# HPCForge/Bubbleformer

Measured on AMD Instinct MI355X. Metric: train samples/sec, FiLMAViT 16x192x192x4ch, bs=8 per GPU, higher is better.
Workload: dtype bf16; 1 GPU; FiLMAViT-small (E=384, 6 heads, 12 blocks, P=16, 9 fluid params) fwd + relative-L2 loss + bwd + AdamW, 4-field 16x192x192 clips, batch 8 per GPU (BASELINE.json configs[1]); global_batch=8, parallelism=dp1

## Files before the change

bubbleformer_amd/_lib.py:

```python
import ctypes as C
import os
import subprocess

_HERE = os.path.dirname(os.path.abspath(__file__))
LIB_PATH = os.path.join(_HERE, "libbubbleformer_hip.so")
CSRC = os.path.join(_HERE, "csrc")

BF_DTYPE_F32, BF_DTYPE_BF16 = 0, 1
BF_LAY_KC, BF_LAY_XC = 0, 1
BF_PRO_NONE, BF_PRO_AFFINE, BF_PRO_AFFINE_GELU, BF_PRO_GELU = 0, 1, 2, 3
BF_AUX_NONE, BF_AUX_ADD, BF_AUX_DGELU = 0, 1, 2
BF_OUT_STORE, BF_OUT_STORE_F32, BF_OUT_ATOMIC_F32 = 0, 1, 2
BF_MAX_STAGES = 5
BF_LOSS_LIMBS = 5

vp, fp, i32, i64, f32 = C.c_void_p, C.c_void_p, C.c_int32, C.c_int64, C.c_float


class Operand(C.Structure):
    _fields_ = [("p", vp), ("ld", i64), ("layout", i32), ("seglen", i32), ("segstride", i64), ("gw", i32), ("gh", i32),
                ("gc", i32), ("pro", i32), ("sc", fp), ("sh", fp), ("rows_per_frame", i32), ("nch", i32)]


class Epilogue(C.Structure):
# ... 24 lines not shown


class FrameNorm(C.Structure):
    _fields_ = [("w", fp), ("b", fp), ("g", fp), ("gdiv", i32), ("mean", fp), ("rstd", fp), ("sc", fp), ("sh", fp), ("resid", vp), ("out", vp)]


class EmbedParams(C.Structure):
    _fields_ = [("conv_w", fp * BF_MAX_STAGES), ("in_w", fp * BF_MAX_STAGES), ("in_b", fp * BF_MAX_STAGES), ("film_ln_w", fp),
                ("film_ln_b", fp), ("film_w", fp), ("film_b", fp)]


class DebedParams(C.Structure):
    _fields_ = [("conv_w", fp * BF_MAX_STAGES), ("in_w", fp * BF_MAX_STAGES), ("in_b", fp * BF_MAX_STAGES)]


class ConvSrc(C.Structure):
    _fields_ = [("p", vp), ("C", i32), ("nchw", i32), ("f32", i32)]


class ConvGeo(C.Structure):
    _fields_ = [(n, i32) for n in ("F", "Hi", "Wi", "Ho", "Wo", "kh", "kw", "stride", "pad")]


BF_CONV_PRO_NONE, BF_CONV_PRO_AFFINE_GELU, BF_CONV_PRO_GELU = 0, 1, 2

STAGE_DONE_FN = C.CFUNCTYPE(None, C.c_int, C.c_void_p)
P = C.POINTER
SIGNATURES = {
    "bf_last_error": (C.c_char_p, []),
    "bf_abi_version": (C.c_int, []),
    "bf_prof_enable": (None, [C.c_int]),
    "bf_debug_force_generic_attn": (None, [C.c_int]),
    "bf_debug_tokred_fold": (None, [C.c_int]),
    "bf_side_defer": (None, [C.c_int]),
    "bf_prep_stages": (C.c_int, [C.POINTER(Dims), C.c_int, C.POINTER(C.c_int32), C.POINTER(vp), C.POINTER(vp), C.POINTER(vp), vp]),
    "bf_stage_prepared": (None, [C.c_int]),
    "bf_trunk_train_fwd": (C.c_int, [C.POINTER(Dims), C.c_int, C.POINTER(C.c_int32), C.POINTER(vp), C.POINTER(vp), C.POINTER(vp), C.POINTER(vp), vp,
                                     C.POINTER(vp), vp, vp]),
    "bf_trunk_train_bwd": (C.c_int, [C.POINTER(Dims), C.c_int, C.POINTER(C.c_int32), C.POINTER(vp), C.POINTER(vp), C.POINTER(vp), C.POINTER(vp),
                                     C.POINTER(vp), vp, C.POINTER(vp), vp, C.POINTER(vp), vp, vp, vp, vp, vp]),
    "bf_field_stats_ws_doubles": (i64, [C.c_int]),
    "bf_field_stats": (C.c_int, [fp, vp, vp, C.c_int, vp, vp, vp]),
    "bf_stage_chain_next": (C.c_int, [C.POINTER(Dims), C.c_int, vp, vp]),
    "bf_stage_next_scale": (C.c_int, [fp, C.c_int]),
    "bf_gemm_fwd_frames": (C.c_int, [C.c_int, C.c_int, C.c_int, C.c_int, vp, i64, vp, i64, fp, fp, fp, fp, C.c_int, vp, vp, C.c_int,
                                     C.POINTER(FrameNorm), C.POINTER(FrameNorm), vp]),
    "bf_trunk_eval_weights_bytes": (i64, [C.POINTER(Dims), C.c_int, C.POINTER(C.c_int32)]),
    "bf_trunk_eval_prepare": (C.c_int, [C.POINTER(Dims), C.c_int, C.POINTER(C.c_int32), C.POINTER(vp), vp, vp]),
    "bf_trunk_eval_fwd": (C.c_int, [C.POINTER(Dims), C.c_int, C.POINTER(C.c_int32), C.POINTER(vp), vp, vp, vp, vp, vp]),
    "bf_frame_linear": (C.c_int, [C.c_int, C.c_int, C.c_int, C.c_int, C.c_int, vp, i64, vp, i64, fp, fp, fp, fp, fp, vp, i64, C.c_int, fp, fp, fp,
                                  vp, i64, fp, fp, vp, i64, vp]),
    "bf_side_join": (C.c_int, [vp]),
    "bf_prof_report": (C.c_int, [C.c_char_p, C.c_int]),
    "bf_gemm": (C.c_int, [C.c_int, C.c_int, C.c_int, C.c_int, P(Operand), P(Operand), P(Epilogue), C.c_int, vp]),
    "bf_gemm_tokred": (C.c_int, [C.c_int, C.c_int, C.c_int, i64, vp, i64, vp, i64, fp, C.c_int, fp, fp, i64, vp]),
    "bf_gemm_tokred_ws_floats": (i64, [C.c_int, C.c_int, i64]),
    "bf_gemm_inbwd_frames": (C.c_int, [C.c_int, C.c_int, C.c_int, C.c_int, vp, i64, vp, i64, vp, vp, vp, C.c_int, fp, fp, fp, fp, fp, C.c_int, vp]),
    "bf_gemm_inbwd_frames_chain": (C.c_int, [C.c_int, C.c_int, C.c_int, C.c_int, vp, i64, vp, i64, vp, vp, vp, C.c_int, fp, fp, fp, fp, fp, C.c_int,
                                             vp, vp, fp, fp, fp, fp, C.c_int, fp, vp]),
    "bf_in_stats": (C.c_int, [C.c_int, vp, C.c_int, C.c_int, C.c_int, fp, fp, fp, C.c_int, fp, fp, fp, fp, fp, fp, vp]),
    "bf_in_ws_floats": (i64, [C.c_int, C.c_int, C.c_int, C.c_int]),
    "bf_affine_apply": (C.c_int, [C.c_int, vp, vp, fp, fp, vp, i64, C.c_int, C.c_int, vp]),
    "bf_in_bwd": (C.c_int, [C.c_int, vp, vp, vp, vp, C.c_int, C.c_int, C.c_int, fp, fp, fp, fp, fp, C.c_int, C.c_int, fp, fp,
                            fp, fp, fp, vp]),
    "bf_colsum": (C.c_int, [C.c_int, vp, i64, C.c_int, fp, fp, vp]),
    "bf_attn_axial_fwd": (C.c_int, [C.c_int, vp, vp, i64, C.c_int, C.c_int, C.c_int, C.c_int, fp, fp, fp, fp, fp, fp, fp, vp]),
    "bf_attn_axial_norm_fwd": (C.c_int, [C.c_int, vp, vp, vp, i64, C.c_int, C.c_int, C.c_int, C.c_int, fp, fp, fp, fp, fp, fp, fp, fp, fp, fp, fp, fp,
                                         fp, vp]),
    "bf_attn_fwd": (C.c_int, [C.c_int, vp, vp, i64, C.c_int, i64, i64, i64, i64, C.c_int, C.c_int, fp, fp, fp, fp, fp, fp, f32,
                              C.c_int, vp]),
    "bf_attn_bwd": (C.c_int, [C.c_int, vp, vp, vp, i64, C.c_int, i64, i64, i64, i64, C.c_int, C.c_int, fp, fp, fp, fp, fp, fp,
                              fp, fp, fp, fp, fp, fp, f32, C.c_int, fp, i64, vp]),
    "bf_im2col_nchw": (C.c_int, [C.c_int, fp, vp, C.c_int, C.c_int, C.c_int, C.c_int, C.c_int, vp]),
    "bf_col2im_nchw": (C.c_int, [C.c_int, vp, fp, C.c_int, C.c_int, C.c_int, C.c_int, C.c_int, vp]),
    "bf_pm2nchw": (C.c_int, [fp, fp, fp, fp, C.c_int, C.c_int, C.c_int, C.c_int, C.c_int, vp]),
    "bf_debed_last_bwd": (C.c_int, [C.c_int, fp, fp, fp, fp, fp, vp, vp, vp, C.c_int, C.c_int, C.c_int, C.c_int, C.c_int, C.c_int, vp]),
    "bf_debed_last_bwd_norm": (C.c_int, [C.c_int, fp, fp, fp, fp, fp, vp, vp, vp, fp, fp, fp, fp, vp, fp, fp, C.c_int, C.c_int, C.c_int, C.c_int, C.c_int,
                                         C.c_int, fp, C.c_int64, vp]),
    "bf_gather_gemm": (C.c_int, [C.c_int, vp, vp, C.c_int, fp, fp, vp, C.c_int, C.c_int, C.c_int, C.c_int, C.c_int, vp]),
    "bf_scatter_gemm": (C.c_int, [C.c_int, vp, vp, C.c_int, fp, fp, vp, fp, C.c_int, C.c_int, C.c_int, C.c_int, C.c_int, vp]),
    "bf_gather_wgrad_ws_floats": (C.c_int64, [C.c_int, C.c_int, C.c_int]),
    "bf_gather_wgrad": (C.c_int, [C.c_int, vp, vp, fp, fp, fp, fp, fp, C.c_int, C.c_int, C.c_int, C.c_int, C.c_int, C.c_int, fp, C.c_int64, vp]),
    "bf_gather_gemm_rebuilt": (C.c_int, [C.c_int, vp, vp, vp, C.c_int, fp, fp, vp, C.c_int, C.c_int, C.c_int, C.c_int, C.c_int, vp]),
    "bf_gather_wgrad_rebuilt": (C.c_int, [C.c_int, vp, vp, vp, fp, fp, fp, C.c_int, C.c_int, C.c_int, C.c_int, C.c_int, C.c_int, fp, C.c_int64, vp]),
    "bf_stage_chain_head": (C.c_int, [vp, vp, vp]),
    "bf_stage_chain_tail": (C.c_int, [vp, vp, C.c_int]),
    "bf_embed_tail_ws_floats": (C.c_int64, [C.c_int, C.c_int, C.c_int, C.c_int, C.c_int]),
    "bf_embed_tail_bwd": (C.c_int, [C.c_int, vp, vp, vp, vp, vp, fp, fp, fp, fp, fp, fp, fp, fp, C.c_int, C.c_int, C.c_int, C.c_int, C.c_int, C.c_int,
                                    fp, C.c_int64, vp]),
    "bf_embed_first": (C.c_int, [C.c_int, fp, vp, vp, vp, C.c_int, C.c_int, C.c_int, C.c_int, C.c_int, C.c_int, fp, vp]),
    "bf_in_stats_merge_slices": (C.c_int, [C.c_int, C.c_int, C.c_int, C.c_int, C.c_int, fp, fp, fp, C.c_int, fp, fp, fp, fp, fp, fp, vp]),
    "bf_debed_last": (C.c_int, [C.c_int, vp, fp, fp, vp, fp, fp, fp, C.c_int, C.c_int, C.c_int, C.c_int, C.c_int, C.c_int, vp]),
    "bf_lploss_finalize": (C.c_int, [fp, C.c_int, C.c_int, fp, fp, vp]),
    "bf_nchw2pm": (C.c_int, [C.c_int, fp, fp, fp, fp, fp, vp, C.c_int, C.c_int, C.c_int, C.c_int, C.c_int, vp]),
    "bf_wprep": (C.c_int, [C.c_int, C.c_int, fp, vp, C.c_int, C.c_int, C.c_int, vp]),
    "bf_wgrad_unprep": (C.c_int, [C.c_int, fp, fp, C.c_int, C.c_int, C.c_int, C.c_int, vp]),
    "bf_film_net_fwd": (C.c_int, [fp, fp, fp, fp, fp, fp, fp, fp, C.c_int, C.c_int, C.c_int, vp]),
    "bf_film_net_bwd": (C.c_int, [fp, fp, fp, fp, fp, fp, fp, fp, fp, C.c_int, C.c_int, C.c_int, vp]),
    "bf_adamw": (C.c_int, [fp, fp, fp, fp, i64, C.c_int, f32, f32, f32, f32, f32, f32, vp]),
    "bf_adam": (C.c_int, [fp, fp, fp, fp, i64, C.c_int, f32, f32, f32, f32, f32, f32, vp]),
    "bf_lion": (C.c_int, [fp, fp, fp, i64, f32, f32, f32, f32, f32, vp]),
    "bf_grad_norm_ws_doubles": (i64, [i64]),
    "bf_grad_norm": (C.c_int, [fp, i64, f32, f32, fp, vp, i64, vp]),
    "bf_adamw_dev": (C.c_int, [fp, fp, fp, fp, i64, C.c_int, f32, f32, f32, f32, f32, f32, fp, f32, vp]),
    "bf_adam_dev": (C.c_int, [fp, fp, fp, fp, i64, C.c_int, f32, f32, f32, f32, f32, f32, fp, f32, vp]),
# ... 99 lines not shown
```

bubbleformer_amd/csrc/attn.hip:

```cpp
#include "bf_common.h"
#include "param_reduce.h"

namespace {

constexpr int NT = 256;
__device__ __forceinline__ void wave_sync() {
    __builtin_amdgcn_fence(__ATOMIC_ACQ_REL, "wavefront");
    __builtin_amdgcn_wave_barrier();
}
constexpr int LMAX = 32;
constexpr int LONG_LMAX = 128;
constexpr int DMAX = 128;

__device__ __forceinline__ int t5_bucket(int n) {
    const int a = n < 0 ? -n : n;
    int b;
    if (a < 8) b = a;
    else if (a < 10) b = 8;
    else if (a < 12) b = 9;
    else if (a < 14) b = 10;
    else if (a < 16) b = 11;
    else if (a < 20) b = 12;
    else if (a < 23) b = 13;
    else if (a < 27) b = 14;
// ... 307 lines not shown

template <typename K>
int plan_waves(K kernel, size_t floats_per_wave, int* wpb, size_t* shm) {
    int w = 4;
    while (w > 1 && (size_t)w * floats_per_wave * sizeof(float) > 64 * 1024) w >>= 1;
    *wpb = w;
    *shm = (size_t)w * floats_per_wave * sizeof(float);
    if (*shm > 156 * 1024) return bf_fail_msg("attention: L*d too large for the LDS plan", __FILE__, __LINE__);
    if (*shm > 64 * 1024) {
        hipError_t e = hipFuncSetAttribute(reinterpret_cast<const void*>(kernel), hipFuncAttributeMaxDynamicSharedMemorySize, (int)*shm);
        if (e != hipSuccess) return bf_fail(e, __FILE__, __LINE__);
    }
    return 0;
}

bool g_force_generic = false;

int check_geo(const char* who, int dtype, int heads, int d, int L) {
    const int ch = dtype == BF_DTYPE_BF16 ? 8 : 4;
    if (heads < 1 || heads > 16) return bf_fail_msg("attention: heads must be in 1..16", who, 0);
    if (d < ch || d > DMAX || d % ch) return bf_fail_msg("attention: head dim must be a multiple of the 16-byte chunk and <= 128", who, 0);
    if (L < 1 || L > LONG_LMAX) return bf_fail_msg("attention: sequence length must be in 1..128", who, 0);
    return 0;
}

}

int bf_attn_fwd_mfma(const void* qkv, void* out, long nseq, int L, long inner, long outer_stride, long inner_stride, long tok_stride, int heads,
                     int d, const float* qw, const float* qb, const float* kw, const float* kb, const float* emb, const float* hscale,
                     float out_scale, int accumulate, hipStream_t st);
int bf_attn_bwd_mfma(const void* qkv, const void* dout, void* dqkv, long nseq, int L, long inner, long outer_stride, long inner_stride,
                     long tok_stride, int heads, int d, const float* qw, const float* qb, const float* kw, const float* kb, const float* emb,
                     const float* hscale, float* dqw, float* dqb, float* dkw, float* dkb, float* demb, float* dhscale, float out_scale,
                     int accumulate, float* ws, long ws_floats, int* rows_out, hipStream_t st);
int bf_attn_fwd_long(int dtype, const void* qkv, void* out, long nseq, int L, long inner, long outer_stride, long inner_stride, long tok_stride,
                     int heads, int d, const float* qw, const float* qb, const float* kw, const float* kb, const float* emb, const float* hscale,
                     float out_scale, int accumulate, hipStream_t st);
int bf_attn_bwd_long(int dtype, const void* qkv, const void* dout, void* dqkv, long nseq, int L, long inner, long outer_stride, long inner_stride,
                     long tok_stride, int heads, int d, const float* qw, const float* qb, const float* kw, const float* kb, const float* emb,
                     const float* hscale, float* dqw, float* dqb, float* dkw, float* dkb, float* demb, float* dhscale, float out_scale,
                     int accumulate, float* ws, long ws_floats, int* rows_out, hipStream_t st);
int bf_attn_axial_fwd_mfma(const void* qkv, void* out, int frames, int h, int w, int heads, int d, const float* qw, const float* qb, const float* kw,
                           const float* kb, const float* emb, const float* hscale_x, const float* hscale_y, const float* nw, const float* nb,
                           void* out_n, float* mean, float* rstd, float* sc, float* sh, hipStream_t st);
static bool use_mfma(int dtype, int d) { return !g_force_generic && dtype == BF_DTYPE_BF16 && d % 32 == 0 && d <= 128; }
bool bf_attn_raw_modes(int dtype, int d) { return use_mfma(dtype, d); }

extern "C" void bf_debug_force_generic_attn(int on) { g_force_generic = on != 0; }

extern "C" int bf_attn_fwd(int dtype, const void* qkv, void* out, int64_t nseq, int L, int64_t inner, int64_t outer_stride,
                           int64_t inner_stride, int64_t tok_stride, int heads, int d, const float* qw, const float* qb,
                           const float* kw, const float* kb, const float* emb, const float* hscale, float out_scale,
                           int accumulate, bf_stream_t stream) {
    BF_REQUIRE(qkv && out && qw && qb && kw && kb && nseq > 0 && inner > 0, "bf_attn_fwd: bad arguments");
    if (int rc = check_geo("bf_attn_fwd", dtype, heads, d, L)) return rc;
    if (L > LMAX) {
        BfProfScope prof((hipStream_t)stream, "attn_fwd", 4.0 * nseq * heads * L * L * d, (double)nseq * heads * L * d * bf_esize(dtype) * (accumulate ? 5.0 : 4.0));
        return bf_attn_fwd_long(dtype, qkv, out, nseq, L, inner, outer_stride, inner_stride, tok_stride, heads, d, qw, qb, kw, kb, emb, hscale,
                                out_scale, accumulate, (hipStream_t)stream);
    }
    if (use_mfma(dtype, d)) {
        BfProfScope prof((hipStream_t)stream, "attn_fwd", 4.0 * nseq * heads * L * L * d, (double)nseq * heads * L * d * 2.0 * (accumulate ? 5.0 : 4.0));
        return bf_attn_fwd_mfma(qkv, out, nseq, L, inner, outer_stride, inner_stride, tok_stride, heads, d, qw, qb, kw, kb, emb, hscale, out_scale,
                                accumulate, (hipStream_t)stream);
    }
    SeqGeo g{nseq, L, inner, outer_stride, inner_stride, tok_stride};
    AttnParams p{qw, qb, kw, kb, emb, hscale};
// ... 14 lines not shown
extern "C" int bf_attn_axial_fwd(int dtype, const void* qkv, void* out, int64_t frames, int h, int w, int heads, int d, const float* qw,
                                 const float* qb, const float* kw, const float* kb, const float* emb, const float* hscale_x,
                                 const float* hscale_y, bf_stream_t stream) {
    BF_REQUIRE(qkv && out && qw && qb && kw && kb && frames > 0 && h > 0 && w > 0, "bf_attn_axial_fwd: bad arguments");
    if (use_mfma(dtype, d) && frames < (1L << 24)) {
        BfProfScope prof((hipStream_t)stream, "attn_fwd", 4.0 * frames * heads * h * w * (h + w) * d, (double)frames * h * w * heads * d * 2.0 * 4.0);
        const int rc = bf_attn_axial_fwd_mfma(qkv, out, (int)frames, h, w, heads, d, qw, qb, kw, kb, emb, hscale_x, hscale_y, nullptr, nullptr, nullptr,
                                              nullptr, nullptr, nullptr, nullptr, (hipStream_t)stream);
        if (rc <= 0) return rc;
    }
    const long S = (long)h * w;
    int rc = bf_attn_fwd(dtype, qkv, out, frames * h, w, 1, w, 0, 1, heads, d, qw, qb, kw, kb, emb, hscale_x, 0.5f, 0, stream);
    if (rc) return rc;
    return bf_attn_fwd(dtype, qkv, out, frames * w, h, w, S, 1, w, heads, d, qw, qb, kw, kb, emb, hscale_y, 0.5f, 1, stream);
}

extern "C" int bf_attn_axial_norm_fwd(int dtype, const void* qkv, void* out, void* out_n, int64_t frames, int h, int w, int heads, int d,
                                      const float* qw, const float* qb, const float* kw, const float* kb, const float* emb,
                                      const float* hscale_x, const float* hscale_y, const float* norm_w, const float* norm_b, float* mean,
                                      float* rstd, float* sc, float* sh, bf_stream_t stream) {
    BF_REQUIRE(qkv && out && out_n && qw && qb && kw && kb && norm_w && norm_b && mean && rstd && sc && sh && frames > 0 && h > 0 && w > 0,
               "bf_attn_axial_norm_fwd: bad arguments");
    static const bool off = bf_knob("BF_ATTN_AXIAL_NORM", 1) == 0;
    if (off || !use_mfma(dtype, d) || frames >= (1L << 24)) return 1;
    BfProfScope prof((hipStream_t)stream, "attn_fwd", 4.0 * frames * heads * h * w * (h + w) * d, (double)frames * h * w * heads * d * 2.0 * 5.0);
    return bf_attn_axial_fwd_mfma(qkv, out, (int)frames, h, w, heads, d, qw, qb, kw, kb, emb, hscale_x, hscale_y, norm_w, norm_b, out_n, mean, rstd, sc,
                                  sh, (hipStream_t)stream);
}

static int attn_bwd_impl(int dtype, const void* qkv, const void* dout, void* dqkv, int64_t nseq, int L, int64_t inner,
                         int64_t outer_stride, int64_t inner_stride, int64_t tok_stride, int heads, int d, const float* qw,
                         const float* qb, const float* kw, const float* kb, const float* emb, const float* hscale,
                         float* dqw, float* dqb, float* dkw, float* dkb, float* demb, float* dhscale, float out_scale,
                         int accumulate, float* ws, int64_t ws_floats, int* rows_out, bf_stream_t stream) {
    if (rows_out) *rows_out = 0;
    BF_REQUIRE(qkv && dout && dqkv && qw && qb && kw && kb && nseq > 0 && inner > 0, "bf_attn_bwd: bad arguments");
    if (int rc = check_geo("bf_attn_bwd", dtype, heads, d, L)) return rc;
    BF_REQUIRE(accumulate == 0 || accumulate == 1 || ((accumulate == 2 || accumulate == 5) && use_mfma(dtype, d)),
               "bf_attn_bwd: accumulate must be 0 / 1 (or 2 / 5, the raw-gradient pair of passes, on the bf16 MFMA path)");
    if (L > LMAX) {
        BfProfScope prof((hipStream_t)stream, "attn_bwd", 10.0 * nseq * heads * L * L * d, (double)nseq * heads * L * d * bf_esize(dtype) * (accumulate ? 10.0 : 7.0));
        return bf_attn_bwd_long(dtype, qkv, dout, dqkv, nseq, L, inner, outer_stride, inner_stride, tok_stride, heads, d, qw, qb, kw, kb, emb, hscale,
                                dqw, dqb, dkw, dkb, demb, dhscale, out_scale, accumulate, ws, (long)ws_floats, rows_out, (hipStream_t)stream);
    }
    if (use_mfma(dtype, d)) {
        BfProfScope prof((hipStream_t)stream, "attn_bwd", 10.0 * nseq * heads * L * L * d, (double)nseq * heads * L * d * 2.0 * (accumulate ? 10.0 : 7.0));
        return bf_attn_bwd_mfma(qkv, dout, dqkv, nseq, L, inner, outer_stride, inner_stride, tok_stride, heads, d, qw, qb, kw, kb, emb, hscale, dqw,
                                dqb, dkw, dkb, demb, dhscale, out_scale, accumulate, ws, (long)ws_floats, rows_out, (hipStream_t)stream);
    }
    SeqGeo g{nseq, L, inner, outer_stride, inner_stride, tok_stride};
    AttnParams p{qw, qb, kw, kb, emb, hscale};
    AttnGrads gr{dqw, dqb, dkw, dkb, demb, dhscale};
    const size_t fpw = 6 * L * (d + 1) + 2 * L * (L + 1) + 2 * L;
    int WPB; size_t shm;
    if (int rc = dtype == BF_DTYPE_BF16 ? plan_waves(attn_bwd_kernel<bf16>, fpw, &WPB, &shm) : plan_waves(attn_bwd_kernel<float>, fpw, &WPB, &shm)) return rc;
    const long nprob = nseq * heads;
    BfProfScope prof((hipStream_t)stream, "attn_bwd", 10.0 * nprob * L * L * d, (double)nprob * L * d * bf_esize(dtype) * (accumulate ? 10.0 : 7.0));
    const int full = (int)std::min<long>((nprob + WPB - 1) / WPB, 256 * 4), nvals = 4 * d + 32 * heads + heads;
    int grid = full;
    if (ws && ws_floats < (int64_t)full * nvals) { grid = (int)(ws_floats / nvals); if (grid < 1) { ws = nullptr; grid = full; } }
    if (dtype == BF_DTYPE_BF16)
        hipLaunchKernelGGL(attn_bwd_kernel<bf16>, dim3(grid), dim3(WPB * 64), shm, (hipStream_t)stream, (const bf16*)qkv, (const bf16*)dout, (bf16*)dqkv, g, heads, d, p, gr, out_scale, accumulate, ws);
    else
        hipLaunchKernelGGL(attn_bwd_kernel<float>, dim3(grid), dim3(WPB * 64), shm, (hipStream_t)stream, (const float*)qkv, (const float*)dout, (float*)dqkv, g, heads, d, p, gr, out_scale, accumulate, ws);
    BF_CHECK_LAUNCH();
    if (rows_out) { *rows_out = ws ? grid : 0; return 0; }
    if (ws) {
        const AttnReduceJob j{ws, grid, d, heads, dqw, dqb, dkw, dkb, demb, dhscale};
        hipLaunchKernelGGL(attn_rows_reduce_kernel, dim3(bf_cdiv(nvals, 64)), dim3(64 * BF_RED_FL), 0, (hipStream_t)stream, j);
        BF_CHECK_LAUNCH();
    }
    return 0;
}

extern "C" int bf_attn_bwd(int dtype, const void* qkv, const void* dout, void* dqkv, int64_t nseq, int L, int64_t inner,
                           int64_t outer_stride, int64_t inner_stride, int64_t tok_stride, int heads, int d, const float* qw,
                           const float* qb, const float* kw, const float* kb, const float* emb, const float* hscale,
                           float* dqw, float* dqb, float* dkw, float* dkb, float* demb, float* dhscale, float out_scale,
                           int accumulate, float* ws, int64_t ws_floats, bf_stream_t stream) {
    return attn_bwd_impl(dtype, qkv, dout, dqkv, nseq, L, inner, outer_stride, inner_stride, tok_stride, heads, d, qw, qb, kw, kb, emb, hscale, dqw,
                         dqb, dkw, dkb, demb, dhscale, out_scale, accumulate, ws, ws_floats, nullptr, stream);
}
int bf_attn_bwd_partials(int dtype, const void* qkv, const void* dout, void* dqkv, int64_t nseq, int L, int64_t inner, int64_t outer_stride,
                         int64_t inner_stride, int64_t tok_stride, int heads, int d, const float* qw, const float* qb, const float* kw,
                         const float* kb, const float* emb, const float* hscale, float* dqw, float* dqb, float* dkw, float* dkb, float* demb,
                         float* dhscale, float out_scale, int accumulate, float* ws, int64_t ws_floats, int* rows, hipStream_t stream) {
    return attn_bwd_impl(dtype, qkv, dout, dqkv, nseq, L, inner, outer_stride, inner_stride, tok_stride, heads, d, qw, qb, kw, kb, emb, hscale, dqw,
                         dqb, dkw, dkb, demb, dhscale, out_scale, accumulate, ws, ws_floats, rows, (bf_stream_t)stream);
}
```

bubbleformer_amd/csrc/attn_mfma.hip:

```cpp
#include "bf_common.h"
#include "param_reduce.h"
#include <stdlib.h>

namespace {

typedef __attribute__((ext_vector_type(8))) short s16x8;
typedef __attribute__((address_space(3))) s16x4* lds_s16x4;

__device__ __forceinline__ void drain_vm() { __builtin_amdgcn_s_waitcnt(0x0F70); }
__device__ __forceinline__ void wsync() {
    __builtin_amdgcn_fence(__ATOMIC_ACQ_REL, "wavefront");
    __builtin_amdgcn_wave_barrier();
}
__device__ __forceinline__ int t5b(int n) {
    const int a = n < 0 ? -n : n;
    int b;
    if (a < 8) b = a; else if (a < 10) b = 8; else if (a < 12) b = 9; else if (a < 14) b = 10; else if (a < 16) b = 11;
    else if (a < 20) b = 12; else if (a < 23) b = 13; else if (a < 27) b = 14; else b = 15;
    return b + (n < 0 ? 16 : 0);
}
typedef unsigned u32x2 __attribute__((ext_vector_type(2)));
__device__ __forceinline__ float quad_sum(float v) {
    u32x2 r = __builtin_amdgcn_permlane16_swap(__float_as_uint(v), __float_as_uint(v), false, false);
    v = __uint_as_float(r[0]) + __uint_as_float(r[1]);
    r = __builtin_amdgcn_permlane32_swap(__float_as_uint(v), __float_as_uint(v), false, false);
    return __uint_as_float(r[0]) + __uint_as_float(r[1]);
}
__device__ __forceinline__ float row16_sum(float v) {
    v += __builtin_bit_cast(float, __builtin_amdgcn_update_dpp(0, __builtin_bit_cast(int, v), 0xB1, 0xF, 0xF, true));
    v += __builtin_bit_cast(float, __builtin_amdgcn_update_dpp(0, __builtin_bit_cast(int, v), 0x4E, 0xF, 0xF, true));
    v += __builtin_bit_cast(float, __builtin_amdgcn_update_dpp(0, __builtin_bit_cast(int, v), 0x141, 0xF, 0xF, true));
    v += __builtin_bit_cast(float, __builtin_amdgcn_update_dpp(0, __builtin_bit_cast(int, v), 0x140, 0xF, 0xF, true));
    return v;
}
__device__ __forceinline__ float quad_max(float v) {
    u32x2 r = __builtin_amdgcn_permlane16_swap(__float_as_uint(v), __float_as_uint(v), false, false);
    v = fmaxf(__uint_as_float(r[0]), __uint_as_float(r[1]));
    r = __builtin_amdgcn_permlane32_swap(__float_as_uint(v), __float_as_uint(v), false, false);
    return fmaxf(__uint_as_float(r[0]), __uint_as_float(r[1]));
}

struct Geo { long nseq; int L; long inner, outer_stride, inner_stride, tok_stride; };
struct Prob { long tok0; int head; };
__device__ __forceinline__ Prob locate(const Geo& g, int heads, long pr) {
    const unsigned p = (unsigned)pr, hd = (unsigned)heads, inner = (unsigned)g.inner;
    const unsigned s = p / hd, head = p - s * hd;
    const unsigned q = s / inner, r = s - q * inner;
    return Prob{(long)q * g.outer_stride + (long)r * g.inner_stride, (int)head};
}
template <int CTRL>
__device__ __forceinline__ float dpp_add(float keep, float send) {
    return keep + __builtin_bit_cast(float, __builtin_amdgcn_update_dpp(0, __builtin_bit_cast(int, send), CTRL, 0xF, 0xF, true));
}
__device__ __forceinline__ float row16_scatter_sum(const float (&p)[16], int i16) {
    float a0, a1, a2, a3, a4, a5, a6, a7, b[4];
#define BF_M1(a, lo, hi) "v_add_f32_dpp " a ", " lo ", " lo " row_mirror row_mask:0xf bank_mask:0x3\n\t" \
                         "v_add_f32_dpp " a ", " hi ", " hi " row_mirror row_mask:0xf bank_mask:0xc\n\t"
#define BF_M2(b, lo, hi) "v_add_f32_dpp " b ", " lo ", " lo " row_half_mirror row_mask:0xf bank_mask:0x5\n\t" \
                         "v_add_f32_dpp " b ", " hi ", " hi " row_half_mirror row_mask:0xf bank_mask:0xa\n\t"
    asm("s_nop 4\n\t"
        BF_M1("%4", "%12", "%20") BF_M1("%5", "%13", "%21") BF_M1("%6", "%14", "%22") BF_M1("%7", "%15", "%23")
        BF_M1("%8", "%16", "%24") BF_M1("%9", "%17", "%25") BF_M1("%10", "%18", "%26") BF_M1("%11", "%19", "%27")
        BF_M2("%0", "%4", "%8") BF_M2("%1", "%5", "%9") BF_M2("%2", "%6", "%10") BF_M2("%3", "%7", "%11")
        : "=&v"(b[0]), "=&v"(b[1]), "=&v"(b[2]), "=&v"(b[3]), "=&v"(a0), "=&v"(a1), "=&v"(a2), "=&v"(a3), "=&v"(a4), "=&v"(a5), "=&v"(a6), "=&v"(a7)
        : "v"(p[0]), "v"(p[1]), "v"(p[2]), "v"(p[3]), "v"(p[4]), "v"(p[5]), "v"(p[6]), "v"(p[7]),
          "v"(p[8]), "v"(p[9]), "v"(p[10]), "v"(p[11]), "v"(p[12]), "v"(p[13]), "v"(p[14]), "v"(p[15]));
#undef BF_M1
#undef BF_M2
    const bool b1 = i16 & 2, b0 = i16 & 1;
    float c[2];
#pragma unroll
    for (int j = 0; j < 2; ++j) c[j] = dpp_add<0x4E>(b1 ? b[2 + j] : b[j], b1 ? b[j] : b[2 + j]);
    return dpp_add<0xB1>(b0 ? c[1] : c[0], b0 ? c[0] : c[1]);
}
struct Par { const float *qw, *qb, *kw, *kb, *emb, *hscale; };
struct Grd { float *dqw, *dqb, *dkw, *dkb, *demb, *dhscale; };

__device__ __forceinline__ s16x4 tr4(const bf16* tile, int ld, int r0, int c0, int lane) {
    const int i16 = lane & 15, q = i16 >> 2, p = i16 & 3;
// ... 442 lines not shown
            __syncthreads();
        }
    }
}

template <int NB, int KS> struct RawRows { bf16x8 q[NB][KS], k[NB][KS], v[NB][KS], d[NB][KS]; };
template <int NB, int KS> struct OldRows { bf16x8 q[NB][KS], k[NB][KS], v[NB][KS]; };

template <int NB, int KS>
__device__ __forceinline__ void load_raw(RawRows<NB, KS>& r, const bf16* __restrict__ qkv, const bf16* __restrict__ dout, const Geo& g, int heads, const Prob& at,
                                         int lane) {
    constexpr int D = 32 * KS;
    const int E = heads * D;
    const int head = at.head;
    const long tok0 = at.tok0;
    const int gq = lane >> 4, i16 = lane & 15;
#pragma unroll
    for (int b = 0; b < NB; ++b) {
        const int i = b * 16 + i16, ic = i < g.L ? i : g.L - 1;
        const bf16* rp = qkv + (tok0 + ic * g.tok_stride) * 3L * E + head * 3 * D + 8 * gq;
        const bf16* dp = dout + (tok0 + ic * g.tok_stride) * (long)E + head * D + 8 * gq;
#pragma unroll
        for (int ks = 0; ks < KS; ++ks) {
            r.q[b][ks] = *reinterpret_cast<const bf16x8*>(rp + 32 * ks);
            r.k[b][ks] = *reinterpret_cast<const bf16x8*>(rp + D + 32 * ks);
            r.v[b][ks] = *reinterpret_cast<const bf16x8*>(rp + 2 * D + 32 * ks);
            r.d[b][ks] = *reinterpret_cast<const bf16x8*>(dp + 32 * ks);
        }
    }
}

template <int NB, int KS, int ACC>
__global__ void __launch_bounds__(256, ((NB == 1 && KS <= 2) ? 2 : 1)) attn_bwd_mfma(const bf16* __restrict__ qkv, const bf16* __restrict__ dout, bf16* __restrict__ dqkv, Geo g,
                                                     int heads, Par p, Grd gr, float out_scale, int accumulate_rt, float* __restrict__ ws) {
    constexpr int D = 32 * KS, LD = D + 16, NT16 = D / 16, R = 16 * NB, LDP = 32 + 8;
    constexpr bool PREFETCH = NB * KS <= 4;
    extern __shared__ __attribute__((aligned(16))) bf16 smem_bwd[];
    __shared__ float s_demb[32 * 16];
    __shared__ float s_dhs[16];
    __shared__ __attribute__((aligned(16))) float s_par[4 * 32 * KS];
    __shared__ float s_emb[32 * 16];
    __shared__ float s_hsc[16];
    const int lane = threadIdx.x & 63, wave = __builtin_amdgcn_readfirstlane(threadIdx.x >> 6), wpb = blockDim.x >> 6;
    constexpr int PER_WAVE = 3 * R * LD + 2 * R * LDP;
    static_assert(3 * R * LD * 2 >= 4 * D * 4, "the parameter-gradient flush must fit in the operand tiles");
    bf16* qn_t = smem_bwd + wave * PER_WAVE;
    bf16* kn_t = qn_t + R * LD;
    bf16* do_t = kn_t + R * LD;
    bf16* at_t = do_t + R * LD;
    bf16* ds_t = at_t + R * LDP;
    float* relay = reinterpret_cast<float*>(qn_t);
    for (int i = threadIdx.x; i < 32 * 16; i += blockDim.x) {
        s_demb[i] = 0.f;
        const int t = i >> 4, h = i & 15;
        s_emb[i] = (p.emb && h < heads) ? p.emb[t * heads + h] : 0.f;
    }
    if (threadIdx.x < 16) { s_dhs[threadIdx.x] = 0.f; s_hsc[threadIdx.x] = (p.hscale && (int)threadIdx.x < heads) ? p.hscale[threadIdx.x] : 1.f; }
    for (int i = threadIdx.x; i < 4 * D; i += blockDim.x) {
        const int q = i / D, e = i % D;
        s_par[i] = (q == 0 ? p.qw : q == 1 ? p.qb : q == 2 ? p.kw : p.kb)[e];
    }
    __syncthreads();
    const int E = heads * D, L = g.L;
    const float scale = rsqrtf((float)D);
    const long nprob = g.nseq * heads;
    const int gq = lane >> 4, i16 = lane & 15;
    const int mode = ACC >= 0 ? ACC : accumulate_rt;
    const bool raw_out = mode & 2, raw_in = mode & 4, accumulate = mode & 1;

    constexpr int NACC = 2 * KS;
    float a_ln[NACC];
#pragma unroll
    for (int k = 0; k < NACC; ++k) a_ln[k] = 0.f;
    const long pstep = (long)gridDim.x * wpb;
    const bool one_head = pstep % heads == 0;
    float a_emb[NB][NB][4], a_dhs = 0.f;
#pragma unroll
    for (int jb = 0; jb < NB; ++jb)
#pragma unroll
        for (int ib = 0; ib < NB; ++ib)
#pragma unroll
            for (int r = 0; r < 4; ++r) a_emb[jb][ib][r] = 0.f;
    long pr = (long)blockIdx.x * wpb + wave;
    RawRows<NB, KS> cur, nxt;
    Prob at = locate(g, heads, pr < nprob ? pr : 0), at_next = at;
    if (pr < nprob) load_raw<NB, KS>(cur, qkv, dout, g, heads, at, lane);
    if (PREFETCH) drain_vm();
    float mk[NB][NB][4], mneg[NB][NB][4];
    int eidx[NB][NB][4];
    lane_masks<NB>(L, lane, mk, mneg, eidx);
    if (NB == 1) {
        for (int c = lane; c < 16 * 16; c += 64) { at_t[(c >> 4) * LDP + 16 + (c & 15)] = (bf16)0.f; ds_t[(c >> 4) * LDP + 16 + (c & 15)] = (bf16)0.f; }
    }
    for (; pr < nprob; pr += pstep) {
        const int head = at.head;
        const long tok0 = at.tok0;
        const bool more = pr + pstep < nprob;
        if (more) at_next = locate(g, heads, pr + pstep);
        if (PREFETCH && more) load_raw<NB, KS>(nxt, qkv, dout, g, heads, at_next, lane);
        OldRows<NB, KS> old;
        if (accumulate) {
#pragma unroll
            for (int b = 0; b < NB; ++b) {
                const int row = b * 16 + i16, rc = row < L ? row : L - 1;
                const bf16* ob = dqkv + (tok0 + rc * g.tok_stride) * 3L * E + head * 3 * D;
#pragma unroll
                for (int ks = 0; ks < KS; ++ks) {
                    old.q[b][ks] = *reinterpret_cast<const bf16x8*>(ob + 32 * ks + 8 * gq);
                    old.k[b][ks] = *reinterpret_cast<const bf16x8*>(ob + D + 32 * ks + 8 * gq);
                    old.v[b][ks] = *reinterpret_cast<const bf16x8*>(ob + 2 * D + 32 * ks + 8 * gq);
                }
                if (raw_in && row >= L) {
                    const bf16x8 z8 = {};
#pragma unroll
                    for (int ks = 0; ks < KS; ++ks) { old.q[b][ks] = z8; old.k[b][ks] = z8; }
                }
            }
        }
        float xq[NB][KS][8], xk[NB][KS][8], rq[NB], rk[NB];
        bf16x8 qf[NB][KS], kf[NB][KS], vf[NB][KS], df[NB][KS];
#pragma unroll
        for (int b = 0; b < NB; ++b) {
#pragma unroll
            for (int ks = 0; ks < KS; ++ks)
#pragma unroll
                for (int j = 0; j < 8; ++j) { xq[b][ks][j] = (float)cur.q[b][ks][j]; xk[b][ks][j] = (float)cur.k[b][ks][j]; }
            rq[b] = ln_quad<KS>(xq[b], D);
            affine_frag<KS>(xq[b], s_par, s_par + D, scale, lane, qf[b]);
            rk[b] = ln_quad<KS>(xk[b], D);
            affine_frag<KS>(xk[b], s_par + 2 * D, s_par + 3 * D, 1.f, lane, kf[b]);
            const int row = b * 16 + i16;
// ... 149 lines not shown
#pragma unroll
                    for (int ks = 0; ks < KS; ++ks) {
                        bf16x8 o;
#pragma unroll
                        for (int j = 0; j < 8; ++j) {
                            const float xh = part == 0 ? xq[b][ks][j] : xk[b][ks][j];
                            float v = rs * (dn[ks][j] - m1 - xh * m2);
                            if (accumulate && !raw_in) v += (float)(part == 0 ? old.q[b][ks][j] : old.k[b][ks][j]);
                            o[j] = (bf16)v;
                        }
                        *reinterpret_cast<bf16x8*>(dst + 32 * ks) = o;
                    }
                }
            }
            {
                float flat[16 * KS];
#pragma unroll
                for (int ks = 0; ks < KS; ++ks)
#pragma unroll
                    for (int j = 0; j < 8; ++j) { flat[8 * ks + j] = pw[ks][j]; flat[8 * KS + 8 * ks + j] = pb[ks][j]; }
#pragma unroll
                for (int gi = 0; gi < KS; ++gi) {
                    float grp[16];
#pragma unroll
                    for (int q = 0; q < 16; ++q) grp[q] = flat[16 * gi + q];
                    a_ln[part * KS + gi] += row16_scatter_sum(grp, i16);
                }
            }
        }
        wsync();
        if (PREFETCH) cur = nxt;
        else if (more) load_raw<NB, KS>(cur, qkv, dout, g, heads, at_next, lane);
        at = at_next;
    }
    if (one_head && pr - pstep >= 0) {
        const int head = (int)(((long)blockIdx.x * wpb + wave) % heads);
#pragma unroll
        for (int jb = 0; jb < NB; ++jb)
#pragma unroll
            for (int ib = 0; ib < NB; ++ib)
#pragma unroll
                for (int r = 0; r < 4; ++r) {
                    const int i = 16 * ib + i16, j = 16 * jb + 4 * gq + r;
                    if (gr.demb && i < L && j < L) atomicAdd(&s_demb[t5b(i - j) * 16 + head], a_emb[jb][ib][r]);
                }
        if (p.hscale && gr.dhscale) {
            a_dhs = wave_sum(a_dhs);
            if (lane == 0) atomicAdd(&s_dhs[head], a_dhs);
        }
    }
#pragma unroll
    for (int k = 0; k < NACC; ++k) {
        const int v = 16 * k + i16, q = v / (8 * KS), ks = (v >> 3) % KS, j = v & 7;
        relay[q * D + 32 * ks + 8 * gq + j] = a_ln[k];
    }
    __syncthreads();
    const int nvals = 4 * D + 32 * heads + heads;
    for (int i = threadIdx.x; i < nvals; i += blockDim.x) {
        float val;
        float* dst;
        if (i < 4 * D) {
            val = 0.f;
            for (int w = 0; w < wpb; ++w) val += reinterpret_cast<const float*>(smem_bwd + w * PER_WAVE)[i];
            const int q = i / D, e = i % D; dst = (q == 0 ? gr.dqw : q == 1 ? gr.dqb : q == 2 ? gr.dkw : gr.dkb); if (dst) dst += e; }
        else if (i < 4 * D + 32 * heads) { const int t = i - 4 * D; val = s_demb[(t / heads) * 16 + (t % heads)]; dst = gr.demb ? gr.demb + t : nullptr; }
        else { const int t = i - 4 * D - 32 * heads; val = s_dhs[t]; dst = gr.dhscale ? gr.dhscale + t : nullptr; }
// ... 1 lines not shown
        else if (dst && val != 0.f) atomicAdd(dst, val);
    }
}

__global__ void __launch_bounds__(64 * BF_RED_FL) attn_ws_reduce(AttnReduceJob j) {
    __shared__ float red[1][BF_RED_FL][64];
    attn_reduce_block(j, blockIdx.x, blockIdx.y, gridDim.y, red);
}

template <typename K>
int set_lds(K kernel, size_t shm) {
    if (shm > 64 * 1024) {
        hipError_t e = hipFuncSetAttribute(reinterpret_cast<const void*>(kernel), hipFuncAttributeMaxDynamicSharedMemorySize, (int)shm);
        if (e != hipSuccess) return bf_fail(e, __FILE__, __LINE__);
    }
    return 0;
}

template <int NB, int KS>
int go_fwd(const bf16* qkv, bf16* out, Geo g, int heads, Par p, float out_scale, int accumulate, hipStream_t st) {
    constexpr int D = 32 * KS;
    const int wpb = 4;
    const size_t shm = (size_t)wpb * 16 * NB * (D + 16) * sizeof(bf16);
    const long nprob = g.nseq * heads;
    BF_REQUIRE(nprob < (1L << 31) && g.inner < (1L << 31), "attention: problem count must fit 31 bits");
    static const int bpc = bf_knob("BF_ATTN_FWD_BPC", 2);
    const int grid = (int)std::min<long>((nprob + wpb - 1) / wpb, 256L * bpc);
    hipLaunchKernelGGL((attn_fwd_mfma<NB, KS>), dim3(grid), dim3(wpb * 64), shm, st, qkv, out, g, heads, p, out_scale, accumulate);
    BF_CHECK_LAUNCH();
    return 0;
}
template <int NB, int KS, int ACC>
int go_bwd_mode(const bf16* qkv, const bf16* dout, bf16* dqkv, Geo g, int heads, Par p, Grd gr, float out_scale, int accumulate, float* ws,
                long ws_floats, int* rows_out, hipStream_t st) {
    constexpr int D = 32 * KS, R = 16 * NB;
    const int wpb = NB == 1 ? 4 : 2;
    const size_t shm = (size_t)wpb * (3 * R * (D + 16) + 2 * R * 40) * sizeof(bf16);
    if (int rc = set_lds(attn_bwd_mfma<NB, KS, ACC>, shm)) return rc;
    const long nprob = g.nseq * heads;
    BF_REQUIRE(nprob < (1L << 31) && g.inner < (1L << 31), "attention: problem count must fit 31 bits");
    const int nvals = 4 * D + 32 * heads + heads;
    static int resident = 0;
    if (!resident) {
        int dev = 0, cus = 256, per_cu = 1;
        (void)hipGetDevice(&dev);
        (void)hipDeviceGetAttribute(&cus, hipDeviceAttributeMultiprocessorCount, dev);
        if (hipOccupancyMaxActiveBlocksPerMultiprocessor(&per_cu, attn_bwd_mfma<NB, KS, ACC>, wpb * 64, shm) != hipSuccess || per_cu < 1) per_cu = 1;
        static const int bpc = bf_knob("BF_ATTN_BWD_BPC", 0);
        if (bpc > 0) per_cu = bpc;
        resident = cus * per_cu;
    }
    long grid = std::min<long>((nprob + wpb - 1) / wpb, (long)resident);
    {
        long a = wpb, b = heads;
        while (b) { const long t = a % b; a = b; b = t; }
        const long m = heads / a;
        if (grid >= 8 * m) grid -= grid % m;
    }
    if (ws && ws_floats < grid * nvals) { grid = ws_floats / nvals; if (grid < 1) ws = nullptr; }
    hipLaunchKernelGGL((attn_bwd_mfma<NB, KS, ACC>), dim3((int)grid), dim3(wpb * 64), shm, st, qkv, dout, dqkv, g, heads, p, gr, out_scale, accumulate, ws);
    BF_CHECK_LAUNCH();
    if (rows_out) { *rows_out = ws ? (int)grid : 0; return 0; }
    if (ws) {
        const AttnReduceJob j{ws, (int)grid, D, heads, gr.dqw, gr.dqb, gr.dkw, gr.dkb, gr.demb, gr.dhscale};
        hipLaunchKernelGGL(attn_ws_reduce, dim3(bf_cdiv(nvals, 64), 1), dim3(64 * BF_RED_FL), 0, st, j);
        BF_CHECK_LAUNCH();
    }
    return 0;
}
template <int NB, int KS>
int go_bwd(const bf16* qkv, const bf16* dout, bf16* dqkv, Geo g, int heads, Par p, Grd gr, float out_scale, int accumulate, float* ws,
           long ws_floats, int* rows_out, hipStream_t st) {
#define BF_MODE(A) return go_bwd_mode<NB, KS, A>(qkv, dout, dqkv, g, heads, p, gr, out_scale, accumulate, ws, ws_floats, rows_out, st)
    if constexpr (NB == 1 && KS == 2) {
        switch (accumulate) { case 0: BF_MODE(0); case 1: BF_MODE(1); case 2: BF_MODE(2); case 5: BF_MODE(5); default: break; }
    }
    BF_MODE(-1);
#undef BF_MODE
}

}

int bf_attn_fwd_mfma(const void* qkv, void* out, long nseq, int L, long inner, long outer_stride, long inner_stride, long tok_stride, int heads,
                     int d, const float* qw, const float* qb, const float* kw, const float* kb, const float* emb, const float* hscale,
                     float out_scale, int accumulate, hipStream_t st) {
    Geo g{nseq, L, inner, outer_stride, inner_stride, tok_stride};
    Par p{qw, qb, kw, kb, emb, hscale};
    const int nb = L <= 16 ? 1 : 2, ks = d / 32;
#define GO(NB, KS) if (nb == NB && ks == KS) return go_fwd<NB, KS>((const bf16*)qkv, (bf16*)out, g, heads, p, out_scale, accumulate, st)
    GO(1, 1); GO(1, 2); GO(1, 3); GO(1, 4); GO(2, 1); GO(2, 2); GO(2, 3); GO(2, 4);
#undef GO
    return bf_fail_msg("bf_attn_fwd_mfma: unsupported shape", __FILE__, __LINE__);
}
int bf_attn_axial_fwd_mfma(const void* qkv, void* out, int frames, int h, int w, int heads, int d, const float* qw, const float* qb, const float* kw,
                           const float* kb, const float* emb, const float* hscale_x, const float* hscale_y, const float* nw, const float* nb,
                           void* out_n, float* mean, float* rstd, float* sc, float* sh, hipStream_t st) {
    static const bool off = bf_knob("BF_ATTN_AXIAL_FUSED", 1) == 0;
    if (off || h > 16 || w > 16 || h < 1 || w < 1 || d % 32 || d > 128 || heads > 16) return 1;
    Par p{qw, qb, kw, kb, emb, hscale_x};
    const long ntile = (long)frames * heads;
    static const int wpb_env = bf_knob("BF_ATTN_AXIAL_WPB", 0);
    const int ks = d / 32, wpb = (wpb_env == 4 || wpb_env == 12) ? wpb_env : (ntile <= 256 ? 12 : 4);
    const bool norm = nw != nullptr;
    const size_t tile = ((size_t)h * w * (d + 8) + 7) & ~(size_t)7;
    const size_t shm = ((size_t)wpb * 16 * (d + 16) + tile) * sizeof(bf16) + (norm ? ((size_t)(256 / (d / 8)) + 2) * d * sizeof(float) : 0);
    const int grid = (int)std::min<long>(ntile, 256L * 3);
    const AxNorm nrm{nw, nb, (bf16*)out_n, mean, rstd, sc, sh};
#define GO2(KS, NRM, W) { if (int rc = set_lds(attn_fwd_axial_mfma<KS, NRM, W>, shm)) return rc; \
        hipLaunchKernelGGL((attn_fwd_axial_mfma<KS, NRM, W>), dim3(grid), dim3(W * 64), shm, st, (const bf16*)qkv, (bf16*)out, frames, h, w, heads, p, hscale_y, nrm); }
#define GO(KS) if (ks == KS) { \
        if (norm) { if (wpb == 12) GO2(KS, true, 12) else GO2(KS, true, 4) } \
        else { if (wpb == 12) GO2(KS, false, 12) else GO2(KS, false, 4) } }
    GO(1) GO(2) GO(3) GO(4)
#undef GO
#undef GO2
    BF_CHECK_LAUNCH();
    return 0;
}
int bf_attn_bwd_mfma(const void* qkv, const void* dout, void* dqkv, long nseq, int L, long inner, long outer_stride, long inner_stride,
                     long tok_stride, int heads, int d, const float* qw, const float* qb, const float* kw, const float* kb, const float* emb,
                     const float* hscale, float* dqw, float* dqb, float* dkw, float* dkb, float* demb, float* dhscale, float out_scale,
                     int accumulate, float* ws, long ws_floats, int* rows_out, hipStream_t st) {
    Geo g{nseq, L, inner, outer_stride, inner_stride, tok_stride};
    Par p{qw, qb, kw, kb, emb, hscale};
    Grd gr{dqw, dqb, dkw, dkb, demb, dhscale};
    const int nb = L <= 16 ? 1 : 2, ks = d / 32;
#define GO(NB, KS) if (nb == NB && ks == KS) return go_bwd<NB, KS>((const bf16*)qkv, (const bf16*)dout, (bf16*)dqkv, g, heads, p, gr, out_scale, accumulate, ws, ws_floats, rows_out, st)
    GO(1, 1); GO(1, 2); GO(1, 3); GO(1, 4); GO(2, 1); GO(2, 2); GO(2, 3); GO(2, 4);
#undef GO
    return bf_fail_msg("bf_attn_bwd_mfma: unsupported shape", __FILE__, __LINE__);
}
```

bubbleformer_amd/csrc/bf_common.h:

```cpp
#pragma once
#include <hip/hip_runtime.h>
#include <stdint.h>
#include <math.h>

#include "../../include/bubbleformer_hip.h"

typedef __bf16 bf16;
typedef __attribute__((ext_vector_type(8))) __bf16 bf16x8;
typedef __attribute__((ext_vector_type(4))) __bf16 bf16x4;
typedef __attribute__((ext_vector_type(4))) short s16x4;
typedef __attribute__((ext_vector_type(4))) float f32x4;

#define BF_WAVE 64
#define BF_IN_EPS 1e-5f

#define BF_CHECK_LAUNCH()                                   \
    do {                                                    \
        hipError_t e__ = hipGetLastError();                 \
        if (e__ != hipSuccess) return bf_fail(e__, __FILE__, __LINE__); \
    } while (0)
#define BF_REQUIRE(cond, msg)                                \
    do {                                                     \
        if (!(cond)) return bf_fail_msg(msg, __FILE__, __LINE__); \
    } while (0)

int bf_prof_begin(hipStream_t st);
bool bf_prof_is_on();
void bf_prof_end(int idx, hipStream_t st, const char* name, double flops, double bytes);
struct BfProfScope {
    int idx; hipStream_t st; const char* name; double flops, bytes;
    BfProfScope(hipStream_t s, const char* n, double f, double b) : idx(bf_prof_begin(s)), st(s), name(n), flops(f), bytes(b) {}
    ~BfProfScope() { if (idx >= 0) bf_prof_end(idx, st, name, flops, bytes); }
};

int bf_in_bwd_partials(int dtype, const void* dy, const void* x, const void* add, void* dx, int frames, int S, int C, const float* mean,
                       const float* rstd, const float* w, const float* b, const float* g, int gdiv, int gelu, float* ws, hipStream_t stream);
int bf_attn_bwd_partials(int dtype, const void* qkv, const void* dout, void* dqkv, int64_t nseq, int L, int64_t inner, int64_t outer_stride,
                         int64_t inner_stride, int64_t tok_stride, int heads, int d, const float* qw, const float* qb, const float* kw,
                         const float* kb, const float* emb, const float* hscale, float* dqw, float* dqb, float* dkw, float* dkb, float* demb,
                         float* dhscale, float out_scale, int accumulate, float* ws, int64_t ws_floats, int* rows, hipStream_t stream);
int bf_in_stats_apply(int dtype, const void* x, int frames, int S, int C, const float* w, const float* b, const float* g, int gdiv, const float* gb,
                      float* mean, float* rstd, float* sc, float* sh, float* ws, const void* resid, void* out, hipStream_t stream);
int bf_in_stats_apply_chain(int dtype, const void* x, int frames, int S, int C, const float* w, const float* b, const float* g, int gdiv, const float* gb,
                            float* mean, float* rstd, float* sc, float* sh, float* ws, const void* resid, void* out, const float* nw, const float* nb,
                            float* nmean, float* nrstd, float* nsc, float* nsh, void* nxn, bool* chained, hipStream_t stream);
int bf_wprep_multi(int dtype, int n, const int* mode, const float* const* src, void* const* dst, const int* R, const int* K, const int* Kp, hipStream_t st);
int bf_frame_scale(int dtype, const void* z, const float* m, int fdiv, void* out, long nrows, int S, int C, hipStream_t st);

int bf_gemm_slabs(int dtype, int M, int N, int K, const bf_operand* A, const bf_operand* B, float* out, long ldc, int accumulate, int splitk,
                  float* ws, long ws_floats, hipStream_t st);
int bf_tokred_narrow(int dtype, int C, int64_t P, const void* wide, const void* narrow, float* out, int ldo, int accumulate, int transposed,
                     const float* sc, const float* sh, int64_t rows_per_frame, float* ws, int64_t ws_floats, hipStream_t st);
int bf_gemm_pair_scaled(int M, int N, int K, const bf_operand* A, const bf_operand* B, const bf_epilogue* E, void* out2, const float* rowfac,
                        int rows_per_group, hipStream_t st);

#ifdef BF_EXPERIMENTS
#include <stdlib.h>
inline int bf_knob(const char* name, int dflt) { const char* v = getenv(name); return v ? atoi(v) : dflt; }
#else
constexpr int bf_knob(const char*, int dflt) { return dflt; }
#endif

struct BfPerDeviceOnce {
    bool done[64] = {};
    bool& flag() { int dev = 0; (void)hipGetDevice(&dev); return done[(dev >= 0 && dev < 64) ? dev : 0]; }
};
template <class T> struct BfPerDevice {
    T tab[64] = {};
    T& get() { int dev = 0; (void)hipGetDevice(&dev); return tab[(dev >= 0 && dev < 64) ? dev : 0]; }
};
int bf_fail(hipError_t e, const char* file, int line);
int bf_fail_msg(const char* msg, const char* file, int line);
int bf_decline(const char* msg);
// ... 77 lines not shown
```

bubbleformer_amd/csrc/gemm_tokred.hip:

```cpp
#include "gemm_common.h"
#include <stdio.h>
#include <stdlib.h>
#include <algorithm>

namespace {
using namespace bfgemm;

constexpr int PTN = 192;
constexpr int HR = 32;
constexpr int NSB = PTN / 64;
constexpr int SUBB = HR * 64 * 2;
constexpr int NBUF = 4;
template <int NI> struct PPGeom {
    static constexpr int TM = 64 * NI, HALFB = (NI + NSB) * SUBB, TILES = NI * 6, TILE_FLOATS = TM * PTN;
};

template <int OFF>
__device__ __forceinline__ void glds16_off(const void* gsrc, unsigned lds_dst) {
    unsigned keep;
    asm volatile("s_mov_b32 %0, m0\n\ts_mov_b32 m0, %2\n\ts_nop 0\n\tglobal_load_lds_dwordx4 %1, off offset:%3\n\ts_mov_b32 m0, %0"
                 : "=&s"(keep) : "v"(gsrc), "s"(lds_dst - (unsigned)OFF), "n"(OFF) : "memory");
}

typedef __attribute__((address_space(3))) s16x4* lds_s16x4_ptr;
__device__ __forceinline__ bf16x8 tr_frag(unsigned addr) {
    const s16x4 lo = __builtin_amdgcn_ds_read_tr16_b64_v4i16((lds_s16x4_ptr)(uintptr_t)addr);
    const s16x4 hi = __builtin_amdgcn_ds_read_tr16_b64_v4i16((lds_s16x4_ptr)(uintptr_t)(addr + 512u));
    typedef __attribute__((ext_vector_type(8))) short s16x8;
    const s16x8 r = {lo[0], lo[1], lo[2], lo[3], hi[0], hi[1], hi[2], hi[3]};
    return __builtin_bit_cast(bf16x8, r);
}

template <int NI, int GRP>
__device__ __forceinline__ void tokred_pp_body(const bf16* __restrict__ A, long lda, const bf16* __restrict__ B, long ldb,
                                               float* __restrict__ slab_tile, float* __restrict__ cslab_row, int nh, bool do_cs,
                                               unsigned ring_lds, int lane, int w4) {
    using Gm = PPGeom<NI>;
    constexpr int HALFB = Gm::HALFB;
    constexpr int PG = NI == 6 ? (GRP == 0 ? 5 : 4) : 3;
    constexpr int NCS = 3;
    const int wm = w4, wn = GRP;
    const int dr = 8 * w4 + (lane >> 3);
    const int dkey = ((dr >> 1) & 1) | (((dr >> 3) & 1) << 1);
    const int dch = (lane & 7) ^ (dkey << 1);
    const bf16* pA = A + (long)dr * lda + 8 * dch;
    const bf16* pB = B + (long)dr * ldb + 8 * dch;
    const long stepA = (long)HR * lda, stepB = (long)HR * ldb;
    auto issue = [&](int buf) {
        const unsigned base = __builtin_amdgcn_readfirstlane(ring_lds + (unsigned)buf * (unsigned)HALFB + (unsigned)w4 * 1024u);
        if constexpr (NI == 6 && GRP == 0) {
            glds16_off<0>(pA, base + 0 * SUBB); glds16_off<128>(pA, base + 1 * SUBB); glds16_off<256>(pA, base + 2 * SUBB);
            glds16_off<384>(pA, base + 3 * SUBB); glds16_off<512>(pA, base + 4 * SUBB);
            pA += stepA;
        } else if constexpr (NI == 6) {
            glds16_off<640>(pA, base + 5 * SUBB);
            glds16_off<0>(pB, base + 6 * SUBB); glds16_off<128>(pB, base + 7 * SUBB); glds16_off<256>(pB, base + 8 * SUBB);
            pA += stepA; pB += stepB;
        } else if constexpr (GRP == 0) {
            glds16_off<0>(pA, base + 0 * SUBB); glds16_off<128>(pA, base + 1 * SUBB); glds16_off<256>(pA, base + 2 * SUBB);
            pA += stepA;
        } else {
            glds16_off<0>(pB, base + 3 * SUBB); glds16_off<128>(pB, base + 4 * SUBB); glds16_off<256>(pB, base + 5 * SUBB);
            pB += stepB;
        }
    };
    const int g = lane >> 4, q = (lane >> 2) & 3, p = lane & 3;
    const int fkey = ((q >> 1) & 1) | ((g & 1) << 1);
    const unsigned rowb = (unsigned)(8 * g + q) * 128u + (unsigned)(p & 1) * 8u;
    const unsigned offA = rowb + (unsigned)(((2 * wm + (p >> 1)) ^ (fkey << 1)) * 16);
    const unsigned offB0 = rowb + (unsigned)(((2 * wn + (p >> 1)) ^ (fkey << 1)) * 16) + (unsigned)(NI * SUBB);
    const unsigned offB1 = rowb + (unsigned)(((2 * wn + 4 + (p >> 1)) ^ (fkey << 1)) * 16) + (unsigned)(NI * SUBB);

    f32x4 acc[NI][6];
#pragma unroll
    for (int i = 0; i < NI; ++i)
#pragma unroll
        for (int j = 0; j < 6; ++j) acc[i][j] = f32x4{0.f, 0.f, 0.f, 0.f};
    f32x4 cs[NCS];
#pragma unroll
    for (int c = 0; c < NCS; ++c) cs[c] = f32x4{0.f, 0.f, 0.f, 0.f};
    bf16x8 ones;
#pragma unroll
    for (int c = 0; c < 8; ++c) ones[c] = (bf16)1.0f;

    issue(0);
    if (nh > 1) issue(1);
    if (nh > 2) issue(2);
    if (nh > 2) wait_vm<2 * PG>(); else if (nh > 1) wait_vm<PG>(); else wait_vm<0>();
    __builtin_amdgcn_s_barrier();
    if constexpr (GRP == 1) __builtin_amdgcn_s_barrier();

    int buf = 0;
    for (int h = 0; h < nh; ++h) {
        const unsigned hb = ring_lds + (unsigned)buf * (unsigned)HALFB;
        bf16x8 fa[NI], fb[6];
#pragma unroll
        for (int i = 0; i < NI; ++i) fa[i] = tr_frag(hb + offA + (unsigned)(i * SUBB));
#pragma unroll
        for (int j = 0; j < 6; ++j) fb[j] = tr_frag(hb + ((j & 1) ? offB1 : offB0) + (unsigned)((j >> 1) * SUBB));
        if (h + 3 < nh) issue((buf + 3) & 3);
        const int younger = min(h + 3, nh - 1) - (h + 1);
        if (younger >= 2) wait_vm<2 * PG>(); else if (younger == 1) wait_vm<PG>(); else wait_vm<0>();
        asm volatile("s_waitcnt lgkmcnt(0)" ::: "memory");
        __builtin_amdgcn_sched_barrier(0);
        __builtin_amdgcn_s_barrier();
#pragma unroll
        for (int i = 0; i < NI; ++i)
#pragma unroll
            for (int j = 0; j < 6; ++j) acc[i][j] = __builtin_amdgcn_mfma_f32_16x16x32_bf16(fb[j], fa[i], acc[i][j], 0, 0, 0);
        if (do_cs) {
#pragma unroll
            for (int c = 0; c < NCS; ++c) {
                if constexpr (NI == 6) cs[c] = __builtin_amdgcn_mfma_f32_16x16x32_bf16(ones, fa[NCS * GRP + c], cs[c], 0, 0, 0);
                else if constexpr (GRP == 0) cs[c] = __builtin_amdgcn_mfma_f32_16x16x32_bf16(ones, fa[c], cs[c], 0, 0, 0);
            }
        }
        __builtin_amdgcn_sched_barrier(0);
        __builtin_amdgcn_s_barrier();
        buf = (buf + 1) & 3;
    }
    if constexpr (GRP == 0) __builtin_amdgcn_s_barrier();

    const int wave = GRP * 4 + w4;
    float* so = slab_tile + ((size_t)wave * Gm::TILES * 64 + lane) * 4;
#pragma unroll
    for (int i = 0; i < NI; ++i)
#pragma unroll
        for (int j = 0; j < 6; ++j)
            *reinterpret_cast<float4*>(so + (size_t)(i * 6 + j) * 256) = make_float4(acc[i][j][0], acc[i][j][1], acc[i][j][2], acc[i][j][3]);
    if (do_cs && lane < 16) {
        if constexpr (NI == 6) {
#pragma unroll
            for (int c = 0; c < NCS; ++c) cslab_row[16 * (wm + 4 * (NCS * GRP + c)) + lane] = cs[c][0];
        } else if constexpr (GRP == 0) {
#pragma unroll
            for (int c = 0; c < NCS; ++c) cslab_row[16 * (wm + 4 * c) + lane] = cs[c][0];
        }
    }
// ... 3 lines not shown
template <int NI>
__device__ __forceinline__ void fold_reduce(const FoldRed& r, int b) {
    using Gm = PPGeom<NI>;
    constexpr int T4 = Gm::TILE_FLOATS / 4;
    const long total = (long)r.ntiles * T4;
    const size_t sstride = (size_t)r.ntiles * Gm::TILE_FLOATS;
    for (long e = (long)b * 512 + threadIdx.x; e < total; e += (long)r.nwg * 512) {
        const int tile = (int)(e / T4), q = (int)(e - (long)tile * T4);
        const int lane = q & 63, t = q >> 6, wave = t / Gm::TILES, ij = t - wave * Gm::TILES, i = ij / 6, j = ij - i * 6;
        const int wm = wave & 3, wn = wave >> 2;
        const int nout = (tile / r.tiles_k) * Gm::TM + 16 * (wm + 4 * i) + (lane & 15);
        const int kin = (tile % r.tiles_k) * PTN + 16 * (wn + 2 * j) + 4 * (lane >> 4);
        const float* src = r.slab + (size_t)tile * Gm::TILE_FLOATS + (size_t)q * 4;
        float4* dst = reinterpret_cast<float4*>(r.out + (size_t)nout * r.Kin + kin);
        float4 a = r.accumulate ? *dst : make_float4(0.f, 0.f, 0.f, 0.f);
        for (int s0 = 0; s0 < r.nslice; s0 += 8) {
            float4 v[8];
#pragma unroll
            for (int u = 0; u < 8; ++u) v[u] = s0 + u < r.nslice ? *reinterpret_cast<const float4*>(src + (size_t)(s0 + u) * sstride) : make_float4(0.f, 0.f, 0.f, 0.f);
#pragma unroll
            for (int u = 0; u < 8; ++u)
                if (s0 + u < r.nslice) { a.x += v[u].x; a.y += v[u].y; a.z += v[u].z; a.w += v[u].w; }
        }
        *dst = a;
    }
    if (r.colsum)
        for (long m = (long)b * 512 + threadIdx.x; m < r.Nout; m += (long)r.nwg * 512) {
            float a = r.accumulate ? r.colsum[m] : 0.f;
            for (int s2 = 0; s2 < r.nslice; ++s2) a += r.cslab[(size_t)s2 * r.Nout + m];
            r.colsum[m] = a;
        }
}

template <int NI>
__global__ void __launch_bounds__(512) tokred_pp_kernel(const bf16* __restrict__ A, long lda, const bf16* __restrict__ B, long ldb,
                                                      float* __restrict__ slab, float* __restrict__ cslab, int Nout, int halves_total,
                                                      int halves_per, int tiles_k, int ntiles, int main_wgs, FoldRed red) {
    using Gm = PPGeom<NI>;
    extern __shared__ __attribute__((aligned(16))) char smem[];
    if ((int)blockIdx.x >= main_wgs) { fold_reduce<NI>(red, (int)blockIdx.x - main_wgs); return; }
    const int tid = threadIdx.x, lane = tid & 63, wave = __builtin_amdgcn_readfirstlane(tid >> 6);
    const int seq = xcd_remap(blockIdx.x, main_wgs);
    const int slice = seq / ntiles, tile = seq - slice * ntiles;
    const int n0 = (tile / tiles_k) * Gm::TM, c0 = (tile % tiles_k) * PTN;
    const int h_beg = slice * halves_per;
    const int nh = min(halves_per, halves_total - h_beg);
    const bf16* a0 = A + (long)h_beg * HR * lda + n0;
    const bf16* b0 = B + (long)h_beg * HR * ldb + c0;
    float* slab_tile = slab + ((size_t)slice * ntiles + tile) * Gm::TILE_FLOATS;
    const bool do_cs = cslab != nullptr && c0 == 0;
    float* cslab_row = do_cs ? cslab + (size_t)slice * Nout + n0 : nullptr;
    const unsigned ring_lds = lds_addr(smem);
    if (wave < 4) tokred_pp_body<NI, 0>(a0, lda, b0, ldb, slab_tile, cslab_row, nh, do_cs, ring_lds, lane, wave);
    else tokred_pp_body<NI, 1>(a0, lda, b0, ldb, slab_tile, cslab_row, nh, do_cs, ring_lds, lane, wave - 4);
}

template <int NI, int MAXS>
__global__ void __launch_bounds__(256) tokred_pp_reduce_kernel(const float* __restrict__ slab, const float* __restrict__ cslab, int nslice,
                                                               int ntiles, int tiles_k, int Nout, int Kin, float* __restrict__ out,
                                                               float* __restrict__ colsum, int accumulate) {
    using Gm = PPGeom<NI>;
    constexpr int T4 = Gm::TILE_FLOATS / 4;
    const long e = (long)blockIdx.x * 256 + threadIdx.x;
    if (e < (long)ntiles * T4) {
        const int tile = (int)(e / T4), r = (int)(e - (long)tile * T4);
        const int lane = r & 63, t = r >> 6, wave = t / Gm::TILES, ij = t - wave * Gm::TILES, i = ij / 6, j = ij - i * 6;
        const int wm = wave & 3, wn = wave >> 2;
        const int nout = (tile / tiles_k) * Gm::TM + 16 * (wm + 4 * i) + (lane & 15);
        const int kin = (tile % tiles_k) * PTN + 16 * (wn + 2 * j) + 4 * (lane >> 4);
        const size_t sstride = (size_t)ntiles * Gm::TILE_FLOATS;
        const float* src = slab + (size_t)tile * Gm::TILE_FLOATS + (size_t)r * 4;
        float4 v[MAXS];
#pragma unroll
        for (int s = 0; s < MAXS; ++s) v[s] = s < nslice ? *reinterpret_cast<const float4*>(src + s * sstride) : make_float4(0.f, 0.f, 0.f, 0.f);
        float4* dst = reinterpret_cast<float4*>(out + (size_t)nout * Kin + kin);
        float4 a = accumulate ? *dst : make_float4(0.f, 0.f, 0.f, 0.f);
#pragma unroll
        for (int s = 0; s < MAXS; ++s)
            if (s < nslice) { a.x += v[s].x; a.y += v[s].y; a.z += v[s].z; a.w += v[s].w; }
        *dst = a;
    }
    if (colsum && e < Nout) {
        float v[MAXS];
#pragma unroll
        for (int s = 0; s < MAXS; ++s) v[s] = s < nslice ? cslab[(size_t)s * Nout + e] : 0.f;
        float a = accumulate ? colsum[e] : 0.f;
#pragma unroll
// ... 211 lines not shown
            float4 v[8];
#pragma unroll
            for (int q = 0; q < 8; ++q) v[q] = s0 + q < nslice ? reinterpret_cast<const float4*>(slab + (size_t)(s0 + q) * n)[i] : make_float4(0.f, 0.f, 0.f, 0.f);
#pragma unroll
            for (int q = 0; q < 8; ++q)
                if (s0 + q < nslice) { a.x += v[q].x; a.y += v[q].y; a.z += v[q].z; a.w += v[q].w; }
        }
        reinterpret_cast<float4*>(out)[i] = a;
    }
    if (colsum) {
        for (long m = (long)blockIdx.x * 256 + threadIdx.x; m < Nout; m += (long)gridDim.x * 256) {
            float a = accumulate ? colsum[m] : 0.f;
            for (int s = 0; s < nslice; ++s) a += cslab[(size_t)s * Nout + m];
            colsum[m] = a;
        }
    }
}

constexpr int MAX_SLICES = 16;

}

extern "C" int64_t bf_gemm_tokred_ws_floats(int Nout, int Kin, int64_t M) {
    if (Nout <= 0 || Kin <= 0 || M <= 0) return 0;
    return (int64_t)MAX_SLICES * ((int64_t)Nout * Kin + Nout);
}

namespace {
struct PendingRed { bool on = false; FoldRed r{}; int NI = 0; hipStream_t st = nullptr; bool half = false; hipEvent_t handoff = nullptr; };
PendingRed g_pending[64];
PendingRed& pending_slot() { int dev = 0; (void)hipGetDevice(&dev); return g_pending[(dev >= 0 && dev < 64) ? dev : 0]; }
constexpr int FOLD_WGS = 40;
}
static int tokred_impl(int dtype, int Nout, int Kin, int64_t M, const void* dy, int64_t ldy, const void* x, int64_t ldx, float* out,
                       int accumulate, float* colsum, float* ws, int64_t ws_floats, bool defer, bf_stream_t stream);
static int flush_pending(PendingRed& p, hipStream_t caller) {
    if (!p.on) return 0;
    p.on = false;
    hipStream_t st = p.st;
    const FoldRed& r = p.r;
    const long n = (long)r.Nout * r.Kin;
    const unsigned rblocks = (unsigned)bf_cdiv(std::max<long>(n / 4, r.Nout), 256);
    BfProfScope prof(st, "tokred_reduce_kernel", 0.0, (double)(r.nslice + 1 + (r.accumulate ? 1 : 0)) * n * 4.0);
    if (p.NI == 6) {
        if (r.nslice <= 8) hipLaunchKernelGGL((tokred_pp_reduce_kernel<6, 8>), dim3(rblocks), dim3(256), 0, st, r.slab, r.cslab, r.nslice, r.ntiles, r.tiles_k, r.Nout, r.Kin, r.out, r.colsum, r.accumulate);
        else hipLaunchKernelGGL((tokred_pp_reduce_kernel<6, MAX_SLICES>), dim3(rblocks), dim3(256), 0, st, r.slab, r.cslab, r.nslice, r.ntiles, r.tiles_k, r.Nout, r.Kin, r.out, r.colsum, r.accumulate);
    } else {
        if (r.nslice <= 8) hipLaunchKernelGGL((tokred_pp_reduce_kernel<3, 8>), dim3(rblocks), dim3(256), 0, st, r.slab, r.cslab, r.nslice, r.ntiles, r.tiles_k, r.Nout, r.Kin, r.out, r.colsum, r.accumulate);
        else hipLaunchKernelGGL((tokred_pp_reduce_kernel<3, MAX_SLICES>), dim3(rblocks), dim3(256), 0, st, r.slab, r.cslab, r.nslice, r.ntiles, r.tiles_k, r.Nout, r.Kin, r.out, r.colsum, r.accumulate);
    }
    BF_CHECK_LAUNCH();
    if (caller == st) return 0;
    hipError_t e = p.handoff ? hipSuccess : hipEventCreateWithFlags(&p.handoff, hipEventDisableTiming);
    if (e == hipSuccess) e = hipEventRecord(p.handoff, st);
    if (e == hipSuccess) e = hipStreamWaitEvent(caller, p.handoff, 0);
    return e == hipSuccess ? 0 : bf_fail(e, __FILE__, __LINE__);
}
int bf_gemm_tokred_flush(hipStream_t st) { return flush_pending(pending_slot(), st); }
namespace { bool g_fold_off = false; }
extern "C" void bf_debug_tokred_fold(int on) { g_fold_off = on == 0; }
bool bf_gemm_tokred_pending() { return pending_slot().on; }
const float* bf_gemm_tokred_pending_out() { const PendingRed& p = pending_slot(); return p.on ? p.r.out : nullptr; }
int bf_gemm_tokred_deferred(int dtype, int Nout, int Kin, int64_t M, const void* dy, int64_t ldy, const void* x, int64_t ldx, float* out,
                            int accumulate, float* colsum, float* ws, int64_t ws_floats, hipStream_t stream) {
    return tokred_impl(dtype, Nout, Kin, M, dy, ldy, x, ldx, out, accumulate, colsum, ws, ws_floats, true, (bf_stream_t)stream);
}
extern "C" int bf_gemm_tokred(int dtype, int Nout, int Kin, int64_t M, const void* dy, int64_t ldy, const void* x, int64_t ldx, float* out,
                              int accumulate, float* colsum, float* ws, int64_t ws_floats, bf_stream_t stream) {
    return tokred_impl(dtype, Nout, Kin, M, dy, ldy, x, ldx, out, accumulate, colsum, ws, ws_floats, false, stream);
}
static int tokred_impl(int dtype, int Nout, int Kin, int64_t M, const void* dy, int64_t ldy, const void* x, int64_t ldx, float* out,
                       int accumulate, float* colsum, float* ws, int64_t ws_floats, bool defer, bf_stream_t stream) {
    if (dtype != BF_DTYPE_BF16) return 1;
    static const int skip_env = bf_knob("BF_TOKRED_SKIP", 0);
    if (skip_env) return 0;
    const bool pp = Nout % 192 == 0 && Kin % PTN == 0 && M % HR == 0 && M >= 4 * HR;
    if (!pp && (Nout % TB || Kin % TB || M % BK || M < BK)) return 1;
    if (ldy % 8 || ldx % 8) return 1;
    BF_REQUIRE(dy && x && out && ws, "bf_gemm_tokred: null pointer");
    BF_REQUIRE(((uintptr_t)dy & 15) == 0 && ((uintptr_t)x & 15) == 0 && ((uintptr_t)out & 15) == 0 && ((uintptr_t)ws & 15) == 0,
               "bf_gemm_tokred: operands must be 16-byte aligned");
    BF_REQUIRE(ldy >= Nout && ldx >= Kin, "bf_gemm_tokred: leading dimensions smaller than the row length");
    hipStream_t st = (hipStream_t)stream;
    const long n = (long)Nout * Kin;
    static const int slices_env = bf_knob("BF_TOKRED_SLICES", 0);
    static const int tile_env = bf_knob("BF_TOKRED_TILE", 0);
    static const int wgs_env = bf_knob("BF_TOKRED_WGS", 128);
    if (pp) {
        const long halves = M / HR;
        const int tiles_k0 = Kin / PTN;
        const bool big = Nout % 384 == 0 && tile_env == 384;
        const int tm = big ? 384 : 192;
        int nslice = slices_env > 0 ? slices_env : std::max(1, wgs_env / ((Nout / tm) * tiles_k0));
        nslice = (int)std::max<long>(1, std::min<long>({(long)nslice, (long)MAX_SLICES, halves / 4}));
        const int halves_per = bf_cdiv(halves, nslice);
        const int ns = bf_cdiv(halves, halves_per);
        BF_REQUIRE(ws_floats >= (int64_t)ns * (n + Nout), "bf_gemm_tokred: workspace too small (bf_gemm_tokred_ws_floats)");
        const int tiles_k = Kin / PTN, ntiles = (Nout / tm) * tiles_k;
        static const bool fold_on = bf_knob("BF_TOKRED_FOLD", 1) != 0;
        const int64_t half_floats = (ws_floats / 2) & ~(int64_t)3;
        const bool fold = defer && fold_on && !g_fold_off && (int64_t)ns * (n + Nout) <= half_floats;
        PendingRed& pend = pending_slot();
        if (pend.on && (!fold || pend.NI != (big ? 6 : 3) || pend.st != st)) { const int frc = flush_pending(pend, st); if (frc) return frc; }
        float* region = ws;
        if (fold) { region = ws + (pend.half ? half_floats : 0); pend.half = !pend.half; }
        float* slab = region;
        float* cslab = colsum ? region + (size_t)ns * n : nullptr;
        const unsigned rblocks = (unsigned)bf_cdiv(std::max<long>(n / 4, Nout), 256);
        FoldRed red{};
        static const int fold_wgs = bf_knob("BF_TOKRED_FOLD_WGS", FOLD_WGS);
        if (fold && pend.on) { red = pend.r; red.nwg = fold_wgs; }
        const unsigned extra = red.nwg > 0 ? (unsigned)red.nwg : 0u;
#define BF_PP_GO(NIV)                                                                                                                     \
        do {                                                                                                                              \
            {                                                                                                                             \
                BfProfScope prof(st, NIV == 6 ? "tokred_pp_kernel<384x192,h32,ring4>" : "tokred_pp_kernel<192x192,h32,ring4>",           \
                                 2.0 * Nout * Kin * (double)M, (double)M * (Nout + Kin) * 2.0 + (double)n * 4.0);                         \
                static BfPerDeviceOnce attr_once; bool& attr_done = attr_once.flag();                                                                                            \
                constexpr int lds_bytes = NBUF * PPGeom<NIV>::HALFB;                                                                      \
                if (!attr_done) {                                                                                                         \
                    hipError_t e_ = hipFuncSetAttribute((const void*)tokred_pp_kernel<NIV>, hipFuncAttributeMaxDynamicSharedMemorySize, lds_bytes); \
                    if (e_ != hipSuccess) return bf_fail(e_, __FILE__, __LINE__);                                                         \
                    attr_done = true;                                                                                                     \
                }                                                                                                                         \
                hipLaunchKernelGGL(tokred_pp_kernel<NIV>, dim3((unsigned)(ns * ntiles) + extra), dim3(512), lds_bytes, st, (const bf16*)dy, (long)ldy, \
                                   (const bf16*)x, (long)ldx, slab, cslab, Nout, (int)halves, halves_per, tiles_k, ntiles, ns * ntiles, red); \
                BF_CHECK_LAUNCH();                                                                                                        \
            }                                                                                                                             \
            if (fold) {                                                                                                                   \
                pend.on = true; pend.NI = NIV; pend.st = st;                                                                              \
                pend.r = FoldRed{slab, cslab, ns, ntiles, tiles_k, Nout, Kin, out, colsum, accumulate, 0};                                \
                break;                                                                                                                    \
            }                                                                                                                             \
            BfProfScope prof(st, "tokred_reduce_kernel", 0.0, (double)(ns + 1 + (accumulate ? 1 : 0)) * n * 4.0);                         \
            if (ns <= 8) hipLaunchKernelGGL((tokred_pp_reduce_kernel<NIV, 8>), dim3(rblocks), dim3(256), 0, st, slab, cslab, ns, ntiles, tiles_k, Nout, Kin, out, colsum, accumulate); \
            else hipLaunchKernelGGL((tokred_pp_reduce_kernel<NIV, MAX_SLICES>), dim3(rblocks), dim3(256), 0, st, slab, cslab, ns, ntiles, tiles_k, Nout, Kin, out, colsum, accumulate); \
            BF_CHECK_LAUNCH();                                                                                                            \
        } while (0)
        if (big) BF_PP_GO(6); else BF_PP_GO(3);
#undef BF_PP_GO
        return 0;
    }
    { const int frc = flush_pending(pending_slot(), st); if (frc) return frc; }
    const long steps = M / BK;
    int nslice = slices_env > 0 ? slices_env : 8;
    nslice = (int)std::max<long>(1, std::min<long>({(long)nslice, (long)MAX_SLICES, steps}));
    BF_REQUIRE(ws_floats >= (int64_t)nslice * (n + Nout), "bf_gemm_tokred: workspace too small (bf_gemm_tokred_ws_floats)");
    const int steps_per = bf_cdiv(steps, nslice);
    const int ns = bf_cdiv(steps, steps_per);
    const int tiles_k = Kin / TB, ntiles = (Nout / TB) * tiles_k;
    float* slab = ws;
    float* cslab = colsum ? ws + (size_t)ns * n : nullptr;
    {
        BfProfScope prof(st, "tokred_kernel<128x128,bk64,slots3>", 2.0 * Nout * Kin * (double)M, (double)M * (Nout + Kin) * 2.0 + (double)n * 4.0);
        static BfPerDeviceOnce attr_once; bool& attr_done = attr_once.flag();
        constexpr int lds_bytes = NSLOT * 2 * BK * TB * 2;
        if (!attr_done) {
            hipError_t e_ = hipFuncSetAttribute((const void*)tokred_kernel, hipFuncAttributeMaxDynamicSharedMemorySize, lds_bytes);
            if (e_ != hipSuccess) return bf_fail(e_, __FILE__, __LINE__);
            attr_done = true;
        }
        hipLaunchKernelGGL(tokred_kernel, dim3((unsigned)(ns * ntiles)), dim3(512), lds_bytes, st, (const bf16*)dy, (long)ldy, (const bf16*)x,
                           (long)ldx, slab, cslab, Nout, Kin, (int)steps, steps_per, tiles_k, ntiles);
        BF_CHECK_LAUNCH();
    }
    {
        BfProfScope prof(st, "tokred_reduce_kernel", 0.0, (double)(ns + 1 + (accumulate ? 1 : 0)) * n * 4.0);
        const int blocks = (int)std::min<long>(512, (n / 4 + 255) / 256);
        hipLaunchKernelGGL(tokred_reduce_kernel, dim3(blocks), dim3(256), 0, st, slab, cslab, ns, n, Nout, out, colsum, accumulate);
        BF_CHECK_LAUNCH();
    }
    return 0;
// ... 28 lines not shown
```

bubbleformer_amd/csrc/model.hip:

```cpp
#include <functional>
#include <vector>
#include "bf_common.h"
#include "param_reduce.h"
#include <stdlib.h>
#include <string.h>

bool bf_attn_raw_modes(int dtype, int d);
int bf_gemm_tokred_deferred(int dtype, int Nout, int Kin, int64_t M, const void* dy, int64_t ldy, const void* x, int64_t ldx, float* out,
                            int accumulate, float* colsum, float* ws, int64_t ws_floats, hipStream_t stream);
int bf_gemm_tokred_flush(hipStream_t st);
bool bf_gemm_tokred_pending();
const float* bf_gemm_tokred_pending_out();
int bf_gemm_inbwd_frames_scaled(int dtype, int M, int N, int K, const void* A, int64_t lda, const void* B, int64_t ldb, const void* x,
                                const void* add, void* out, int S, const float* mean, const float* rstd, const float* w, float* ws,
                                const float* fscale, int fdiv, void* out_s, const float* f_s, int fdiv_s, hipStream_t stream);

namespace {

struct D {
    int dtype, B, T, h, w, E, heads, attn_scale, feat_scale, patch, cin, cout, nfluid;
    long N, F, S;
    int d, nst;
    size_t es;
};
int get_dims(const bf_dims* s, D* o) {
    if (!s) return bf_fail_msg("dims: null", __FILE__, __LINE__);
    o->dtype = s->dtype; o->B = s->B; o->T = s->T; o->h = s->h; o->w = s->w; o->E = s->E; o->heads = s->heads;
    o->attn_scale = s->attn_scale; o->feat_scale = s->feat_scale; o->patch = s->patch; o->cin = s->cin; o->cout = s->cout;
    o->nfluid = s->nfluid;
    if (o->B < 1 || o->T < 1 || o->h < 1 || o->w < 1 || o->E < 8 || o->E > 1024 || o->heads < 1 || o->E % o->heads)
        return bf_fail_msg("dims: bad sizes", __FILE__, __LINE__);
    if (o->dtype != BF_DTYPE_F32 && o->dtype != BF_DTYPE_BF16) return bf_fail_msg("dims: bad dtype", __FILE__, __LINE__);
    o->F = (long)o->B * o->T; o->S = (long)o->h * o->w; o->N = o->F * o->S; o->d = o->E / o->heads;
    o->es = bf_esize(o->dtype);
    const int ch = o->dtype == BF_DTYPE_BF16 ? 8 : 4;
    if (o->E % ch || o->d % ch) return bf_fail_msg("dims: E and head dim must be multiples of the 16-byte chunk", __FILE__, __LINE__);
    if (o->T > 128 || o->h > 128 || o->w > 128) return bf_fail_msg("dims: attention axes are limited to 128 tokens", __FILE__, __LINE__);
    o->nst = 0;
    if (o->patch > 0) {
        int p = o->patch;
        while (p > 1) { if (p & 1) return bf_fail_msg("dims: patch must be a power of two", __FILE__, __LINE__); p >>= 1; o->nst++; }
        if (o->nst < 1 || o->nst > BF_MAX_STAGES) return bf_fail_msg("dims: patch size out of range", __FILE__, __LINE__);
// ... 508 lines not shown
    __shared__ float red[5][BF_RED_FL][64];
    const int z = blockIdx.z;
    if (z < J.n_in) {
        const InReduceJob& j = J.in[z];
        if ((int)blockIdx.x < (j.C + 63) / 64 && (int)blockIdx.y < (j.frames + j.rdiv() - 1) / j.rdiv()) in_reduce_block(j, blockIdx.x, blockIdx.y, red);
    } else {
        int a = z - J.n_in;
        if (J.at_follows[a]) return;
        for (;; ++a) {
            const AttnReduceJob& j = J.at[a];
            const int nvals = 4 * j.D + 32 * j.heads + j.heads;
            if ((int)blockIdx.x < (nvals + 63) / 64 && blockIdx.y == 0) attn_reduce_block(j, blockIdx.x, 0, 1, red);
            if (a + 1 >= J.n_attn || !J.at_follows[a + 1]) break;
            __syncthreads();
        }
    }
}
int launch_reduce_jobs(ReduceJobs& J, hipStream_t st) {
    int k = 0;
    for (int i = 0; i < J.n_attn; ++i) if (J.at[i].rows > 0) J.at[k++] = J.at[i];
    J.n_attn = k;
    for (int i = 0; i < J.n_attn; ++i)
        J.at_follows[i] = i > 0 && J.at[i].D == J.at[i - 1].D && J.at[i].heads == J.at[i - 1].heads &&
                          ((J.at[i].dqw && J.at[i].dqw == J.at[i - 1].dqw) || (J.at[i].demb && J.at[i].demb == J.at[i - 1].demb));
    if (J.n_in + J.n_attn == 0) return 0;
    int gx = 1, gy = 1;
    for (int i = 0; i < J.n_in; ++i) { gx = std::max(gx, bf_cdiv(J.in[i].C, 64)); gy = std::max(gy, bf_cdiv(J.in[i].frames, J.in[i].rdiv())); }
    for (int i = 0; i < J.n_attn; ++i) { gx = std::max(gx, bf_cdiv(4 * J.at[i].D + 33 * J.at[i].heads, 64)); }
    hipLaunchKernelGGL(stage_param_reduce_kernel, dim3(gx, gy, J.n_in + J.n_attn), dim3(64 * BF_RED_FL), 0, st, J);
    BF_CHECK_LAUNCH();
    return 0;
}

int qkv_gemm(const D& d, const void* xn, const void* w_c, const float* bias, void* qkv, hipStream_t st) {
    bf_operand A = op_plain(xn, d.E, BF_LAY_KC);
    bf_operand Bo = op_plain(w_c, d.E, BF_LAY_KC);
    bf_epilogue e = epi_store(qkv, 3L * d.E);
    e.bias = bias;
    return bf_gemm(d.dtype, (int)d.N, 3 * d.E, d.E, &A, &Bo, &e, 1, st);
}
int outproj_gemm(const D& d, const void* on, const void* w_c, const float* alpha, const float* beta,
                 const void* resid, void* out, const float* drop, long rows_per_group, hipStream_t st) {
    bf_operand A = op_plain(on, d.E, BF_LAY_KC);
    bf_operand Bo = op_plain(w_c, d.E, BF_LAY_KC);
    bf_epilogue e = epi_store(out, d.E);
    e.colscale = alpha; e.colshift = beta; e.aux_mode = BF_AUX_ADD; e.aux = resid; e.ld_aux = d.E;
    e.rowscale = drop; e.rows_per_group = (int)rows_per_group;
    return bf_gemm(d.dtype, (int)d.N, d.E, d.E, &A, &Bo, &e, 1, st);
}
void* bwd_scratch(TrunkLinks& L, const D& d, void* scratch) {
    if (!g_side_defer || !L.side_stream()) return scratch;
    L.scratch_parity ^= 1;
    return (char*)scratch + (size_t)L.scratch_parity * Scratch(d, nullptr).bytes;
}
struct TailNorm { const void* z; void* dz; const float *mean, *rstd, *w, *g; int gdiv; float* ws; bool* done; };
struct InFuse { const void* x; const void* add; void* dx; const float* mean; const float* rstd; const float* w; const float* b; float* ws;
                const float* fscale = nullptr; int fdiv = 1;
                const TailNorm* tail = nullptr;
                void* scaled_out = nullptr; const float* scaled_f = nullptr; int scaled_fdiv = 1; bool* scaled_done = nullptr; };
int dgrad_inbwd(const D& d, const void* dy, int Kdim, const void* w_xc, int Nout, void* tmp, const InFuse& f, hipStream_t st) {
    if (f.tail) {
        const TailNorm& t = *f.tail;
        const int crc = bf_gemm_inbwd_frames_chain(d.dtype, (int)d.N, Nout, Kdim, dy, Kdim, w_xc, Nout, f.x, f.add, f.dx, (int)d.S, f.mean, f.rstd, f.w, f.ws,
                                                   f.fscale, f.fdiv, t.z, t.dz, t.mean, t.rstd, t.w, t.g, t.gdiv, t.ws, st);
        if (crc < 0) return crc;
        if (crc == 0) { *t.done = true; return 0; }
    }
    if (f.scaled_out) {
        const int src = bf_gemm_inbwd_frames_scaled(d.dtype, (int)d.N, Nout, Kdim, dy, Kdim, w_xc, Nout, f.x, f.add, f.dx, (int)d.S, f.mean, f.rstd, f.w, f.ws,
                                                    f.fscale, f.fdiv, f.scaled_out, f.scaled_f, f.scaled_fdiv, st);
        if (src < 0) return src;
        if (src == 0) { *f.scaled_done = true; return 0; }
    }
    const int rc = bf_gemm_inbwd_frames(d.dtype, (int)d.N, Nout, Kdim, dy, Kdim, w_xc, Nout, f.x, f.add, f.dx, (int)d.S, f.mean, f.rstd, f.w, f.ws,
                                        f.fscale, f.fdiv, st);
    if (rc <= 0) return rc;
    bf_operand A = op_plain(dy, Kdim, BF_LAY_KC);
    bf_operand Bo = op_plain(w_xc, Nout, BF_LAY_XC);
    bf_epilogue e = epi_store(tmp, Nout);
    if (f.fscale) { e.rowscale = f.fscale; e.rows_per_group = (int)(d.S * f.fdiv); }
    TRY(bf_gemm(d.dtype, (int)d.N, Nout, Kdim, &A, &Bo, &e, 1, st));
    return bf_in_bwd_partials(d.dtype, tmp, f.x, f.add, f.dx, (int)d.F, (int)d.S, Nout, f.mean, f.rstd, f.w, f.b, nullptr, 1, 0, f.ws, st);
}
int outproj_bwd(const D& d, const Scratch& sc, const void* dout, const void* on, const void* w_s,
                const float* W, const float* bias, const float* nb, const float* gamma, const float* lo, const float* hi,
                const float* alpha, const float* mc, float* dW, float* dbias, float* dnb, float* dgamma, float* dlo, float* dhi,
                void* don, hipStream_t st, Fork& fk, const InFuse* fu = nullptr) {
    TRY(fk.run([=](hipStream_t ss) -> int {
        const void* dsrc = dout;
        const int trc = bf_gemm_tokred_deferred(d.dtype, d.E, d.E, d.N, dsrc, d.E, on, d.E, sc.G, 0, sc.csum, sc.tokred_ws, sc.tokred_floats, ss);
        if (trc < 0) return trc;
        if (trc == 1) {
            ZERO_ON(ss, sc.G, (size_t)((char*)sc.csum - (char*)sc.G) + (size_t)d.E * 4);
            bf_operand A = op_plain(dsrc, d.E, BF_LAY_XC);
            bf_operand Bo = op_plain(on, d.E, BF_LAY_XC);
            bf_epilogue e = epi_atomic(sc.G, d.E);
            e.colsum = sc.csum;
            TRY(bf_gemm(d.dtype, d.E, d.E, (int)d.N, &A, &Bo, &e, splitk_for(d.E, d.E, d.N), ss));
        }
        return 0;
    }));
    fk.run_late([=](hipStream_t ss) -> int {
        if (bf_gemm_tokred_pending_out() == sc.G) TRY(bf_gemm_tokred_flush(ss));
        hipLaunchKernelGGL(outproj_finalize_kernel, dim3(d.E + (lo ? bf_cdiv(d.E, 16) : 0)), dim3(256), 0, ss, sc.G, sc.csum, W, bias, nb, gamma, lo, hi, mc,
                           dW, dbias, dnb, dgamma, dlo, dhi, d.E);
        BF_CHECK_LAUNCH();
        return 0;
    });
    if (fu) return dgrad_inbwd(d, dout, d.E, w_s, d.E, don, *fu, st);
    {
        bf_operand A = op_plain(dout, d.E, BF_LAY_KC);
        bf_operand Bo = op_plain(w_s, d.E, BF_LAY_XC);
        bf_epilogue e = epi_store(don, d.E);
        TRY(bf_gemm(d.dtype, (int)d.N, d.E, d.E, &A, &Bo, &e, 1, st));
    }
    return 0;
}
int linear_bwd(const D& d, const Scratch& sc, const void* dy, int Nout, const void* x, int Kin, int xpro, const float* xsc, const float* xsh,
               const void* w_c, float* dW, float* db, void* dxn, const bf_epilogue* dx_epi, hipStream_t st, Fork& fk, const InFuse* fu = nullptr,
               bool last = false, const void* w_t = nullptr, void* scaled_out = nullptr, const float* rowfac = nullptr, int rpg = 1,
               bool* scaled_done = nullptr) {
    TRY(fk.run([=](hipStream_t ss) -> int {
        const void* xo = x;
        int pro = xpro;
        bf_operand A = op_plain(dy, Nout, BF_LAY_XC);
        if (pro == BF_PRO_AFFINE) {
            TRY(bf_affine_apply(d.dtype, x, nullptr, xsc, xsh, sc.s1, d.N, (int)d.S, Kin, ss));
            xo = sc.s1;
            pro = BF_PRO_NONE;
        }
        bf_operand Bo = op_plain(xo, Kin, BF_LAY_XC);
        if (pro == BF_PRO_NONE) {
            const int trc = bf_gemm_tokred_deferred(d.dtype, Nout, Kin, d.N, dy, Nout, xo, Kin, dW, 1, db, sc.tokred_ws, sc.tokred_floats, ss);
            if (trc <= 0) return trc;
        }
        if (pro != BF_PRO_NONE) op_affine(Bo, pro, xsc, xsh, d.S, Kin);
        bf_epilogue e = epi_atomic(dW, Kin);
        e.colsum = db;
        return bf_gemm(d.dtype, Nout, Kin, (int)d.N, &A, &Bo, &e, splitk_for(Nout, Kin, d.N), ss);
    }));
    if (last) TRY(fk.flush());
    if (fu) return dgrad_inbwd(d, dy, Nout, w_c, Kin, dxn, *fu, st);
    {
        bf_operand A = op_plain(dy, Nout, BF_LAY_KC);
        bf_operand Bo = w_t ? op_plain(w_t, Nout, BF_LAY_KC) : op_plain(w_c, Kin, BF_LAY_XC);
        bf_epilogue e = dx_epi ? *dx_epi : epi_store(dxn, Kin);
        e.c = dxn; e.ldc = Kin;
        if (scaled_out && rowfac && d.dtype == BF_DTYPE_BF16) {
            const int rc = bf_gemm_pair_scaled((int)d.N, Kin, Nout, &A, &Bo, &e, scaled_out, rowfac, rpg, st);
            if (rc < 0) return rc;
            if (rc == 0) { if (scaled_done) *scaled_done = true; return 0; }
        }
        TRY(bf_gemm(d.dtype, (int)d.N, Kin, Nout, &A, &Bo, &e, 1, st));
    }
    return 0;
}

}

extern "C" int64_t bf_temporal_saved_bytes(const bf_dims* s) { D d; if (get_dims(s, &d)) return -1; return (int64_t)TemporalSaved(d, nullptr).bytes; }
extern "C" int64_t bf_spatial_saved_bytes(const bf_dims* s) { D d; if (get_dims(s, &d)) return -1; return (int64_t)SpatialSaved(d, nullptr).bytes; }
size_t dbr_bytes(const D& d) { return (((size_t)d.N * d.E * d.es) + 255) & ~(size_t)255; }
extern "C" int64_t bf_scratch_bytes(const bf_dims* s) { D d; if (get_dims(s, &d)) return -1; return 2 * (int64_t)Scratch(d, nullptr).bytes + 2 * (int64_t)dbr_bytes(d); }

extern "C" void bf_side_defer(int on) { g_side_defer = on != 0; }
extern "C" int bf_side_join(bf_stream_t s) { return side_join_pending(g_links.get(), (hipStream_t)s); }

extern "C" void bf_stage_prepared(int on) { g_links.get().hints.prepared = on != 0; }
extern "C" int bf_stage_chain_tail(const bf_spatial_params* prev_p, const void* prev_saved, int has_drop_mlp) {
    g_links.get().hints.tail = NextTail{prev_p && prev_saved, prev_p, prev_saved, has_drop_mlp != 0};
    return 0;
}
extern "C" int bf_stage_next_scale(const float* factors, int fdiv) { g_links.get().hints.scale = NextScale{factors, fdiv > 0 ? fdiv : 1}; return 0; }
static NextHead next_head(const D& d, int kind, const void* params, void* saved) {
    auto of = [&](auto* np, const auto& sv) { return NextHead{true, np->norm1_w, np->norm1_b, sv.mean1, sv.rstd1, sv.sc1, sv.sh1, sv.xn, saved}; };
    return kind == 0 ? of((const bf_temporal_params*)params, TemporalSaved(d, saved)) : of((const bf_spatial_params*)params, SpatialSaved(d, saved));
}
extern "C" int bf_stage_chain_next(const bf_dims* dims, int next_kind, const void* next_params, void* next_saved) {
    NextHead& h = g_links.get().hints.head;
    h = NextHead{};
    if (!dims || !next_params || !next_saved) return 0;
    BF_REQUIRE(next_kind == 0 || next_kind == 1, "bf_stage_chain_next: kind must be 0 (temporal) or 1 (spatial)");
    D d; TRY(get_dims(dims, &d));
    h = next_head(d, next_kind, next_params, next_saved);
    return 0;
}
extern "C" int bf_stage_chain_head(const bf_dims* dims, const bf_temporal_params* next_p, void* next_saved) {
    return bf_stage_chain_next(dims, 0, next_p, next_saved);
}

static int temporal_fwd(TrunkLinks& L, const StageHints& H, const bf_dims* dims, const bf_temporal_params* p, const void* x, void* out, void* saved,
                        void* scratch, const float* drop, bf_stream_t s) {
    D d; TRY(get_dims(dims, &d));
    BF_REQUIRE(p && x && out && saved && scratch, "bf_temporal_fwd: null pointer");
    hipStream_t st = (hipStream_t)s;
    const bool head_done = L.take_head_done(saved, st);
    TRY(side_join_pending(L, st));
    TemporalSaved sv(d, saved);
// ... 26 lines not shown
        const int rc = bf_gemm_fwd_frames(d.dtype, (int)d.N, d.E, d.E, sv.on, d.E, sv.wout_t, d.E, nullptr, sv.alpha, sv.beta, drop, d.T, x, out, (int)d.S,
                                          nullptr, &n2, s);
        if (rc < 0) return rc;
        if (rc == 0) { L.head_done = {h.saved, st}; return 0; }
    }
    TRY(outproj_gemm(d, sv.on, wout_c, sv.alpha, sv.beta, x, out, drop, (long)d.T * d.S, st));
    return 0;
}

static int temporal_bwd(TrunkLinks& L, const StageHints& H, const bf_dims* dims, const bf_temporal_params* p, const bf_temporal_params* g, const void* x,
                        const void* dout, void* dx, void* saved, void* scratch, const float* drop, bf_stream_t s) {
    D d; TRY(get_dims(dims, &d));
    BF_REQUIRE(p && g && x && dout && dx && saved && scratch, "bf_temporal_bwd: null pointer");
    hipStream_t st = (hipStream_t)s;
    TemporalSaved sv(d, saved);
    Scratch sc(d, bwd_scratch(L, d, scratch));
    const void* win_c = d.dtype == BF_DTYPE_F32 ? (const void*)p->input_head_w : sv.win_c;
    Fork fk(L, st, true, L.scratch_parity);
    if (fk.deferred) TRY(side_join_pending(L, st, fk.set));
    void* don = sc.t1;
    void* dO = sc.t1b;
    void* dqkv = sc.t3;
    const void* dbr = dout;
    if (drop) {
        const TrunkLinks::DbrReady& r = L.dbr_ready;
        if (r.dx == dout && r.f == drop && r.buf && r.st == st) dbr = r.buf;
        else {
            TRY(bf_frame_scale(d.dtype, dout, drop, d.T, sc.t4, d.N, (int)d.S, d.E, st));
            dbr = sc.t4;
        }
    }
    L.dbr_ready = TrunkLinks::DbrReady{};
    const InFuse fu2{sv.o, nullptr, dO, sv.mean2, sv.rstd2, p->norm2_w, p->norm2_b, sc.in_ws2};
    TRY(outproj_bwd(d, sc, dbr, sv.on, sv.wout_s, p->output_head_w, p->output_head_b, p->norm2_b, p->gamma, nullptr, nullptr,
                    sv.alpha, sv.mc, g->output_head_w, g->output_head_b, nullptr, g->gamma, nullptr, nullptr, don, st, fk, &fu2));
    ReduceJobs jobs;
    TRY(jobs.push(InReduceJob{sc.in_ws2, (int)d.F, d.E, p->norm2_w, p->norm2_b, nullptr, 1, g->norm2_w, g->norm2_b, nullptr, nullptr, nullptr, nullptr}));
    {
        int rows = 0;
        TRY(bf_attn_bwd_partials(d.dtype, sv.qkv, dO, dqkv, (long)d.B * d.S, d.T, d.S, (long)d.T * d.S, 1, d.S, d.heads, d.d, p->qnorm_w, p->qnorm_b,
                                 p->knorm_w, p->knorm_b, p->rel_pos_emb, d.attn_scale ? p->attn_scale_factor : nullptr, g->qnorm_w, g->qnorm_b,
                                 g->knorm_w, g->knorm_b, g->rel_pos_emb, d.attn_scale ? g->attn_scale_factor : nullptr, 1.f, 0, sc.attn_ws,
                                 Scratch::ATTN_WS_FLOATS, &rows, st));
        TRY(jobs.push(AttnReduceJob{sc.attn_ws, rows, d.d, d.heads, g->qnorm_w, g->qnorm_b, g->knorm_w, g->knorm_b, g->rel_pos_emb,
                                    d.attn_scale ? g->attn_scale_factor : nullptr}));
    }
    void* dxn = sc.t1;
    InFuse fu1{x, dout, dx, sv.mean1, sv.rstd1, p->norm1_w, p->norm1_b, sc.in_ws};
    TailNorm tn;
    bool tail_done = false;
    static const bool chain_on = bf_knob("BF_BWD_CHAIN", 1) != 0;
    if (H.tail.armed && chain_on && fk.deferred && d.dtype == BF_DTYPE_BF16 && d.S == 144 && d.F % 2 == 0) {
        const NextTail& h = H.tail;
        const int oset = L.scratch_parity ^ 1;
        TRY(side_join_pending(L, st, oset));
        Scratch so(d, (char*)scratch + (size_t)oset * Scratch(d, nullptr).bytes);
        SpatialSaved ps(d, const_cast<void*>(h.saved));
        tn = TailNorm{ps.z, so.t1, ps.mean3, ps.rstd3, h.p->mlp_norm_w, h.drop ? ps.gtab : h.p->gamma_mlp, h.drop ? 1 : (int)d.F, L.tail_ws_flip ? so.in_ws5 : so.in_ws4, &tail_done};
        L.tail_ws_flip = !L.tail_ws_flip;
        fu1.tail = &tn;
    }
    if (H.tail.armed) L.tail_done = TrunkLinks::TailDone{};
    TRY(linear_bwd(d, sc, dqkv, 3 * d.E, sv.xn, d.E, BF_PRO_NONE, nullptr, nullptr, win_c, g->input_head_w, g->input_head_b, dxn, nullptr, st, fk, &fu1, true));
    if (tail_done) L.tail_done = {H.tail.saved, dx, tn.ws, st};
    TRY(jobs.push(InReduceJob{sc.in_ws, (int)d.F, d.E, p->norm1_w, p->norm1_b, nullptr, 1, g->norm1_w, g->norm1_b, nullptr, nullptr, nullptr, nullptr}));
    TRY(launch_with_pending(L, jobs, st));
    return fk.join();
}
extern "C" int bf_temporal_fwd(const bf_dims* dims, const bf_temporal_params* p, const void* x, void* out, void* saved, void* scratch,
                               const float* drop, bf_stream_t s) {
    TrunkLinks& L = g_links.get();
    return temporal_fwd(L, L.take_hints(), dims, p, x, out, saved, scratch, drop, s);
}
extern "C" int bf_temporal_bwd(const bf_dims* dims, const bf_temporal_params* p, const bf_temporal_params* g, const void* x, const void* dout,
                               void* dx, void* saved, void* scratch, const float* drop, bf_stream_t s) {
    TrunkLinks& L = g_links.get();
    return temporal_bwd(L, L.take_hints(), dims, p, g, x, dout, dx, saved, scratch, drop, s);
}

static int prep_stages(TrunkLinks& L, const bf_dims* dims, int n, const int32_t* kinds, const void* const* params, void* const* saved,
                       const float* const* drop_mlp, bf_stream_t s) {
    D d; TRY(get_dims(dims, &d));
    BF_REQUIRE(n >= 1 && kinds && params && saved, "bf_prep_stages: bad arguments");
    if (d.dtype != BF_DTYPE_BF16) return 1;
    hipStream_t st = (hipStream_t)s;
    TRY(side_join_pending(L, st));
    for (int i0 = 0; i0 < n; i0 += PREP_BATCH) {
        PrepBatch b;
        memset(&b, 0, sizeof(b));
        const int m = std::min(PREP_BATCH, n - i0);
        for (int i = 0; i < m; ++i) {
            BF_REQUIRE(params[i0 + i] && saved[i0 + i] && (kinds[i0 + i] == 0 || kinds[i0 + i] == 1), "bf_prep_stages: bad stage entry");
            Cast4& j = b.j[i];
            if (kinds[i0 + i] == 0) {
                const bf_temporal_params* p = (const bf_temporal_params*)params[i0 + i];
                TemporalSaved sv(d, saved[i0 + i]);
// ... 118 lines not shown
    }
    TRY(bf_in_stats_apply(d.dtype, sv.z, (int)d.F, (int)d.S, d.E, p->mlp_norm_w, p->mlp_norm_b, g3, g3div, nullptr, sv.mean3, sv.rstd3,
                          sv.sc3, sv.sh3, sc.in_ws, sv.x1, out, st));
    return 0;
}

static int spatial_bwd(TrunkLinks& L, const StageHints& H, const bf_dims* dims, const bf_spatial_params* p, const bf_spatial_params* g, const void* x,
                       const void* dout, void* dx, void* saved, void* scratch, const float* drop_att, const float* drop_mlp, bf_stream_t s) {
    D d; TRY(get_dims(dims, &d));
    BF_REQUIRE(p && g && x && dout && dx && saved && scratch, "bf_spatial_bwd: null pointer");
    hipStream_t st = (hipStream_t)s;
    SpatialSaved sv(d, saved);
    Scratch sc(d, bwd_scratch(L, d, scratch));
    const bool f32 = d.dtype == BF_DTYPE_F32;
    const void* win_c = f32 ? (const void*)p->input_head_w : sv.win_c;
    const void* w1_c = f32 ? (const void*)p->fc1_w : sv.w1_c;
    const void* w2_c = f32 ? (const void*)p->fc2_w : sv.w2_c;
    TRY(flush_pending_reduce(L, st));
    Fork fk(L, st, true, L.scratch_parity);
    if (fk.deferred) TRY(side_join_pending(L, st, fk.set));
    void* dz = sc.t1;
    ReduceJobs jobs;
    const TrunkLinks::TailDone td = L.tail_done;
    L.tail_done = TrunkLinks::TailDone{};
    const bool tail_done = td.saved == saved && td.dx == dout && td.st == st;
    {
        const float* gsc = drop_mlp ? sv.gtab : p->gamma_mlp;
        const int gdiv = drop_mlp ? 1 : (int)d.F;
        if (!tail_done)
            TRY(bf_in_bwd_partials(d.dtype, dout, sv.z, nullptr, dz, (int)d.F, (int)d.S, d.E, sv.mean3, sv.rstd3, p->mlp_norm_w, p->mlp_norm_b, gsc, gdiv, 0, sc.in_ws3, st));
        TRY(jobs.push(InReduceJob{tail_done ? td.ws : sc.in_ws3, (int)d.F, d.E, p->mlp_norm_w, p->mlp_norm_b, gsc, gdiv, g->mlp_norm_w, g->mlp_norm_b,
                                  drop_mlp ? nullptr : g->gamma_mlp, nullptr, drop_mlp, drop_mlp ? g->gamma_mlp : nullptr}));
    }
    void* dpre = sc.t4;
    {
        bf_epilogue e; memset(&e, 0, sizeof(e));
        e.aux_mode = BF_AUX_DGELU; e.aux = sv.pre; e.ld_aux = 4L * d.E; e.out_mode = BF_OUT_STORE;
        static const bool use_t = bf_knob("BF_FC2_DGRAD_T", 1) != 0;
        TRY(linear_bwd(d, sc, dz, d.E, sv.hid, 4 * d.E, BF_PRO_NONE, nullptr, nullptr, w2_c, g->fc2_w, g->fc2_b, dpre, &e, st, fk, nullptr, false,
                       (!f32 && use_t) ? sv.w2t_c : nullptr));
    }
    void* dx1 = sc.t1b;
    bool dbr_done = false;
    {
        bf_epilogue e; memset(&e, 0, sizeof(e));
        e.aux_mode = BF_AUX_ADD; e.aux = dout; e.ld_aux = d.E; e.out_mode = BF_OUT_STORE;
        TRY(linear_bwd(d, sc, dpre, 4 * d.E, sv.x1, d.E, BF_PRO_NONE, nullptr, nullptr, w1_c, g->fc1_w, g->fc1_b, dx1, &e, st, fk, nullptr, false, nullptr,
                       drop_att ? sc.e5 : nullptr, drop_att, (int)d.S, &dbr_done));
    }
    void* don = sc.e6;
    const void* dbr = dx1;
    if (dbr_done) dbr = sc.e5;
    else if (drop_att) {
        TRY(bf_frame_scale(d.dtype, dx1, drop_att, 1, sc.e5, d.N, (int)d.S, d.E, st));
        dbr = sc.e5;
    }
    void* dO = sc.e7;
    const InFuse fu2{sv.o, nullptr, dO, sv.mean2, sv.rstd2, p->norm2_w, p->norm2_b, sc.in_ws2};
    TRY(outproj_bwd(d, sc, dbr, sv.on, sv.wout_s, p->output_head_w, p->output_head_b, p->norm2_b, p->gamma_att,
                    d.feat_scale ? p->low_freq_scalar : nullptr, d.feat_scale ? p->high_freq_scalar : nullptr, sv.alpha, sv.mc,
                    g->output_head_w, g->output_head_b, g->norm2_b, g->gamma_att, d.feat_scale ? g->low_freq_scalar : nullptr,
                    d.feat_scale ? g->high_freq_scalar : nullptr, don, st, fk, &fu2));
    TRY(jobs.push(InReduceJob{sc.in_ws2, (int)d.F, d.E, p->norm2_w, p->norm2_b, nullptr, 1, g->norm2_w, g->norm2_b, nullptr, nullptr, nullptr, nullptr}));
    void* dqkv = sc.t3;
    {
        int rows = 0;
        static const bool raw_on = bf_knob("BF_ATTN_RAW", 1) != 0;
        const bool rawm = raw_on && bf_attn_raw_modes(d.dtype, d.d);
        TRY(bf_attn_bwd_partials(d.dtype, sv.qkv, dO, dqkv, d.F * d.h, d.w, 1, d.w, 0, 1, d.heads, d.d, p->qnorm_w, p->qnorm_b, p->knorm_w, p->knorm_b,
                                 p->rel_pos_emb, d.attn_scale ? p->attn_scale_factor_x : nullptr, g->qnorm_w, g->qnorm_b, g->knorm_w, g->knorm_b,
                                 g->rel_pos_emb, d.attn_scale ? g->attn_scale_factor_x : nullptr, 0.5f, rawm ? 2 : 0, sc.attn_ws, Scratch::ATTN_WS_FLOATS, &rows, st));
        TRY(jobs.push(AttnReduceJob{sc.attn_ws, rows, d.d, d.heads, g->qnorm_w, g->qnorm_b, g->knorm_w, g->knorm_b, g->rel_pos_emb,
                                    d.attn_scale ? g->attn_scale_factor_x : nullptr}));
        TRY(bf_attn_bwd_partials(d.dtype, sv.qkv, dO, dqkv, d.F * d.w, d.h, d.w, d.S, 1, d.w, d.heads, d.d, p->qnorm_w, p->qnorm_b, p->knorm_w, p->knorm_b,
                                 p->rel_pos_emb, d.attn_scale ? p->attn_scale_factor_y : nullptr, g->qnorm_w, g->qnorm_b, g->knorm_w, g->knorm_b,
                                 g->rel_pos_emb, d.attn_scale ? g->attn_scale_factor_y : nullptr, 0.5f, rawm ? 5 : 1, sc.attn_ws2, Scratch::ATTN_WS_FLOATS, &rows, st));
        TRY(jobs.push(AttnReduceJob{sc.attn_ws2, rows, d.d, d.heads, g->qnorm_w, g->qnorm_b, g->knorm_w, g->knorm_b, g->rel_pos_emb,
                                    d.attn_scale ? g->attn_scale_factor_y : nullptr}));
    }
    void* dxn = sc.e6;
    InFuse fu1{x, dx1, dx, sv.mean1, sv.rstd1, p->norm1_w, p->norm1_b, sc.in_ws};
    bool scaled_done = false;
    const NextScale& ns = H.scale;
    L.dbr_ready = TrunkLinks::DbrReady{};
    static const bool scaled_on = bf_knob("BF_BWD_SCALED_COPY", 1) != 0;
    if (ns.f && scaled_on && fk.deferred && d.dtype == BF_DTYPE_BF16) {
        fu1.scaled_out = (char*)scratch + 2 * Scratch(d, nullptr).bytes + (L.dbr_flip ? dbr_bytes(d) : 0);
        fu1.scaled_f = ns.f; fu1.scaled_fdiv = ns.fdiv; fu1.scaled_done = &scaled_done;
    }
    TRY(linear_bwd(d, sc, dqkv, 3 * d.E, sv.xn, d.E, BF_PRO_NONE, nullptr, nullptr, win_c, g->input_head_w, g->input_head_b, dxn, nullptr, st, fk, &fu1, true));
    if (scaled_done) { L.dbr_ready = {dx, ns.f, fu1.scaled_out, st}; L.dbr_flip = !L.dbr_flip; }
    TRY(jobs.push(InReduceJob{sc.in_ws, (int)d.F, d.E, p->norm1_w, p->norm1_b, nullptr, 1, g->norm1_w, g->norm1_b, nullptr, nullptr, nullptr, nullptr}));
    static const bool merge_on = bf_knob("BF_REDUCE_MERGE", 1) != 0;
    if (fk.deferred && merge_on) { L.reduce.jobs = jobs; L.reduce.on = true; L.reduce.st = st; }
    else TRY(launch_reduce_jobs(jobs, st));
    return fk.join();
}
extern "C" int bf_spatial_fwd(const bf_dims* dims, const bf_spatial_params* p, const void* x, void* out, void* saved, void* scratch,
                              const float* drop_att, const float* drop_mlp, bf_stream_t s) {
    TrunkLinks& L = g_links.get();
    return spatial_fwd(L, L.take_hints(), dims, p, x, out, saved, scratch, drop_att, drop_mlp, s);
}
extern "C" int bf_spatial_bwd(const bf_dims* dims, const bf_spatial_params* p, const bf_spatial_params* g, const void* x, const void* dout,
                              void* dx, void* saved, void* scratch, const float* drop_att, const float* drop_mlp, bf_stream_t s) {
    TrunkLinks& L = g_links.get();
    return spatial_bwd(L, L.take_hints(), dims, p, g, x, dout, dx, saved, scratch, drop_att, drop_mlp, s);
}

extern "C" int bf_trunk_train_fwd(const bf_dims* dims, int n, const int32_t* kinds, const void* const* params, void* const* saved,
                                  const float* const* drop_a, const float* const* drop_b, const void* x, void* const* acts, void* scratch,
                                  bf_stream_t s) {
    D d; TRY(get_dims(dims, &d));
    BF_REQUIRE(n >= 1 && kinds && params && saved && x && acts && scratch, "bf_trunk_train_fwd: bad arguments");
    for (int i = 0; i < n; ++i)
        BF_REQUIRE(params[i] && saved[i] && acts[i] && (kinds[i] == 0 || kinds[i] == 1), "bf_trunk_train_fwd: bad stage entry");
    TrunkLinks& L = g_links.get();
    (void)L.take_hints();
    const bool b16 = d.dtype == BF_DTYPE_BF16;
    if (b16) {
        const int rc = prep_stages(L, dims, n, kinds, params, saved, drop_b, s);
        if (rc < 0) return rc;
    }
    for (int i = 0; i < n; ++i) {
// ... 620 lines not shown
```

bubbleformer_amd/ops.py:

```python
import collections
import ctypes as C
import os
from typing import List, Optional, Sequence

import torch

from . import _lib as L

_SCRATCH = {}


def _require_gpu(t: torch.Tensor) -> None:
    if not t.is_cuda:
        raise L.BubbleformerHipError(
            "bubbleformer_amd runs only on a ROCm GPU (gfx950): got a tensor on %s; there is no CPU fallback" % t.device)


def _dt(t: torch.dtype) -> int:
    if t == torch.float32:
        return L.BF_DTYPE_F32
    if t == torch.bfloat16:
        return L.BF_DTYPE_BF16
    raise L.BubbleformerHipError(f"unsupported compute dtype {t}")

# ... 369 lines not shown
        ctx.mask = [p is not None for p in params]
        return out

    @staticmethod
    def backward(ctx, dout):
        x, saved, *ps = ctx.saved_tensors
        it = iter(ps)
        params = [next(it) if m else None for m in ctx.mask]
        heads, attn_scale, feat_scale = ctx.cfg
        B, T, h, w, E = x.shape
        d = make_dims(x.dtype, B, T, h, w, E, heads, attn_scale, feat_scale)
        lib = L.lib()
        dout = dout.contiguous()
        gviews, ret, direct = _stage_grads(params)
        if ctx.kind == "temporal":
            st, gs, bwd = L.TemporalParams(*[_p(p) for p in params]), L.TemporalParams(*[_p(g) for g in gviews]), lib.bf_temporal_bwd
        else:
            st, gs, bwd = L.SpatialParams(*[_p(p) for p in params]), L.SpatialParams(*[_p(g) for g in gviews]), lib.bf_spatial_bwd
        dx = torch.empty_like(x)
        drop_a, drop_b = ctx.drops
        if ctx.kind == "temporal":
            ps = getattr(ctx, "prev_spatial", None)
            if ps is not None and direct:
                L.check(lib.bf_stage_chain_tail(C.byref(ps[0]), _p(ps[1]), 1 if ps[2] else 0), "bf_stage_chain_tail")
            rc = bwd(C.byref(d), C.byref(st), C.byref(gs), _p(x), _p(dout), _p(dx), _p(saved), _p(scratch_for(d, x.device)), _p(drop_a), _stream())
        else:
            ns = getattr(ctx, "next_scale", None)
            if ns is not None and direct:
                lib.bf_stage_next_scale(_p(ns[0]), ns[1])
            rc = bwd(C.byref(d), C.byref(st), C.byref(gs), _p(x), _p(dout), _p(dx), _p(saved), _p(scratch_for(d, x.device)), _p(drop_a),
                     _p(drop_b), _stream())
        L.check(rc, f"bf_{ctx.kind}_bwd")
        if _DEFER["on"]:
            _DEFER["keep"].append((saved, dout, x))
        _stage_done(params, direct)
        return (dx, None, None, None, None, None, None, *ret)


class _TrunkFn(torch.autograd.Function):

    @staticmethod
    def forward(ctx, x, cfg, kinds, masks, drops, *flat):
        _require_gpu(x)
        heads, attn_scale, feat_scale = cfg
        x = x.contiguous()
        B, T, h, w, E = x.shape
        d = make_dims(x.dtype, B, T, h, w, E, heads, attn_scale, feat_scale)
        lib = L.lib()
        n = len(kinds)
        it = iter(flat)
        plist = [[_f32c(next(it)) if m else None for m in mask] for mask in masks]
        for kind, ps in zip(kinds, plist):
            _check_stage_params(kind, ps, E, heads, x.device)
        structs = [(L.TemporalParams if kind == "temporal" else L.SpatialParams)(*[_p(p) for p in ps]) for kind, ps in zip(kinds, plist)]
        kinds_c = (C.c_int32 * n)(*[0 if k == "temporal" else 1 for k in kinds])
        pp = (C.c_void_p * n)(*[C.addressof(s) for s in structs])
        nb = {"temporal": lib.bf_temporal_saved_bytes(C.byref(d)), "spatial": lib.bf_spatial_saved_bytes(C.byref(d))}
        if min(nb.values()) < 0:
            L.check(-1, "bf_*_saved_bytes")
        offs, total = [], 0
        for k in kinds:
            offs.append(total)
            total += (nb[k] + 255) // 256 * 256
        arena = torch.empty(total, dtype=torch.uint8, device=x.device)
        sp = (C.c_void_p * n)(*[arena.data_ptr() + o for o in offs])
        acts = torch.empty((max(n - 1, 1),) + tuple(x.shape), dtype=x.dtype, device=x.device)
        out = torch.empty_like(x)
# ... 28 lines not shown
            rets.append(ret)
            directs.append(direct)
        kinds_c = (C.c_int32 * n)(*[0 if k == "temporal" else 1 for k in kinds])
        pp = (C.c_void_p * n)(*[C.addressof(s) for s in pstructs])
        gp = (C.c_void_p * n)(*[C.addressof(s) for s in gstructs])
        sp = (C.c_void_p * n)(*[arena.data_ptr() + o for o in ctx.offs])
        ap = (C.c_void_p * n)(*([acts[i].data_ptr() for i in range(n - 1)] + [None]))
        da, db = ctx.drops
        dap = (C.c_void_p * n)(*[_p(t) for t in da])
        dbp = (C.c_void_p * n)(*[_p(t) for t in db])
        dout = dout.contiguous()
        gbuf = torch.empty((3,) + tuple(x.shape), dtype=x.dtype, device=x.device)
        g3 = (C.c_void_p * 3)(*[gbuf[i].data_ptr() for i in range(3)])
        dx = torch.empty_like(x)
        on_ready = _DIRECT["on_ready"]
        errs = []

        def done(i, _user):
            try:
                if directs[i] and on_ready is not None:
                    on_ready([p.data_ptr() for p in plist[i] if p is not None])
            except BaseException as e:
                errs.append(e)

        cb = L.STAGE_DONE_FN(done)
        rc = lib.bf_trunk_train_bwd(C.byref(d), n, kinds_c, pp, gp, sp, dap, dbp, _p(x), ap, _p(dout), g3, _p(dx), _p(scratch_for(d, x.device)),
                                    C.cast(cb, C.c_void_p), None, _stream())
        L.check(rc, "bf_trunk_train_bwd")
        if errs:
            raise errs[0]
        if not all(directs):
            L.check(lib.bf_side_join(_stream()), "bf_side_join")
        if _DEFER["on"]:
            _DEFER["keep"].append((arena, acts, dout, x, gbuf))
        flat_ret = [g for ret, mask in zip(rets, masks) for g, m in zip(ret, mask) if m]
        return (dx, None, None, None, None, *flat_ret)


def trunk_train(tok: torch.Tensor, heads: int, attn_scale: bool, feat_scale: bool, stages) -> Optional[torch.Tensor]:
    if not tok.is_cuda or not stages or os.environ.get("BF_TRUNK_NATIVE", "1") == "0" or os.environ.get("BF_STAGE_CHAIN", "1") == "0":
        return None
    if tok.dim() != 5:
        raise L.BubbleformerHipError("trunk_train: tokens must be (B, T, h, w, E)")
    kinds = tuple(k for k, _, _ in stages)
    masks = tuple(tuple(p is not None for p in ps) for _, ps, _ in stages)
    flat = [p for _, ps, _ in stages for p in ps if p is not None]
    drops = [dr for _, _, dr in stages]
    return _TrunkFn.apply(tok, (heads, bool(attn_scale), bool(feat_scale)), kinds, masks, drops, *flat)


def temporal_block(x: torch.Tensor, heads: int, attn_scale: bool, params: List[Optional[torch.Tensor]], drop=None) -> torch.Tensor:
    return _BlockFn.apply(x, "temporal", heads, attn_scale, True, drop, None, *params)


def spatial_block(x: torch.Tensor, heads: int, attn_scale: bool, feat_scale: bool, params: List[Optional[torch.Tensor]], drop_att=None,
                  drop_mlp=None) -> torch.Tensor:
    return _BlockFn.apply(x, "spatial", heads, attn_scale, feat_scale, drop_att, drop_mlp, *params)


def drop_path_factors(n: int, drop_prob: float, device) -> torch.Tensor:
    keep = 1.0 - drop_prob
    return torch.empty(n, dtype=torch.float32, device=device).bernoulli_(keep).div_(keep)


def _stage_arrays(conv, inw, inb):
    n = L.BF_MAX_STAGES
    arr = lambda xs: (L.fp * n)(*([_p(t) for t in xs] + [None] * (n - len(xs))))
# ... 1076 lines not shown
```

include/bubbleformer_hip.h:

```cpp
#ifndef BUBBLEFORMER_HIP_H
#define BUBBLEFORMER_HIP_H

#include <stdint.h>

#ifdef __cplusplus
extern "C" {
#endif

typedef void* bf_stream_t;

enum { BF_DTYPE_F32 = 0, BF_DTYPE_BF16 = 1 };

enum { BF_LAY_KC = 0,
       BF_LAY_XC = 1   };
enum { BF_PRO_NONE = 0, BF_PRO_AFFINE = 1, BF_PRO_AFFINE_GELU = 2, BF_PRO_GELU = 3 };
enum { BF_AUX_NONE = 0, BF_AUX_ADD = 1 , BF_AUX_DGELU = 2  };
enum { BF_OUT_STORE = 0 , BF_OUT_ATOMIC_F32 = 2 ,
       BF_OUT_STORE_F32 = 1  };

typedef struct bf_operand {
    const void* p;
    int64_t ld;
    int32_t layout;
    int32_t seglen;
// ... 21 lines not shown
    int32_t gw, gh, gc;
    void* gelu_out;
    float* colsum;
    const float* rowscale;
    int32_t rows_per_group;
} bf_epilogue;

int bf_gemm(int dtype, int M, int N, int K, const bf_operand* A, const bf_operand* B, const bf_epilogue* E,
            int splitk, bf_stream_t stream);

int bf_gemm_inbwd_frames(int dtype, int M, int N, int K, const void* A, int64_t lda, const void* B, int64_t ldb, const void* x,
                         const void* add, void* out, int S, const float* mean, const float* rstd, const float* w, float* ws,
                         const float* fscale , int fdiv,
                         bf_stream_t stream);
int bf_gemm_inbwd_frames_chain(int dtype, int M, int N, int K, const void* A, int64_t lda, const void* B, int64_t ldb, const void* x,
                               const void* add, void* out, int S, const float* mean, const float* rstd, const float* w, float* ws,
                               const float* fscale, int fdiv, const void* cz, void* cdz, const float* cmean, const float* crstd,
                               const float* cw, const float* cg, int cgdiv, float* cws, bf_stream_t stream);

typedef struct bf_frame_norm {
    const float *w, *b;
    const float* g; int32_t gdiv;
    float *mean, *rstd, *sc, *sh;
    const void* resid;
    void* out;
} bf_frame_norm;
int bf_gemm_fwd_frames(int dtype, int M, int N, int K, const void* A, int64_t lda, const void* Bt, int64_t ldb, const float* bias,
                       const float* colscale, const float* colshift, const float* fscale, int fdiv, const void* add, void* out, int S,
                       const bf_frame_norm* n1, const bf_frame_norm* n2, bf_stream_t stream);

int bf_gemm_tokred(int dtype, int Nout, int Kin, int64_t M, const void* dy, int64_t ldy, const void* x, int64_t ldx, float* out,
                   int accumulate, float* colsum, float* ws, int64_t ws_floats, bf_stream_t stream);
int64_t bf_gemm_tokred_ws_floats(int Nout, int Kin, int64_t M);

int bf_frame_linear(int dtype, int frames, int S, int K, int N, const void* A, int64_t lda, const void* W, int64_t ldw,
                    const float* norm_w, const float* norm_b, const float* bias, const float* colscale, const float* colshift,
                    const void* resid, int64_t ldr, int gelu, const float* en_w, const float* en_b, const float* en_g,
                    void* out, int64_t ldo,
                    const float* next_w, const float* next_b, void* out_n, int64_t ldn,
                    bf_stream_t stream);


int bf_in_stats(int dtype, const void* x, int frames, int S, int C, const float* w, const float* b, const float* g, int gdiv,
                const float* gb, float* mean, float* rstd, float* sc, float* sh,
                float* ws ,
                bf_stream_t stream);
int64_t bf_in_ws_floats(int dtype, int frames, int S, int C);
int bf_affine_apply(int dtype, const void* z, const void* resid, const float* sc, const float* sh, void* out, int64_t nrows,
                    int S, int C, bf_stream_t stream);
int bf_in_bwd(int dtype, const void* dy, const void* x, const void* add, void* dx, int frames, int S, int C, const float* mean,
              const float* rstd, const float* w, const float* b, const float* g, int gdiv, int gelu, float* dw, float* db,
              float* dg, float* dgb, float* ws ,
              bf_stream_t stream);
int bf_colsum(int dtype, const void* x, int64_t nrows, int C, const float* scale, float* out, bf_stream_t stream);

int bf_attn_fwd(int dtype, const void* qkv, void* out, int64_t nseq, int L, int64_t inner, int64_t outer_stride,
                int64_t inner_stride, int64_t tok_stride, int heads, int d, const float* qw, const float* qb, const float* kw,
                const float* kb, const float* emb, const float* hscale, float out_scale, int accumulate, bf_stream_t stream);
int bf_attn_axial_fwd(int dtype, const void* qkv, void* out, int64_t frames, int h, int w, int heads, int d, const float* qw,
                      const float* qb, const float* kw, const float* kb, const float* emb, const float* hscale_x,
                      const float* hscale_y, bf_stream_t stream);
int bf_attn_axial_norm_fwd(int dtype, const void* qkv, void* out, void* out_n, int64_t frames, int h, int w, int heads, int d,
                           const float* qw, const float* qb, const float* kw, const float* kb, const float* emb, const float* hscale_x,
                           const float* hscale_y, const float* norm_w, const float* norm_b, float* mean, float* rstd, float* sc,
                           float* sh, bf_stream_t stream);
int bf_attn_bwd(int dtype, const void* qkv, const void* dout, void* dqkv, int64_t nseq, int L, int64_t inner,
                int64_t outer_stride, int64_t inner_stride, int64_t tok_stride, int heads, int d, const float* qw,
                const float* qb, const float* kw, const float* kb, const float* emb, const float* hscale, float* dqw,
                float* dqb, float* dkw, float* dkb, float* demb, float* dhscale, float out_scale, int accumulate,
                float* ws, int64_t ws_floats,
                bf_stream_t stream);

void bf_side_defer(int on);
int bf_side_join(bf_stream_t stream);
void bf_debug_force_generic_attn(int on);
void bf_debug_tokred_fold(int on);

int bf_im2col_nchw(int dtype, const float* x, void* out, int frames, int C, int H, int W, int Kp, bf_stream_t stream);
int bf_col2im_nchw(int dtype, const void* g, float* dx, int frames, int C, int H, int W, int Kp, bf_stream_t stream);
#define BF_LOSS_LIMBS 5
int bf_pm2nchw(const float* pm, float* pred, const float* y, float* lossbuf, int frames, int Co, int h, int w, int Np,
               bf_stream_t stream);
int bf_debed_last(int dtype, const void* act, const float* sc, const float* sh, const void* wc, float* pred, const float* y,
                  float* lossbuf, int frames, int Ci, int Co, int h, int w, int Np, bf_stream_t stream);
int bf_debed_last_bwd(int dtype, const float* dpred, const float* pred, const float* y, const float* coef, const float* gscale,
                      const void* wc, void* dpm, void* dact, int frames, int Ci, int Co, int h, int w, int Np, bf_stream_t stream);
int bf_debed_last_bwd_norm(int dtype, const float* dpred, const float* pred, const float* y, const float* coef, const float* gscale,
                           const void* wc, void* dpm, const void* ymap, const float* mean, const float* rstd, const float* in_w,
                           const float* in_b, void* dx, float* d_in_w, float* d_in_b, int frames, int Ci, int Co, int h, int w, int Np,
                           float* ws, int64_t ws_floats, bf_stream_t stream);
int bf_embed_first(int dtype, const float* x, const void* wc, void* patches, void* y0, int frames, int C0, int cin, int h2, int w2,
                   int Kp, float* stat_part, bf_stream_t stream);
int bf_in_stats_merge_slices(int dtype, int frames, int S, int C, int rows, const float* w, const float* b, const float* g, int gdiv,
                             const float* gb, float* mean, float* rstd, float* sc, float* sh, float* ws, bf_stream_t stream);
int bf_gather_gemm(int dtype, const void* map, const void* w, int w_kn, const float* sc, const float* sh, void* out, int frames, int gh,
                   int gw, int C0, int N, bf_stream_t stream);
int bf_scatter_gemm(int dtype, const void* a, const void* w, int w_kn, const float* sc, const float* sh, void* map, float* stat_part, int frames,
                    int gh, int gw, int K, int C0, bf_stream_t stream);
int64_t bf_gather_wgrad_ws_floats(int frames, int gh, int gw);
int bf_gather_wgrad(int dtype, const void* fine, const void* coarse, const float* fsc, const float* fsh, const float* csc, const float* csh,
                    float* out, int transposed, int frames, int gh, int gw, int C0, int Kc, float* ws, int64_t ws_floats, bf_stream_t stream);
int bf_gather_gemm_rebuilt(int dtype, const void* patches, const void* w0c, const void* w, int w_kn, const float* sc, const float* sh, void* out,
                           int frames, int gh, int gw, int C0, int N, bf_stream_t stream);
int bf_gather_wgrad_rebuilt(int dtype, const void* patches, const void* w0c, const void* coarse, const float* fsc, const float* fsh, float* out,
                            int transposed, int frames, int gh, int gw, int C0, int Kc, float* ws, int64_t ws_floats, bf_stream_t stream);
int64_t bf_embed_tail_ws_floats(int frames, int gh1, int gw1, int C0, int Kp);
int bf_embed_tail_bwd(int dtype, const void* dy1, const void* w1c, const void* y0, const void* patches, const void* w0c, const float* sc,
                      const float* sh, const float* mean, const float* rstd, const float* in_w, float* dwprep, float* d_in_w, float* d_in_b,
                      int frames, int gh1, int gw1, int C1, int C0, int Kp, float* ws, int64_t ws_floats, bf_stream_t stream);
// ... 186 lines not shown
```

Baseline: 821.8 samples/s.

## Skip backward work for drop-path-dropped sample groups in attention and weight-grad

Adds a per-group liveness table, taken from the stochastic-depth drop masks, to the attention backward kernel and the token-reduction weight-gradient GEMMs. The kernel compacts live groups into an order table in shared memory, runs attention backward only over live sequences, and zero-fills the dqkv rows of dropped groups. Samples whose branch was dropped contribute zero gradient, so their backward FLOPs are wasted. The cost is extra indirection, extra kernel variants and plumbing of the masks through the backward path, and the drop tensors are now kept alive in deferred mode.

```diff
diff --git a/bubbleformer_amd/_lib.py b/bubbleformer_amd/_lib.py
--- a/bubbleformer_amd/_lib.py
+++ b/bubbleformer_amd/_lib.py
@@ -80,6 +80,7 @@
     "bf_prof_enable": (None, [C.c_int]),
     "bf_debug_force_generic_attn": (None, [C.c_int]),
     "bf_debug_tokred_fold": (None, [C.c_int]),
+    "bf_debug_drop_skip": (None, [C.c_int]),
     "bf_side_defer": (None, [C.c_int]),
     "bf_prep_stages": (C.c_int, [C.POINTER(Dims), C.c_int, C.POINTER(C.c_int32), C.POINTER(vp), C.POINTER(vp), C.POINTER(vp), vp]),
     "bf_stage_prepared": (None, [C.c_int]),
@@ -103,6 +104,9 @@
     "bf_gemm": (C.c_int, [C.c_int, C.c_int, C.c_int, C.c_int, P(Operand), P(Operand), P(Epilogue), C.c_int, vp]),
     "bf_gemm_tokred": (C.c_int, [C.c_int, C.c_int, C.c_int, i64, vp, i64, vp, i64, fp, C.c_int, fp, fp, i64, vp]),
     "bf_gemm_tokred_ws_floats": (i64, [C.c_int, C.c_int, i64]),
+    "bf_gemm_tokred_live": (C.c_int, [C.c_int, C.c_int, C.c_int, i64, vp, i64, vp, i64, fp, C.c_int, fp, fp, i64, fp, C.c_int, C.c_int, vp]),
+    "bf_gemm_tokred_deferred_live": (C.c_int, [C.c_int, C.c_int, C.c_int, i64, vp, i64, vp, i64, fp, C.c_int, fp, fp, i64, fp, C.c_int, C.c_int, vp]),
+    "bf_gemm_tokred_flush_on": (C.c_int, [vp]),
     "bf_gemm_inbwd_frames": (C.c_int, [C.c_int, C.c_int, C.c_int, C.c_int, vp, i64, vp, i64, vp, vp, vp, C.c_int, fp, fp, fp, fp, fp, C.c_int, vp]),
     "bf_gemm_inbwd_frames_chain": (C.c_int, [C.c_int, C.c_int, C.c_int, C.c_int, vp, i64, vp, i64, vp, vp, vp, C.c_int, fp, fp, fp, fp, fp, C.c_int,
                                              vp, vp, fp, fp, fp, fp, C.c_int, fp, vp]),
@@ -119,6 +123,8 @@
                               C.c_int, vp]),
     "bf_attn_bwd": (C.c_int, [C.c_int, vp, vp, vp, i64, C.c_int, i64, i64, i64, i64, C.c_int, C.c_int, fp, fp, fp, fp, fp, fp,
                               fp, fp, fp, fp, fp, fp, f32, C.c_int, fp, i64, vp]),
+    "bf_attn_bwd_live": (C.c_int, [C.c_int, vp, vp, vp, i64, C.c_int, i64, i64, i64, i64, C.c_int, C.c_int, fp, fp, fp, fp, fp, fp,
+                                   fp, fp, fp, fp, fp, fp, f32, C.c_int, fp, i64, fp, C.c_int, vp]),
     "bf_im2col_nchw": (C.c_int, [C.c_int, fp, vp, C.c_int, C.c_int, C.c_int, C.c_int, C.c_int, vp]),
     "bf_col2im_nchw": (C.c_int, [C.c_int, vp, fp, C.c_int, C.c_int, C.c_int, C.c_int, C.c_int, vp]),
     "bf_pm2nchw": (C.c_int, [fp, fp, fp, fp, C.c_int, C.c_int, C.c_int, C.c_int, C.c_int, vp]),
diff --git a/bubbleformer_amd/csrc/attn.hip b/bubbleformer_amd/csrc/attn.hip
--- a/bubbleformer_amd/csrc/attn.hip
+++ b/bubbleformer_amd/csrc/attn.hip
@@ -363,7 +363,7 @@
 int bf_attn_bwd_mfma(const void* qkv, const void* dout, void* dqkv, long nseq, int L, long inner, long outer_stride, long inner_stride,
                      long tok_stride, int heads, int d, const float* qw, const float* qb, const float* kw, const float* kb, const float* emb,
                      const float* hscale, float* dqw, float* dqb, float* dkw, float* dkb, float* demb, float* dhscale, float out_scale,
-                     int accumulate, float* ws, long ws_floats, int* rows_out, hipStream_t st);
+                     int accumulate, float* ws, long ws_floats, int* rows_out, hipStream_t st, BfLive live);
 int bf_attn_fwd_long(int dtype, const void* qkv, void* out, long nseq, int L, long inner, long outer_stride, long inner_stride, long tok_stride,
                      int heads, int d, const float* qw, const float* qb, const float* kw, const float* kb, const float* emb, const float* hscale,
                      float out_scale, int accumulate, hipStream_t st);
@@ -444,8 +444,10 @@
                          int64_t outer_stride, int64_t inner_stride, int64_t tok_stride, int heads, int d, const float* qw,
                          const float* qb, const float* kw, const float* kb, const float* emb, const float* hscale,
                          float* dqw, float* dqb, float* dkw, float* dkb, float* demb, float* dhscale, float out_scale,
-                         int accumulate, float* ws, int64_t ws_floats, int* rows_out, bf_stream_t stream) {
+                         int accumulate, float* ws, int64_t ws_floats, int* rows_out, bf_stream_t stream, BfLive live = BfLive{}) {
     if (rows_out) *rows_out = 0;
+    if (live.tab) BF_REQUIRE(live.group > 0 && nseq % live.group == 0, "bf_attn_bwd: nseq must be whole groups of seqs_per_group sequences");
+    if (live.tab && nseq / live.group > BF_LIVE_MAX_GROUPS) live = BfLive{};
     BF_REQUIRE(qkv && dout && dqkv && qw && qb && kw && kb && nseq > 0 && inner > 0, "bf_attn_bwd: bad arguments");
     if (int rc = check_geo("bf_attn_bwd", dtype, heads, d, L)) return rc;
     BF_REQUIRE(accumulate == 0 || accumulate == 1 || ((accumulate == 2 || accumulate == 5) && use_mfma(dtype, d)),
@@ -458,7 +460,7 @@
     if (use_mfma(dtype, d)) {
         BfProfScope prof((hipStream_t)stream, "attn_bwd", 10.0 * nseq * heads * L * L * d, (double)nseq * heads * L * d * 2.0 * (accumulate ? 10.0 : 7.0));
         return bf_attn_bwd_mfma(qkv, dout, dqkv, nseq, L, inner, outer_stride, inner_stride, tok_stride, heads, d, qw, qb, kw, kb, emb, hscale, dqw,
-                                dqb, dkw, dkb, demb, dhscale, out_scale, accumulate, ws, (long)ws_floats, rows_out, (hipStream_t)stream);
+                                dqb, dkw, dkb, demb, dhscale, out_scale, accumulate, ws, (long)ws_floats, rows_out, (hipStream_t)stream, live);
     }
     SeqGeo g{nseq, L, inner, outer_stride, inner_stride, tok_stride};
     AttnParams p{qw, qb, kw, kb, emb, hscale};
@@ -493,10 +495,18 @@
     return attn_bwd_impl(dtype, qkv, dout, dqkv, nseq, L, inner, outer_stride, inner_stride, tok_stride, heads, d, qw, qb, kw, kb, emb, hscale, dqw,
                          dqb, dkw, dkb, demb, dhscale, out_scale, accumulate, ws, ws_floats, nullptr, stream);
 }
+extern "C" int bf_attn_bwd_live(int dtype, const void* qkv, const void* dout, void* dqkv, int64_t nseq, int L, int64_t inner,
+                                int64_t outer_stride, int64_t inner_stride, int64_t tok_stride, int heads, int d, const float* qw,
+                                const float* qb, const float* kw, const float* kb, const float* emb, const float* hscale,
+                                float* dqw, float* dqb, float* dkw, float* dkb, float* demb, float* dhscale, float out_scale,
+                                int accumulate, float* ws, int64_t ws_floats, const float* live, int seqs_per_group, bf_stream_t stream) {
+    return attn_bwd_impl(dtype, qkv, dout, dqkv, nseq, L, inner, outer_stride, inner_stride, tok_stride, heads, d, qw, qb, kw, kb, emb, hscale, dqw,
+                         dqb, dkw, dkb, demb, dhscale, out_scale, accumulate, ws, ws_floats, nullptr, stream, BfLive{live, seqs_per_group});
+}
 int bf_attn_bwd_partials(int dtype, const void* qkv, const void* dout, void* dqkv, int64_t nseq, int L, int64_t inner, int64_t outer_stride,
                          int64_t inner_stride, int64_t tok_stride, int heads, int d, const float* qw, const float* qb, const float* kw,
                          const float* kb, const float* emb, const float* hscale, float* dqw, float* dqb, float* dkw, float* dkb, float* demb,
-                         float* dhscale, float out_scale, int accumulate, float* ws, int64_t ws_floats, int* rows, hipStream_t stream) {
+                         float* dhscale, float out_scale, int accumulate, float* ws, int64_t ws_floats, int* rows, hipStream_t stream, BfLive live) {
     return attn_bwd_impl(dtype, qkv, dout, dqkv, nseq, L, inner, outer_stride, inner_stride, tok_stride, heads, d, qw, qb, kw, kb, emb, hscale, dqw,
-                         dqb, dkw, dkb, demb, dhscale, out_scale, accumulate, ws, ws_floats, rows, (bf_stream_t)stream);
-}
+                         dqb, dkw, dkb, demb, dhscale, out_scale, accumulate, ws, ws_floats, rows, (bf_stream_t)stream, live);
+}
diff --git a/bubbleformer_amd/csrc/attn_mfma.hip b/bubbleformer_amd/csrc/attn_mfma.hip
--- a/bubbleformer_amd/csrc/attn_mfma.hip
+++ b/bubbleformer_amd/csrc/attn_mfma.hip
@@ -42,9 +42,14 @@
 
 struct Geo { long nseq; int L; long inner, outer_stride, inner_stride, tok_stride; };
 struct Prob { long tok0; int head; };
-__device__ __forceinline__ Prob locate(const Geo& g, int heads, long pr) {
+__device__ __forceinline__ Prob locate(const Geo& g, int heads, long pr, const unsigned char* order = nullptr, int spg = 1) {
     const unsigned p = (unsigned)pr, hd = (unsigned)heads, inner = (unsigned)g.inner;
-    const unsigned s = p / hd, head = p - s * hd;
+    unsigned s = p / hd;
+    const unsigned head = p - s * hd;
+    if (order) {
+        const unsigned gi = s / (unsigned)spg;
+        s = (unsigned)__builtin_amdgcn_readfirstlane((int)order[gi]) * (unsigned)spg + (s - gi * (unsigned)spg);
+    }
     const unsigned q = s / inner, r = s - q * inner;
     return Prob{(long)q * g.outer_stride + (long)r * g.inner_stride, (int)head};
 }
@@ -553,7 +558,7 @@
 
 template <int NB, int KS, int ACC>
 __global__ void __launch_bounds__(256, ((NB == 1 && KS <= 2) ? 2 : 1)) attn_bwd_mfma(const bf16* __restrict__ qkv, const bf16* __restrict__ dout, bf16* __restrict__ dqkv, Geo g,
-                                                     int heads, Par p, Grd gr, float out_scale, int accumulate_rt, float* __restrict__ ws) {
+                                                     int heads, Par p, Grd gr, float out_scale, int accumulate_rt, float* __restrict__ ws, BfLive live) {
     constexpr int D = 32 * KS, LD = D + 16, NT16 = D / 16, R = 16 * NB, LDP = 32 + 8;
     constexpr bool PREFETCH = NB * KS <= 4;
     extern __shared__ __attribute__((aligned(16))) bf16 smem_bwd[];
@@ -562,7 +567,16 @@
     __shared__ __attribute__((aligned(16))) float s_par[4 * 32 * KS];
     __shared__ float s_emb[32 * 16];
     __shared__ float s_hsc[16];
+    __shared__ unsigned char s_order[BF_LIVE_MAX_GROUPS];
     const int lane = threadIdx.x & 63, wave = __builtin_amdgcn_readfirstlane(threadIdx.x >> 6), wpb = blockDim.x >> 6;
+    int ngroups = 0, nlive = 0;
+    float tab_lo = 0.f, tab_hi = 0.f;
+    if (live.tab) {
+        ngroups = (int)(g.nseq / live.group);
+        if (lane < ngroups) tab_lo = live.tab[lane];
+        if (lane + 64 < ngroups) tab_hi = live.tab[lane + 64];
+    }
+    const unsigned char* order = live.tab ? s_order : nullptr;
     constexpr int PER_WAVE = 3 * R * LD + 2 * R * LDP;
     static_assert(3 * R * LD * 2 >= 4 * D * 4, "the parameter-gradient flush must fit in the operand tiles");
     bf16* qn_t = smem_bwd + wave * PER_WAVE;
@@ -581,10 +595,21 @@
         const int q = i / D, e = i % D;
         s_par[i] = (q == 0 ? p.qw : q == 1 ? p.qb : q == 2 ? p.kw : p.kb)[e];
     }
+    if (live.tab) {
+        const unsigned long long lo = __ballot(tab_lo != 0.f), hi = __ballot(tab_hi != 0.f);
+        nlive = __popcll(lo) + __popcll(hi);
+        const int t = threadIdx.x;
+        if (t < ngroups) {
+            const unsigned long long below = t < 64 ? (1ull << t) - 1ull : ~0ull, below_hi = t < 64 ? 0ull : (1ull << (t - 64)) - 1ull;
+            const int rank = __popcll(lo & below) + __popcll(hi & below_hi);
+            const bool on = ((t < 64 ? lo >> t : hi >> (t - 64)) & 1ull) != 0;
+            s_order[on ? rank : nlive + (t - rank)] = (unsigned char)t;
+        }
+    }
     __syncthreads();
     const int E = heads * D, L = g.L;
     const float scale = rsqrtf((float)D);
-    const long nprob = g.nseq * heads;
+    const long nprob = (live.tab ? (long)nlive * live.group : g.nseq) * heads;
     const int gq = lane >> 4, i16 = lane & 15;
     const int mode = ACC >= 0 ? ACC : accumulate_rt;
     const bool raw_out = mode & 2, raw_in = mode & 4, accumulate = mode & 1;
@@ -604,7 +629,7 @@
             for (int r = 0; r < 4; ++r) a_emb[jb][ib][r] = 0.f;
     long pr = (long)blockIdx.x * wpb + wave;
     RawRows<NB, KS> cur, nxt;
-    Prob at = locate(g, heads, pr < nprob ? pr : 0), at_next = at;
+    Prob at = locate(g, heads, pr < nprob ? pr : 0, order, live.group), at_next = at;
     if (pr < nprob) load_raw<NB, KS>(cur, qkv, dout, g, heads, at, lane);
     if (PREFETCH) drain_vm();
     float mk[NB][NB][4], mneg[NB][NB][4];
@@ -617,7 +642,7 @@
         const int head = at.head;
         const long tok0 = at.tok0;
         const bool more = pr + pstep < nprob;
-        if (more) at_next = locate(g, heads, pr + pstep);
+        if (more) at_next = locate(g, heads, pr + pstep, order, live.group);
         if (PREFETCH && more) load_raw<NB, KS>(nxt, qkv, dout, g, heads, at_next, lane);
         OldRows<NB, KS> old;
         if (accumulate) {
@@ -833,6 +858,17 @@
         if (PREFETCH) cur = nxt;
         else if (more) load_raw<NB, KS>(cur, qkv, dout, g, heads, at_next, lane);
         at = at_next;
+    }
+    if (live.tab && (!accumulate || raw_in)) {
+        const long nrows = (long)(ngroups - nlive) * live.group * L;
+        const bf16x8 z8 = {};
+        for (long it = (long)blockIdx.x * wpb + wave; it < nrows; it += pstep) {
+            const unsigned sq = (unsigned)(it / L), i = (unsigned)(it - (long)sq * L), gi = sq / (unsigned)live.group;
+            const unsigned s = (unsigned)__builtin_amdgcn_readfirstlane((int)s_order[nlive + gi]) * (unsigned)live.group + (sq - gi * (unsigned)live.group);
+            const unsigned q = s / (unsigned)g.inner, r = s - q * (unsigned)g.inner;
+            bf16* row = dqkv + ((long)q * g.outer_stride + (long)r * g.inner_stride + (long)i * g.tok_stride) * 3L * E;
+            for (int c = lane; c < 3 * E / 8; c += 64) *reinterpret_cast<bf16x8*>(row + 8 * c) = z8;
+        }
     }
     if (one_head && pr - pstep >= 0) {
         const int head = (int)(((long)blockIdx.x * wpb + wave) % heads);
@@ -900,7 +936,7 @@
 }
 template <int NB, int KS, int ACC>
 int go_bwd_mode(const bf16* qkv, const bf16* dout, bf16* dqkv, Geo g, int heads, Par p, Grd gr, float out_scale, int accumulate, float* ws,
-                long ws_floats, int* rows_out, hipStream_t st) {
+                long ws_floats, int* rows_out, hipStream_t st, BfLive live) {
     constexpr int D = 32 * KS, R = 16 * NB;
     const int wpb = NB == 1 ? 4 : 2;
     const size_t shm = (size_t)wpb * (3 * R * (D + 16) + 2 * R * 40) * sizeof(bf16);
@@ -926,7 +962,7 @@
         if (grid >= 8 * m) grid -= grid % m;
     }
     if (ws && ws_floats < grid * nvals) { grid = ws_floats / nvals; if (grid < 1) ws = nullptr; }
-    hipLaunchKernelGGL((attn_bwd_mfma<NB, KS, ACC>), dim3((int)grid), dim3(wpb * 64), shm, st, qkv, dout, dqkv, g, heads, p, gr, out_scale, accumulate, ws);
+    hipLaunchKernelGGL((attn_bwd_mfma<NB, KS, ACC>), dim3((int)grid), dim3(wpb * 64), shm, st, qkv, dout, dqkv, g, heads, p, gr, out_scale, accumulate, ws, live);
     BF_CHECK_LAUNCH();
     if (rows_out) { *rows_out = ws ? (int)grid : 0; return 0; }
     if (ws) {
@@ -938,8 +974,8 @@
 }
 template <int NB, int KS>
 int go_bwd(const bf16* qkv, const bf16* dout, bf16* dqkv, Geo g, int heads, Par p, Grd gr, float out_scale, int accumulate, float* ws,
-           long ws_floats, int* rows_out, hipStream_t st) {
-#define BF_MODE(A) return go_bwd_mode<NB, KS, A>(qkv, dout, dqkv, g, heads, p, gr, out_scale, accumulate, ws, ws_floats, rows_out, st)
+           long ws_floats, int* rows_out, hipStream_t st, BfLive live) {
+#define BF_MODE(A) return go_bwd_mode<NB, KS, A>(qkv, dout, dqkv, g, heads, p, gr, out_scale, accumulate, ws, ws_floats, rows_out, st, live)
     if constexpr (NB == 1 && KS == 2) {
         switch (accumulate) { case 0: BF_MODE(0); case 1: BF_MODE(1); case 2: BF_MODE(2); case 5: BF_MODE(5); default: break; }
     }
@@ -988,12 +1024,12 @@
 int bf_attn_bwd_mfma(const void* qkv, const void* dout, void* dqkv, long nseq, int L, long inner, long outer_stride, long inner_stride,
                      long tok_stride, int heads, int d, const float* qw, const float* qb, const float* kw, const float* kb, const float* emb,
                      const float* hscale, float* dqw, float* dqb, float* dkw, float* dkb, float* demb, float* dhscale, float out_scale,
-                     int accumulate, float* ws, long ws_floats, int* rows_out, hipStream_t st) {
+                     int accumulate, float* ws, long ws_floats, int* rows_out, hipStream_t st, BfLive live) {
     Geo g{nseq, L, inner, outer_stride, inner_stride, tok_stride};
     Par p{qw, qb, kw, kb, emb, hscale};
     Grd gr{dqw, dqb, dkw, dkb, demb, dhscale};
     const int nb = L <= 16 ? 1 : 2, ks = d / 32;
-#define GO(NB, KS) if (nb == NB && ks == KS) return go_bwd<NB, KS>((const bf16*)qkv, (const bf16*)dout, (bf16*)dqkv, g, heads, p, gr, out_scale, accumulate, ws, ws_floats, rows_out, st)
+#define GO(NB, KS) if (nb == NB && ks == KS) return go_bwd<NB, KS>((const bf16*)qkv, (const bf16*)dout, (bf16*)dqkv, g, heads, p, gr, out_scale, accumulate, ws, ws_floats, rows_out, st, live)
     GO(1, 1); GO(1, 2); GO(1, 3); GO(1, 4); GO(2, 1); GO(2, 2); GO(2, 3); GO(2, 4);
 #undef GO
     return bf_fail_msg("bf_attn_bwd_mfma: unsupported shape", __FILE__, __LINE__);
diff --git a/bubbleformer_amd/csrc/bf_common.h b/bubbleformer_amd/csrc/bf_common.h
--- a/bubbleformer_amd/csrc/bf_common.h
+++ b/bubbleformer_amd/csrc/bf_common.h
@@ -33,12 +33,15 @@
     ~BfProfScope() { if (idx >= 0) bf_prof_end(idx, st, name, flops, bytes); }
 };
 
+struct BfLive { const float* tab = nullptr; int group = 0; };
+constexpr int BF_LIVE_MAX_GROUPS = 128;
 int bf_in_bwd_partials(int dtype, const void* dy, const void* x, const void* add, void* dx, int frames, int S, int C, const float* mean,
                        const float* rstd, const float* w, const float* b, const float* g, int gdiv, int gelu, float* ws, hipStream_t stream);
 int bf_attn_bwd_partials(int dtype, const void* qkv, const void* dout, void* dqkv, int64_t nseq, int L, int64_t inner, int64_t outer_stride,
                          int64_t inner_stride, int64_t tok_stride, int heads, int d, const float* qw, const float* qb, const float* kw,
                          const float* kb, const float* emb, const float* hscale, float* dqw, float* dqb, float* dkw, float* dkb, float* demb,
-                         float* dhscale, float out_scale, int accumulate, float* ws, int64_t ws_floats, int* rows, hipStream_t stream);
+                         float* dhscale, float out_scale, int accumulate, float* ws, int64_t ws_floats, int* rows, hipStream_t stream,
+                         BfLive live = BfLive{});
 int bf_in_stats_apply(int dtype, const void* x, int frames, int S, int C, const float* w, const float* b, const float* g, int gdiv, const float* gb,
                       float* mean, float* rstd, float* sc, float* sh, float* ws, const void* resid, void* out, hipStream_t stream);
 int bf_in_stats_apply_chain(int dtype, const void* x, int frames, int S, int C, const float* w, const float* b, const float* g, int gdiv, const float* gb,
diff --git a/bubbleformer_amd/csrc/gemm_tokred.hip b/bubbleformer_amd/csrc/gemm_tokred.hip
--- a/bubbleformer_amd/csrc/gemm_tokred.hip
+++ b/bubbleformer_amd/csrc/gemm_tokred.hip
@@ -31,10 +31,39 @@
     return __builtin_bit_cast(bf16x8, r);
 }
 
-template <int NI, int GRP>
+struct LiveSet { unsigned long long lo, hi; int rpg; };
+constexpr int NO_GROUP = 128;
+__device__ uint4 g_zero_row[64];
+__device__ __forceinline__ int nth_live(const LiveSet& s, int k) {
+    unsigned long long m = s.lo;
+    int base = 0;
+    const int pl = __popcll(s.lo);
+    if (k >= pl) { k -= pl; m = s.hi; base = 64; }
+    if (k >= __popcll(m)) return NO_GROUP;
+    int pos = 0;
+#pragma unroll
+    for (int w = 32; w > 0; w >>= 1) {
+        const int c = __popcll((m >> pos) & ((1ull << w) - 1ull));
+        if (k >= c) { k -= c; pos += w; }
+    }
+    return base + pos;
+}
+__device__ __forceinline__ int next_live(const LiveSet& s, int g) {
+    if (g >= NO_GROUP - 1) return NO_GROUP;
+    const int n = g + 1;
+    if (n < 64) {
+        const unsigned long long m = s.lo >> n;
+        if (m) return n + __builtin_ctzll(m);
+    }
+    const int n2 = n < 64 ? 64 : n;
+    const unsigned long long m2 = s.hi >> (n2 - 64);
+    return m2 ? n2 + __builtin_ctzll(m2) : NO_GROUP;
+}
+
+template <int NI, int GRP, bool LIVE>
 __device__ __forceinline__ void tokred_pp_body(const bf16* __restrict__ A, long lda, const bf16* __restrict__ B, long ldb,
                                                float* __restrict__ slab_tile, float* __restrict__ cslab_row, int nh, bool do_cs,
-                                               unsigned ring_lds, int lane, int w4) {
+                                               unsigned ring_lds, int lane, int w4, const LiveSet& live, int c_beg, const bf16* zr) {
     using Gm = PPGeom<NI>;
     constexpr int HALFB = Gm::HALFB;
     constexpr int PG = NI == 6 ? (GRP == 0 ? 5 : 4) : 3;
@@ -45,7 +74,37 @@
     const int dch = (lane & 7) ^ (dkey << 1);
     const bf16* pA = A + (long)dr * lda + 8 * dch;
     const bf16* pB = B + (long)dr * ldb + 8 * dch;
-    const long stepA = (long)HR * lda, stepB = (long)HR * ldb;
+    const long stepA = LIVE ? 0L : (long)HR * lda, stepB = LIVE ? 0L : (long)HR * ldb;
+    const unsigned voA = (unsigned)(((long)(lane >> 3) * lda + 8 * dch) * 2), voB = (unsigned)(((long)(lane >> 3) * ldb + 8 * dch) * 2);
+    const unsigned voZ = (unsigned)(16 * dch);
+    int lg = 0, lw = 0;
+    long stA = (long)HR * lda, stB = (long)HR * ldb;
+    auto to_pad = [&]() {
+        pA = reinterpret_cast<const bf16*>(reinterpret_cast<const char*>(zr) + voZ);
+        pB = pA;
+        stA = stB = 0;
+    };
+    auto advance = [&]() {
+        lw += HR;
+        if (lw >= live.rpg) {
+            lw -= live.rpg;
+            const int nx = next_live(live, lg);
+            if (nx >= NO_GROUP) to_pad();
+            else { const long skip = (long)(nx - lg - 1) * live.rpg; pA += stA + skip * lda; pB += stB + skip * ldb; }
+            lg = nx;
+        } else { pA += stA; pB += stB; }
+    };
+    if constexpr (LIVE) {
+        const int c = c_beg + 8 * w4, gi = c / live.rpg;
+        lw = c - gi * live.rpg;
+        lg = nth_live(live, gi);
+        if (lg >= NO_GROUP) to_pad();
+        else {
+            const long row = (long)lg * live.rpg + lw;
+            pA = reinterpret_cast<const bf16*>(reinterpret_cast<const char*>(A + row * lda) + voA);
+            pB = reinterpret_cast<const bf16*>(reinterpret_cast<const char*>(B + row * ldb) + voB);
+        }
+    }
     auto issue = [&](int buf) {
         const unsigned base = __builtin_amdgcn_readfirstlane(ring_lds + (unsigned)buf * (unsigned)HALFB + (unsigned)w4 * 1024u);
         if constexpr (NI == 6 && GRP == 0) {
@@ -84,8 +143,11 @@
     for (int c = 0; c < 8; ++c) ones[c] = (bf16)1.0f;
 
     issue(0);
+    if constexpr (LIVE) advance();
     if (nh > 1) issue(1);
+    if constexpr (LIVE) advance();
     if (nh > 2) issue(2);
+    if constexpr (LIVE) advance();
     if (nh > 2) wait_vm<2 * PG>(); else if (nh > 1) wait_vm<PG>(); else wait_vm<0>();
     __builtin_amdgcn_s_barrier();
     if constexpr (GRP == 1) __builtin_amdgcn_s_barrier();
@@ -104,6 +166,7 @@
         asm volatile("s_waitcnt lgkmcnt(0)" ::: "memory");
         __builtin_amdgcn_sched_barrier(0);
         __builtin_amdgcn_s_barrier();
+        if constexpr (LIVE) advance();
 #pragma unroll
         for (int i = 0; i < NI; ++i)
 #pragma unroll
@@ -173,10 +236,11 @@
         }
 }
 
-template <int NI>
-__global__ void __launch_bounds__(512) tokred_pp_kernel(const bf16* __restrict__ A, long lda, const bf16* __restrict__ B, long ldb,
-                                                      float* __restrict__ slab, float* __restrict__ cslab, int Nout, int halves_total,
-                                                      int halves_per, int tiles_k, int ntiles, int main_wgs, FoldRed red) {
+template <int NI, bool LIVE>
+__device__ __forceinline__ void tokred_pp_main(const bf16* __restrict__ A, long lda, const bf16* __restrict__ B, long ldb,
+                                               float* __restrict__ slab, float* __restrict__ cslab, int Nout, int halves_total,
+                                               int halves_per, int tiles_k, int ntiles, int main_wgs, const FoldRed& red,
+                                               const float* __restrict__ tab, int ngroups, int rpg, const bf16* zrow) {
     using Gm = PPGeom<NI>;
     extern __shared__ __attribute__((aligned(16))) char smem[];
     if ((int)blockIdx.x >= main_wgs) { fold_reduce<NI>(red, (int)blockIdx.x - main_wgs); return; }
@@ -184,16 +248,49 @@
     const int seq = xcd_remap(blockIdx.x, main_wgs);
     const int slice = seq / ntiles, tile = seq - slice * ntiles;
     const int n0 = (tile / tiles_k) * Gm::TM, c0 = (tile % tiles_k) * PTN;
-    const int h_beg = slice * halves_per;
-    const int nh = min(halves_per, halves_total - h_beg);
-    const bf16* a0 = A + (long)h_beg * HR * lda + n0;
-    const bf16* b0 = B + (long)h_beg * HR * ldb + c0;
+    int h_beg = slice * halves_per;
+    int nh = min(halves_per, halves_total - h_beg);
+    LiveSet live{~0ull, ~0ull, rpg};
+    if constexpr (LIVE) {
+        const bool l0 = lane < ngroups && (tab == nullptr || tab[lane] != 0.f);
+        const bool l1 = lane + 64 < ngroups && (tab == nullptr || tab[lane + 64] != 0.f);
+        live.lo = __ballot(l0);
+        live.hi = __ballot(l1);
+        const int nlive = __popcll(live.lo) + __popcll(live.hi);
+        const int lhalves = (int)(((long)nlive * rpg + HR - 1) / HR);
+        const int nslice = main_wgs / ntiles;
+        const int lper = (lhalves + nslice - 1) / nslice;
+        h_beg = slice * lper;
+        nh = min(lper, lhalves - h_beg);
+    }
     float* slab_tile = slab + ((size_t)slice * ntiles + tile) * Gm::TILE_FLOATS;
     const bool do_cs = cslab != nullptr && c0 == 0;
     float* cslab_row = do_cs ? cslab + (size_t)slice * Nout + n0 : nullptr;
+    if constexpr (LIVE) {
+        if (nh <= 0) {
+            for (int e = tid; e < Gm::TILE_FLOATS / 4; e += 512) reinterpret_cast<float4*>(slab_tile)[e] = make_float4(0.f, 0.f, 0.f, 0.f);
+            if (do_cs) for (int e = tid; e < Gm::TM; e += 512) cslab_row[e] = 0.f;
+            return;
+        }
+    }
+    const bf16* a0 = A + (LIVE ? 0L : (long)h_beg * HR * lda) + n0;
+    const bf16* b0 = B + (LIVE ? 0L : (long)h_beg * HR * ldb) + c0;
     const unsigned ring_lds = lds_addr(smem);
-    if (wave < 4) tokred_pp_body<NI, 0>(a0, lda, b0, ldb, slab_tile, cslab_row, nh, do_cs, ring_lds, lane, wave);
-    else tokred_pp_body<NI, 1>(a0, lda, b0, ldb, slab_tile, cslab_row, nh, do_cs, ring_lds, lane, wave - 4);
+    if (wave < 4) tokred_pp_body<NI, 0, LIVE>(a0, lda, b0, ldb, slab_tile, cslab_row, nh, do_cs, ring_lds, lane, wave, live, h_beg * HR, zrow);
+    else tokred_pp_body<NI, 1, LIVE>(a0, lda, b0, ldb, slab_tile, cslab_row, nh, do_cs, ring_lds, lane, wave - 4, live, h_beg * HR, zrow);
+}
+template <int NI>
+__global__ void __launch_bounds__(512) tokred_pp_kernel(const bf16* __restrict__ A, long lda, const bf16* __restrict__ B, long ldb,
+                                                      float* __restrict__ slab, float* __restrict__ cslab, int Nout, int halves_total,
+                                                      int halves_per, int tiles_k, int ntiles, int main_wgs, FoldRed red) {
+    tokred_pp_main<NI, false>(A, lda, B, ldb, slab, cslab, Nout, halves_total, halves_per, tiles_k, ntiles, main_wgs, red, nullptr, 1, 0, nullptr);
+}
+template <int NI>
+__global__ void __launch_bounds__(512) tokred_pp_live_kernel(const bf16* __restrict__ A, long lda, const bf16* __restrict__ B, long ldb,
+                                                           float* __restrict__ slab, float* __restrict__ cslab, int Nout, int halves_total,
+                                                           int halves_per, int tiles_k, int ntiles, int main_wgs, FoldRed red,
+                                                           const float* __restrict__ tab, int ngroups, int rpg, const bf16* zrow) {
+    tokred_pp_main<NI, true>(A, lda, B, ldb, slab, cslab, Nout, halves_total, halves_per, tiles_k, ntiles, main_wgs, red, tab, ngroups, rpg, zrow);
 }
 
 template <int NI, int MAXS>
@@ -471,8 +568,9 @@
 PendingRed& pending_slot() { int dev = 0; (void)hipGetDevice(&dev); return g_pending[(dev >= 0 && dev < 64) ? dev : 0]; }
 constexpr int FOLD_WGS = 40;
 }
+struct LiveArg { bool entry = false; const float* tab = nullptr; int rpg = 0; int tile_rows = 0; };
 static int tokred_impl(int dtype, int Nout, int Kin, int64_t M, const void* dy, int64_t ldy, const void* x, int64_t ldx, float* out,
-                       int accumulate, float* colsum, float* ws, int64_t ws_floats, bool defer, bf_stream_t stream);
+                       int accumulate, float* colsum, float* ws, int64_t ws_floats, bool defer, bf_stream_t stream, LiveArg lv = LiveArg{});
 static int flush_pending(PendingRed& p, hipStream_t caller) {
     if (!p.on) return 0;
     p.on = false;
@@ -501,20 +599,43 @@
 bool bf_gemm_tokred_pending() { return pending_slot().on; }
 const float* bf_gemm_tokred_pending_out() { const PendingRed& p = pending_slot(); return p.on ? p.r.out : nullptr; }
 int bf_gemm_tokred_deferred(int dtype, int Nout, int Kin, int64_t M, const void* dy, int64_t ldy, const void* x, int64_t ldx, float* out,
-                            int accumulate, float* colsum, float* ws, int64_t ws_floats, hipStream_t stream) {
-    return tokred_impl(dtype, Nout, Kin, M, dy, ldy, x, ldx, out, accumulate, colsum, ws, ws_floats, true, (bf_stream_t)stream);
+                            int accumulate, float* colsum, float* ws, int64_t ws_floats, hipStream_t stream, BfLive live) {
+    return tokred_impl(dtype, Nout, Kin, M, dy, ldy, x, ldx, out, accumulate, colsum, ws, ws_floats, true, (bf_stream_t)stream,
+                       LiveArg{live.tab != nullptr, live.tab, live.group, 0});
 }
 extern "C" int bf_gemm_tokred(int dtype, int Nout, int Kin, int64_t M, const void* dy, int64_t ldy, const void* x, int64_t ldx, float* out,
                               int accumulate, float* colsum, float* ws, int64_t ws_floats, bf_stream_t stream) {
     return tokred_impl(dtype, Nout, Kin, M, dy, ldy, x, ldx, out, accumulate, colsum, ws, ws_floats, false, stream);
 }
+extern "C" int bf_gemm_tokred_live(int dtype, int Nout, int Kin, int64_t M, const void* dy, int64_t ldy, const void* x, int64_t ldx, float* out,
+                                   int accumulate, float* colsum, float* ws, int64_t ws_floats, const float* live, int rows_per_group,
+                                   int tile_rows, bf_stream_t stream) {
+    return tokred_impl(dtype, Nout, Kin, M, dy, ldy, x, ldx, out, accumulate, colsum, ws, ws_floats, false, stream, LiveArg{true, live, rows_per_group, tile_rows});
+}
+extern "C" int bf_gemm_tokred_deferred_live(int dtype, int Nout, int Kin, int64_t M, const void* dy, int64_t ldy, const void* x, int64_t ldx,
+                                            float* out, int accumulate, float* colsum, float* ws, int64_t ws_floats, const float* live,
+                                            int rows_per_group, int tile_rows, bf_stream_t stream) {
+    return tokred_impl(dtype, Nout, Kin, M, dy, ldy, x, ldx, out, accumulate, colsum, ws, ws_floats, true, stream, LiveArg{true, live, rows_per_group, tile_rows});
+}
+extern "C" int bf_gemm_tokred_flush_on(bf_stream_t stream) { return bf_gemm_tokred_flush((hipStream_t)stream); }
 static int tokred_impl(int dtype, int Nout, int Kin, int64_t M, const void* dy, int64_t ldy, const void* x, int64_t ldx, float* out,
-                       int accumulate, float* colsum, float* ws, int64_t ws_floats, bool defer, bf_stream_t stream) {
+                       int accumulate, float* colsum, float* ws, int64_t ws_floats, bool defer, bf_stream_t stream, LiveArg lv) {
     if (dtype != BF_DTYPE_BF16) return 1;
     static const int skip_env = bf_knob("BF_TOKRED_SKIP", 0);
     if (skip_env) return 0;
-    const bool pp = Nout % 192 == 0 && Kin % PTN == 0 && M % HR == 0 && M >= 4 * HR;
-    if (!pp && (Nout % TB || Kin % TB || M % BK || M < BK)) return 1;
+    const bool pp = Nout % 192 == 0 && Kin % PTN == 0 && (M % HR == 0 || lv.entry) && M >= 4 * HR;
+    if (!pp && (lv.tab || Nout % TB || Kin % TB || M % BK || M < BK)) return 1;
+    const bool use_live = pp && (lv.tab || M % HR != 0);
+    int ngroups = 1, rpg = (int)M;
+    if (use_live) {
+        BF_REQUIRE(M < (1L << 31) - HR, "bf_gemm_tokred: the live-group form indexes rows with 31 bits");
+        if (lv.tab) {
+            BF_REQUIRE(lv.rpg > 0 && M % lv.rpg == 0 && M / lv.rpg <= 128, "bf_gemm_tokred: a live table covers at most 128 groups of rows_per_group rows, M in all");
+            ngroups = (int)(M / lv.rpg); rpg = lv.rpg;
+        }
+        if (rpg % 8 || rpg < HR) return 1;
+
+    }
     if (ldy % 8 || ldx % 8) return 1;
     BF_REQUIRE(dy && x && out && ws, "bf_gemm_tokred: null pointer");
     BF_REQUIRE(((uintptr_t)dy & 15) == 0 && ((uintptr_t)x & 15) == 0 && ((uintptr_t)out & 15) == 0 && ((uintptr_t)ws & 15) == 0,
@@ -526,9 +647,11 @@
     static const int tile_env = bf_knob("BF_TOKRED_TILE", 0);
     static const int wgs_env = bf_knob("BF_TOKRED_WGS", 128);
     if (pp) {
-        const long halves = M / HR;
+        const long halves = (M + HR - 1) / HR;
         const int tiles_k0 = Kin / PTN;
-        const bool big = Nout % 384 == 0 && tile_env == 384;
+        const int tile_want = lv.tile_rows ? lv.tile_rows : tile_env;
+        BF_REQUIRE(lv.tile_rows == 0 || lv.tile_rows == 192 || (lv.tile_rows == 384 && Nout % 384 == 0), "bf_gemm_tokred: tile_rows is 0, 192 or 384 (Nout a multiple of it)");
+        const bool big = Nout % 384 == 0 && tile_want == 384;
         const int tm = big ? 384 : 192;
         int nslice = slices_env > 0 ? slices_env : std::max(1, wgs_env / ((Nout / tm) * tiles_k0));
         nslice = (int)std::max<long>(1, std::min<long>({(long)nslice, (long)MAX_SLICES, halves / 4}));
@@ -550,7 +673,7 @@
         static const int fold_wgs = bf_knob("BF_TOKRED_FOLD_WGS", FOLD_WGS);
         if (fold && pend.on) { red = pend.r; red.nwg = fold_wgs; }
         const unsigned extra = red.nwg > 0 ? (unsigned)red.nwg : 0u;
-#define BF_PP_GO(NIV)                                                                                                                     \
+#define BF_PP_GO(NIV, KERN, ...)                                                                                                                   \
         do {                                                                                                                              \
             {                                                                                                                             \
                 BfProfScope prof(st, NIV == 6 ? "tokred_pp_kernel<384x192,h32,ring4>" : "tokred_pp_kernel<192x192,h32,ring4>",           \
@@ -558,12 +681,12 @@
                 static BfPerDeviceOnce attr_once; bool& attr_done = attr_once.flag();                                                                                            \
                 constexpr int lds_bytes = NBUF * PPGeom<NIV>::HALFB;                                                                      \
                 if (!attr_done) {                                                                                                         \
-                    hipError_t e_ = hipFuncSetAttribute((const void*)tokred_pp_kernel<NIV>, hipFuncAttributeMaxDynamicSharedMemorySize, lds_bytes); \
+                    hipError_t e_ = hipFuncSetAttribute((const void*)KERN<NIV>, hipFuncAttributeMaxDynamicSharedMemorySize, lds_bytes); \
                     if (e_ != hipSuccess) return bf_fail(e_, __FILE__, __LINE__);                                                         \
                     attr_done = true;                                                                                                     \
                 }                                                                                                                         \
-                hipLaunchKernelGGL(tokred_pp_kernel<NIV>, dim3((unsigned)(ns * ntiles) + extra), dim3(512), lds_bytes, st, (const bf16*)dy, (long)ldy, \
-                                   (const bf16*)x, (long)ldx, slab, cslab, Nout, (int)halves, halves_per, tiles_k, ntiles, ns * ntiles, red); \
+                hipLaunchKernelGGL(KERN<NIV>, dim3((unsigned)(ns * ntiles) + extra), dim3(512), lds_bytes, st, (const bf16*)dy, (long)ldy, \
+                                   (const bf16*)x, (long)ldx, slab, cslab, Nout, (int)halves, halves_per, tiles_k, ntiles, ns * ntiles, red __VA_ARGS__); \
                 BF_CHECK_LAUNCH();                                                                                                        \
             }                                                                                                                             \
             if (fold) {                                                                                                                   \
@@ -576,7 +699,17 @@
             else hipLaunchKernelGGL((tokred_pp_reduce_kernel<NIV, MAX_SLICES>), dim3(rblocks), dim3(256), 0, st, slab, cslab, ns, ntiles, tiles_k, Nout, Kin, out, colsum, accumulate); \
             BF_CHECK_LAUNCH();                                                                                                            \
         } while (0)
-        if (big) BF_PP_GO(6); else BF_PP_GO(3);
+        const bf16* zrow = nullptr;
+        if (use_live) {
+            static BfPerDevice<const bf16*> zrows;
+            const bf16*& z = zrows.get();
+            if (!z) { hipError_t e_ = hipGetSymbolAddress((void**)&z, HIP_SYMBOL(g_zero_row)); if (e_ != hipSuccess) return bf_fail(e_, __FILE__, __LINE__); }
+            zrow = z;
+        }
+#define BF_LIVE_ARGS , lv.tab, ngroups, rpg, zrow
+        if (use_live) { if (big) BF_PP_GO(6, tokred_pp_live_kernel, BF_LIVE_ARGS); else BF_PP_GO(3, tokred_pp_live_kernel, BF_LIVE_ARGS); }
+        else { if (big) BF_PP_GO(6, tokred_pp_kernel); else BF_PP_GO(3, tokred_pp_kernel); }
+#undef BF_LIVE_ARGS
 #undef BF_PP_GO
         return 0;
     }
diff --git a/bubbleformer_amd/csrc/model.hip b/bubbleformer_amd/csrc/model.hip
--- a/bubbleformer_amd/csrc/model.hip
+++ b/bubbleformer_amd/csrc/model.hip
@@ -7,7 +7,7 @@
 
 bool bf_attn_raw_modes(int dtype, int d);
 int bf_gemm_tokred_deferred(int dtype, int Nout, int Kin, int64_t M, const void* dy, int64_t ldy, const void* x, int64_t ldx, float* out,
-                            int accumulate, float* colsum, float* ws, int64_t ws_floats, hipStream_t stream);
+                            int accumulate, float* colsum, float* ws, int64_t ws_floats, hipStream_t stream, BfLive live);
 int bf_gemm_tokred_flush(hipStream_t st);
 bool bf_gemm_tokred_pending();
 const float* bf_gemm_tokred_pending_out();
@@ -582,6 +582,12 @@
     return 0;
 }
 
+bool g_drop_skip_off = false;
+BfLive live_groups(const D& d, const float* tab, long ngroups, long group) {
+    if (!tab || g_drop_skip_off || d.dtype != BF_DTYPE_BF16 || ngroups > BF_LIVE_MAX_GROUPS) return BfLive{};
+    return BfLive{tab, (int)group};
+}
+
 int qkv_gemm(const D& d, const void* xn, const void* w_c, const float* bias, void* qkv, hipStream_t st) {
     bf_operand A = op_plain(xn, d.E, BF_LAY_KC);
     bf_operand Bo = op_plain(w_c, d.E, BF_LAY_KC);
@@ -635,10 +641,10 @@
 int outproj_bwd(const D& d, const Scratch& sc, const void* dout, const void* on, const void* w_s,
                 const float* W, const float* bias, const float* nb, const float* gamma, const float* lo, const float* hi,
                 const float* alpha, const float* mc, float* dW, float* dbias, float* dnb, float* dgamma, float* dlo, float* dhi,
-                void* don, hipStream_t st, Fork& fk, const InFuse* fu = nullptr) {
+                void* don, hipStream_t st, Fork& fk, const InFuse* fu = nullptr, BfLive live = BfLive{}) {
     TRY(fk.run([=](hipStream_t ss) -> int {
         const void* dsrc = dout;
-        const int trc = bf_gemm_tokred_deferred(d.dtype, d.E, d.E, d.N, dsrc, d.E, on, d.E, sc.G, 0, sc.csum, sc.tokred_ws, sc.tokred_floats, ss);
+        const int trc = bf_gemm_tokred_deferred(d.dtype, d.E, d.E, d.N, dsrc, d.E, on, d.E, sc.G, 0, sc.csum, sc.tokred_ws, sc.tokred_floats, ss, live);
         if (trc < 0) return trc;
         if (trc == 1) {
             ZERO_ON(ss, sc.G, (size_t)((char*)sc.csum - (char*)sc.G) + (size_t)d.E * 4);
@@ -669,7 +675,7 @@
 int linear_bwd(const D& d, const Scratch& sc, const void* dy, int Nout, const void* x, int Kin, int xpro, const float* xsc, const float* xsh,
                const void* w_c, float* dW, float* db, void* dxn, const bf_epilogue* dx_epi, hipStream_t st, Fork& fk, const InFuse* fu = nullptr,
                bool last = false, const void* w_t = nullptr, void* scaled_out = nullptr, const float* rowfac = nullptr, int rpg = 1,
-               bool* scaled_done = nullptr) {
+               bool* scaled_done = nullptr, BfLive live = BfLive{}) {
     TRY(fk.run([=](hipStream_t ss) -> int {
         const void* xo = x;
         int pro = xpro;
@@ -681,7 +687,7 @@
         }
         bf_operand Bo = op_plain(xo, Kin, BF_LAY_XC);
         if (pro == BF_PRO_NONE) {
-            const int trc = bf_gemm_tokred_deferred(d.dtype, Nout, Kin, d.N, dy, Nout, xo, Kin, dW, 1, db, sc.tokred_ws, sc.tokred_floats, ss);
+            const int trc = bf_gemm_tokred_deferred(d.dtype, Nout, Kin, d.N, dy, Nout, xo, Kin, dW, 1, db, sc.tokred_ws, sc.tokred_floats, ss, live);
             if (trc <= 0) return trc;
         }
         if (pro != BF_PRO_NONE) op_affine(Bo, pro, xsc, xsh, d.S, Kin);
@@ -714,6 +720,7 @@
 extern "C" int64_t bf_scratch_bytes(const bf_dims* s) { D d; if (get_dims(s, &d)) return -1; return 2 * (int64_t)Scratch(d, nullptr).bytes + 2 * (int64_t)dbr_bytes(d); }
 
 extern "C" void bf_side_defer(int on) { g_side_defer = on != 0; }
+extern "C" void bf_debug_drop_skip(int on) { g_drop_skip_off = on == 0; }
 extern "C" int bf_side_join(bf_stream_t s) { return side_join_pending(g_links.get(), (hipStream_t)s); }
 
 extern "C" void bf_stage_prepared(int on) { g_links.get().hints.prepared = on != 0; }
@@ -806,8 +813,9 @@
     }
     L.dbr_ready = TrunkLinks::DbrReady{};
     const InFuse fu2{sv.o, nullptr, dO, sv.mean2, sv.rstd2, p->norm2_w, p->norm2_b, sc.in_ws2};
+    const BfLive live_tok = live_groups(d, drop, d.B, (long)d.T * d.S), live_seq = live_groups(d, drop, d.B, d.S);
     TRY(outproj_bwd(d, sc, dbr, sv.on, sv.wout_s, p->output_head_w, p->output_head_b, p->norm2_b, p->gamma, nullptr, nullptr,
-                    sv.alpha, sv.mc, g->output_head_w, g->output_head_b, nullptr, g->gamma, nullptr, nullptr, don, st, fk, &fu2));
+                    sv.alpha, sv.mc, g->output_head_w, g->output_head_b, nullptr, g->gamma, nullptr, nullptr, don, st, fk, &fu2, live_tok));
     ReduceJobs jobs;
     TRY(jobs.push(InReduceJob{sc.in_ws2, (int)d.F, d.E, p->norm2_w, p->norm2_b, nullptr, 1, g->norm2_w, g->norm2_b, nullptr, nullptr, nullptr, nullptr}));
     {
@@ -815,7 +823,7 @@
         TRY(bf_attn_bwd_partials(d.dtype, sv.qkv, dO, dqkv, (long)d.B * d.S, d.T, d.S, (long)d.T * d.S, 1, d.S, d.heads, d.d, p->qnorm_w, p->qnorm_b,
                                  p->knorm_w, p->knorm_b, p->rel_pos_emb, d.attn_scale ? p->attn_scale_factor : nullptr, g->qnorm_w, g->qnorm_b,
                                  g->knorm_w, g->knorm_b, g->rel_pos_emb, d.attn_scale ? g->attn_scale_factor : nullptr, 1.f, 0, sc.attn_ws,
-                                 Scratch::ATTN_WS_FLOATS, &rows, st));
+                                 Scratch::ATTN_WS_FLOATS, &rows, st, live_seq));
         TRY(jobs.push(AttnReduceJob{sc.attn_ws, rows, d.d, d.heads, g->qnorm_w, g->qnorm_b, g->knorm_w, g->knorm_b, g->rel_pos_emb,
                                     d.attn_scale ? g->attn_scale_factor : nullptr}));
     }
@@ -835,7 +843,8 @@
         fu1.tail = &tn;
     }
     if (H.tail.armed) L.tail_done = TrunkLinks::TailDone{};
-    TRY(linear_bwd(d, sc, dqkv, 3 * d.E, sv.xn, d.E, BF_PRO_NONE, nullptr, nullptr, win_c, g->input_head_w, g->input_head_b, dxn, nullptr, st, fk, &fu1, true));
+    TRY(linear_bwd(d, sc, dqkv, 3 * d.E, sv.xn, d.E, BF_PRO_NONE, nullptr, nullptr, win_c, g->input_head_w, g->input_head_b, dxn, nullptr, st, fk, &fu1, true,
+                   nullptr, nullptr, nullptr, 1, nullptr, live_tok));
     if (tail_done) L.tail_done = {H.tail.saved, dx, tn.ws, st};
     TRY(jobs.push(InReduceJob{sc.in_ws, (int)d.F, d.E, p->norm1_w, p->norm1_b, nullptr, 1, g->norm1_w, g->norm1_b, nullptr, nullptr, nullptr, nullptr}));
     TRY(launch_with_pending(L, jobs, st));
@@ -1020,13 +1029,14 @@
         TRY(jobs.push(InReduceJob{tail_done ? td.ws : sc.in_ws3, (int)d.F, d.E, p->mlp_norm_w, p->mlp_norm_b, gsc, gdiv, g->mlp_norm_w, g->mlp_norm_b,
                                   drop_mlp ? nullptr : g->gamma_mlp, nullptr, drop_mlp, drop_mlp ? g->gamma_mlp : nullptr}));
     }
+    const BfLive live_mlp = live_groups(d, drop_mlp, d.F, d.S), live_att = live_groups(d, drop_att, d.F, d.S);
     void* dpre = sc.t4;
     {
         bf_epilogue e; memset(&e, 0, sizeof(e));
         e.aux_mode = BF_AUX_DGELU; e.aux = sv.pre; e.ld_aux = 4L * d.E; e.out_mode = BF_OUT_STORE;
         static const bool use_t = bf_knob("BF_FC2_DGRAD_T", 1) != 0;
         TRY(linear_bwd(d, sc, dz, d.E, sv.hid, 4 * d.E, BF_PRO_NONE, nullptr, nullptr, w2_c, g->fc2_w, g->fc2_b, dpre, &e, st, fk, nullptr, false,
-                       (!f32 && use_t) ? sv.w2t_c : nullptr));
+                       (!f32 && use_t) ? sv.w2t_c : nullptr, nullptr, nullptr, 1, nullptr, live_mlp));
     }
     void* dx1 = sc.t1b;
     bool dbr_done = false;
@@ -1034,7 +1044,7 @@
         bf_epilogue e; memset(&e, 0, sizeof(e));
         e.aux_mode = BF_AUX_ADD; e.aux = dout; e.ld_aux = d.E; e.out_mode = BF_OUT_STORE;
         TRY(linear_bwd(d, sc, dpre, 4 * d.E, sv.x1, d.E, BF_PRO_NONE, nullptr, nullptr, w1_c, g->fc1_w, g->fc1_b, dx1, &e, st, fk, nullptr, false, nullptr,
-                       drop_att ? sc.e5 : nullptr, drop_att, (int)d.S, &dbr_done));
+                       drop_att ? sc.e5 : nullptr, drop_att, (int)d.S, &dbr_done, live_mlp));
     }
     void* don = sc.e6;
     const void* dbr = dx1;
@@ -1048,7 +1058,7 @@
     TRY(outproj_bwd(d, sc, dbr, sv.on, sv.wout_s, p->output_head_w, p->output_head_b, p->norm2_b, p->gamma_att,
                     d.feat_scale ? p->low_freq_scalar : nullptr, d.feat_scale ? p->high_freq_scalar : nullptr, sv.alpha, sv.mc,
                     g->output_head_w, g->output_head_b, g->norm2_b, g->gamma_att, d.feat_scale ? g->low_freq_scalar : nullptr,
-                    d.feat_scale ? g->high_freq_scalar : nullptr, don, st, fk, &fu2));
+                    d.feat_scale ? g->high_freq_scalar : nullptr, don, st, fk, &fu2, live_att));
     TRY(jobs.push(InReduceJob{sc.in_ws2, (int)d.F, d.E, p->norm2_w, p->norm2_b, nullptr, 1, g->norm2_w, g->norm2_b, nullptr, nullptr, nullptr, nullptr}));
     void* dqkv = sc.t3;
     {
@@ -1057,12 +1067,14 @@
         const bool rawm = raw_on && bf_attn_raw_modes(d.dtype, d.d);
         TRY(bf_attn_bwd_partials(d.dtype, sv.qkv, dO, dqkv, d.F * d.h, d.w, 1, d.w, 0, 1, d.heads, d.d, p->qnorm_w, p->qnorm_b, p->knorm_w, p->knorm_b,
                                  p->rel_pos_emb, d.attn_scale ? p->attn_scale_factor_x : nullptr, g->qnorm_w, g->qnorm_b, g->knorm_w, g->knorm_b,
-                                 g->rel_pos_emb, d.attn_scale ? g->attn_scale_factor_x : nullptr, 0.5f, rawm ? 2 : 0, sc.attn_ws, Scratch::ATTN_WS_FLOATS, &rows, st));
+                                 g->rel_pos_emb, d.attn_scale ? g->attn_scale_factor_x : nullptr, 0.5f, rawm ? 2 : 0, sc.attn_ws, Scratch::ATTN_WS_FLOATS, &rows, st,
+                                 live_groups(d, drop_att, d.F, d.h)));
         TRY(jobs.push(AttnReduceJob{sc.attn_ws, rows, d.d, d.heads, g->qnorm_w, g->qnorm_b, g->knorm_w, g->knorm_b, g->rel_pos_emb,
                                     d.attn_scale ? g->attn_scale_factor_x : nullptr}));
         TRY(bf_attn_bwd_partials(d.dtype, sv.qkv, dO, dqkv, d.F * d.w, d.h, d.w, d.S, 1, d.w, d.heads, d.d, p->qnorm_w, p->qnorm_b, p->knorm_w, p->knorm_b,
                                  p->rel_pos_emb, d.attn_scale ? p->attn_scale_factor_y : nullptr, g->qnorm_w, g->qnorm_b, g->knorm_w, g->knorm_b,
-                                 g->rel_pos_emb, d.attn_scale ? g->attn_scale_factor_y : nullptr, 0.5f, rawm ? 5 : 1, sc.attn_ws2, Scratch::ATTN_WS_FLOATS, &rows, st));
+                                 g->rel_pos_emb, d.attn_scale ? g->attn_scale_factor_y : nullptr, 0.5f, rawm ? 5 : 1, sc.attn_ws2, Scratch::ATTN_WS_FLOATS, &rows, st,
+                                 live_groups(d, drop_att, d.F, d.w)));
         TRY(jobs.push(AttnReduceJob{sc.attn_ws2, rows, d.d, d.heads, g->qnorm_w, g->qnorm_b, g->knorm_w, g->knorm_b, g->rel_pos_emb,
                                     d.attn_scale ? g->attn_scale_factor_y : nullptr}));
     }
@@ -1076,7 +1088,8 @@
         fu1.scaled_out = (char*)scratch + 2 * Scratch(d, nullptr).bytes + (L.dbr_flip ? dbr_bytes(d) : 0);
         fu1.scaled_f = ns.f; fu1.scaled_fdiv = ns.fdiv; fu1.scaled_done = &scaled_done;
     }
-    TRY(linear_bwd(d, sc, dqkv, 3 * d.E, sv.xn, d.E, BF_PRO_NONE, nullptr, nullptr, win_c, g->input_head_w, g->input_head_b, dxn, nullptr, st, fk, &fu1, true));
+    TRY(linear_bwd(d, sc, dqkv, 3 * d.E, sv.xn, d.E, BF_PRO_NONE, nullptr, nullptr, win_c, g->input_head_w, g->input_head_b, dxn, nullptr, st, fk, &fu1, true,
+                   nullptr, nullptr, nullptr, 1, nullptr, live_att));
     if (scaled_done) { L.dbr_ready = {dx, ns.f, fu1.scaled_out, st}; L.dbr_flip = !L.dbr_flip; }
     TRY(jobs.push(InReduceJob{sc.in_ws, (int)d.F, d.E, p->norm1_w, p->norm1_b, nullptr, 1, g->norm1_w, g->norm1_b, nullptr, nullptr, nullptr, nullptr}));
     static const bool merge_on = bf_knob("BF_REDUCE_MERGE", 1) != 0;
diff --git a/bubbleformer_amd/ops.py b/bubbleformer_amd/ops.py
--- a/bubbleformer_amd/ops.py
+++ b/bubbleformer_amd/ops.py
@@ -425,7 +425,7 @@
                      _p(drop_b), _stream())
         L.check(rc, f"bf_{ctx.kind}_bwd")
         if _DEFER["on"]:
-            _DEFER["keep"].append((saved, dout, x))
+            _DEFER["keep"].append((saved, dout, x, drop_a, drop_b))
         _stage_done(params, direct)
         return (dx, None, None, None, None, None, None, *ret)
 
@@ -520,7 +520,7 @@
         if not all(directs):
             L.check(lib.bf_side_join(_stream()), "bf_side_join")
         if _DEFER["on"]:
-            _DEFER["keep"].append((arena, acts, dout, x, gbuf))
+            _DEFER["keep"].append((arena, acts, dout, x, gbuf, da, db))
         flat_ret = [g for ret, mask in zip(rets, masks) for g, m in zip(ret, mask) if m]
         return (dx, None, None, None, None, *flat_ret)
 
diff --git a/include/bubbleformer_hip.h b/include/bubbleformer_hip.h
--- a/include/bubbleformer_hip.h
+++ b/include/bubbleformer_hip.h
@@ -77,6 +77,13 @@
 int bf_gemm_tokred(int dtype, int Nout, int Kin, int64_t M, const void* dy, int64_t ldy, const void* x, int64_t ldx, float* out,
                    int accumulate, float* colsum, float* ws, int64_t ws_floats, bf_stream_t stream);
 int64_t bf_gemm_tokred_ws_floats(int Nout, int Kin, int64_t M);
+int bf_gemm_tokred_live(int dtype, int Nout, int Kin, int64_t M, const void* dy, int64_t ldy, const void* x, int64_t ldx, float* out,
+                        int accumulate, float* colsum, float* ws, int64_t ws_floats, const float* live, int rows_per_group, int tile_rows,
+                        bf_stream_t stream);
+int bf_gemm_tokred_deferred_live(int dtype, int Nout, int Kin, int64_t M, const void* dy, int64_t ldy, const void* x, int64_t ldx, float* out,
+                                 int accumulate, float* colsum, float* ws, int64_t ws_floats, const float* live, int rows_per_group,
+                                 int tile_rows, bf_stream_t stream);
+int bf_gemm_tokred_flush_on(bf_stream_t stream);
 
 int bf_frame_linear(int dtype, int frames, int S, int K, int N, const void* A, int64_t lda, const void* W, int64_t ldw,
                     const float* norm_w, const float* norm_b, const float* bias, const float* colscale, const float* colshift,
@@ -115,11 +122,17 @@
                 float* dqb, float* dkw, float* dkb, float* demb, float* dhscale, float out_scale, int accumulate,
                 float* ws, int64_t ws_floats,
                 bf_stream_t stream);
+int bf_attn_bwd_live(int dtype, const void* qkv, const void* dout, void* dqkv, int64_t nseq, int L, int64_t inner,
+                     int64_t outer_stride, int64_t inner_stride, int64_t tok_stride, int heads, int d, const float* qw,
+                     const float* qb, const float* kw, const float* kb, const float* emb, const float* hscale, float* dqw,
+                     float* dqb, float* dkw, float* dkb, float* demb, float* dhscale, float out_scale, int accumulate,
+                     float* ws, int64_t ws_floats, const float* live, int seqs_per_group, bf_stream_t stream);
 
 void bf_side_defer(int on);
 int bf_side_join(bf_stream_t stream);
 void bf_debug_force_generic_attn(int on);
 void bf_debug_tokred_fold(int on);
+void bf_debug_drop_skip(int on);
 
 int bf_im2col_nchw(int dtype, const float* x, void* out, int frames, int C, int H, int W, int Kp, bf_stream_t stream);
 int bf_col2im_nchw(int dtype, const void* g, float* dx, int frames, int C, int H, int W, int Kp, bf_stream_t stream);
```

Result: no change. 826.2 samples/s, median of 4 (+0.5%).
